# Zehong-Ma/MagCache

Hardware: AMD Instinct MI355X
Metric: denoising steps/sec (MagCache on), Wan2.1-T2V-1.3B 480p 81f (higher is better)
Workload: dtype bf16

## Files before the change

### include/magcache_hip.h

```cpp
#ifndef MAGCACHE_HIP_H
#define MAGCACHE_HIP_H

#include <stddef.h>
#include <stdint.h>

#ifdef __cplusplus
extern "C" {
#endif

typedef struct mc_engine mc_engine;
typedef void* mc_stream;

typedef enum {
  MC_OK = 0,
  MC_EINVAL = 1,
  MC_ENOMEM = 2,
  MC_EHIP = 3,
  MC_ESTATE = 4
} mc_status;

typedef enum { MC_F32 = 0, MC_BF16 = 1 } mc_dtype;

typedef enum {
  MC_MODE_FULL = 0,
  MC_MODE_SKIP = 1,
  MC_MODE_CALIB = 2
} mc_mode;

typedef struct {
  int dim, ffn_dim, num_heads, num_layers;
  int in_dim, out_dim, freq_dim, text_dim, text_len;
  int latent_f, latent_h, latent_w;
  float eps;
  int sp_rank, sp_size;
  int n_branches;
  int calibration;
  int clip_dim;
  int vace_layers;
  int vace_stride;
  int vace_in_dim;
  int fp8_linear;
  int no_context_cache;
  int no_token_timesteps;
  int sp_phases;
} mc_config;

const char* mc_last_error(void);
const char* mc_version(void);
mc_status mc_set_option(const char* key, int value);

mc_status mc_create(const mc_config* cfg, mc_engine** out);
mc_status mc_create_sized(const mc_config* cfg, size_t cfg_bytes, mc_engine** out);
void mc_destroy(mc_engine* e);
size_t mc_workspace_bytes(const mc_engine* e);
mc_status mc_set_workspace(mc_engine* e, void* ws_dev, size_t bytes);
mc_status mc_geometry_bytes(const mc_engine* e, int latent_f, int latent_h, int latent_w, size_t* bytes);
mc_status mc_set_geometry(mc_engine* e, int latent_f, int latent_h, int latent_w);
mc_status mc_buffer_info(const mc_engine* e, const char* name, size_t* offset, size_t* bytes);

mc_status mc_set_weight(mc_engine* e, const char* name, const void* src_dev, mc_dtype dtype, const int64_t* shape,
                        int ndim, mc_stream stream);
int mc_weights_missing(const mc_engine* e, char* buf, size_t buflen);

mc_status mc_lora_set(mc_engine* e, const char* adapter, const char* weight_name, const void* down_dev, const int64_t* down_shape,
                      const void* up_dev, const int64_t* up_shape, mc_dtype dtype, float factor, mc_stream stream);
mc_status mc_lora_set_delta(mc_engine* e, const char* adapter, const char* param_name, const void* delta_dev, size_t numel,
                            mc_dtype dtype, mc_stream stream);
mc_status mc_lora_scale(mc_engine* e, const char* adapter, float scale);
mc_status mc_lora_remove(mc_engine* e, const char* adapter);
mc_status mc_lora_apply(mc_engine* e, mc_stream stream);
mc_status mc_lora_info(const mc_engine* e, int* adapters, int* params, size_t* base_bytes);

mc_status mc_forward(mc_engine* e, const float* latent_dev, const float* t_dev, double t_host,
                     const void* context_dev, mc_dtype ctx_dtype, int ctx_len, int branch, mc_mode mode,
                     float* out_dev, mc_stream stream);

mc_status mc_pair_begin(mc_engine* e);
mc_status mc_pair_end(mc_engine* e);

mc_status mc_set_context(mc_engine* e, int slot, const void* context_dev, mc_dtype ctx_dtype, int ctx_len,
                         mc_stream stream);
mc_status mc_use_context(mc_engine* e, int slot);

mc_status mc_set_clip_fea(mc_engine* e, const void* clip_dev, mc_dtype dtype, int n_tokens, mc_stream stream);

mc_status mc_set_vace_context(mc_engine* e, const float* vace_dev, float context_scale, mc_stream stream);

mc_status mc_set_token_timesteps(mc_engine* e, const float* t_tokens_dev, mc_stream stream);

typedef enum {
  MC_PROF_ATTN_SELF = 0,
  MC_PROF_ATTN_CROSS = 1,
  MC_PROF_GEMM_QKV = 2,
  MC_PROF_GEMM_O = 3,
  MC_PROF_GEMM_CROSS_Q = 4,
  MC_PROF_GEMM_CROSS_O = 5,
  MC_PROF_GEMM_FFN1 = 6,
  MC_PROF_GEMM_FFN2 = 7,
  MC_PROF_LN_MODULATE = 8,
  MC_PROF_RMSNORM_ROPE = 9,
  MC_PROF_EMBED = 10,
  MC_PROF_HEAD = 11,
  MC_PROF_OTHER = 12,
  MC_PROF_SP_WAIT = 13,
  MC_PROF_NCLASS = 14
} mc_prof_class;
mc_status mc_profile_enable(mc_engine* e, int level);
mc_status mc_profile_read(mc_engine* e, double* attn_ms_total, int* attn_launches);
mc_status mc_profile_read_classes(mc_engine* e, double ms_total[MC_PROF_NCLASS], int launches[MC_PROF_NCLASS]);

mc_status mc_embed(mc_engine* e, const float* latent_dev, const float* t_dev, double t_host,
                   const void* context_dev, mc_dtype ctx_dtype, int ctx_len, mc_stream stream);
mc_status mc_block_pre_attn(mc_engine* e, int layer, mc_stream stream);
mc_status mc_block_pre_kv(mc_engine* e, int layer, mc_stream stream);
mc_status mc_block_pre_q(mc_engine* e, int layer, mc_stream stream);
mc_status mc_sp_set_chunks(mc_engine* e, int chunks);
mc_status mc_sp_round_info(const mc_engine* e, int round, int* n_rounds, int* chunk_rows, int* valid);
mc_status mc_block_attn_local(mc_engine* e, int layer, mc_stream stream);
mc_status mc_block_attn_round(mc_engine* e, int layer, int round, mc_stream stream);
mc_status mc_block_post_attn(mc_engine* e, int layer, int branch, mc_mode mode, mc_stream stream);
typedef int (*mc_sp_gather_fn)(void* user, int layer, int phase, mc_stream stream);
mc_status mc_blocks_sp(mc_engine* e, int layer_begin, int layer_end, int branch, mc_mode mode, int overlap,
                       mc_sp_gather_fn gather, void* user, mc_stream stream);
mc_status mc_sp_geometry(const mc_engine* e, int* num_layers, int* seq_len, int* rows_per_rank, int* head_stride, int* dim,
                         int* sp_size);
void* mc_workspace_base(const mc_engine* e);

#define MC_SP_ID_BYTES 128
typedef struct mc_sp_comm mc_sp_comm;
int mc_sp_rccl_available(void);
mc_status mc_sp_comm_id(void* id_out);
mc_status mc_sp_comm_create(const void* id, int nranks, int rank, mc_sp_comm** out);
void mc_sp_comm_destroy(mc_sp_comm* c);
const char* mc_sp_comm_info(const mc_sp_comm* c);
mc_status mc_blocks_sp_rccl(mc_engine* e, mc_sp_comm* c, int layer_begin, int layer_end, int branch, mc_mode mode,
                            int overlap, mc_stream stream);
mc_status mc_forward_sp_rccl(mc_engine* e, mc_sp_comm* c, const float* latent_dev, const float* t_dev, double t_host,
                             const void* context_dev, mc_dtype ctx_dtype, int ctx_len, int branch, mc_mode mode,
                             int overlap, float* tokens_full_dev, float* out_dev, mc_stream stream);
mc_status mc_vace_block_pre(mc_engine* e, int i, mc_stream stream);
mc_status mc_vace_block_post(mc_engine* e, int i, int branch, mc_mode mode, mc_stream stream);
mc_status mc_head(mc_engine* e, int branch, mc_mode mode, mc_stream stream);
mc_status mc_unpatchify(mc_engine* e, const float* tokens_dev, int tok0, int n_tok, float* out_dev,
                        mc_stream stream);

mc_status mc_calib_ready(const mc_engine* e, int branch, int* has_stats);
mc_status mc_calib_finalize(mc_engine* e, int branch, mc_stream stream);
mc_status mc_state_reset(mc_engine* e);
mc_status mc_import_residual(mc_engine* e, int branch, const float* src_dev, mc_stream stream);

typedef struct mc_rule mc_rule;
enum {
  MC_RULE_WAN21 = 0,
  MC_RULE_HUNYUAN = 1,
  MC_RULE_FLUX = 2,
  MC_RULE_WAN22_T2V = 3,
  MC_RULE_WAN22_I2V = 4,
  MC_RULE_WAN22_TI2V = 5,
  MC_RULE_FRAMEPACK = 6,
  MC_RULE_OMNIGEN2 = 7,
  MC_RULE_QWEN = 8,
  MC_RULE_EVAL_WAN = 9,
  MC_RULE_EVAL_OPENSORA = 10
};
mc_rule* mc_rule_create(int variant, int num_steps, double thresh, int K, double retention_ratio,
                        const double* mag_ratios, int n_ratios, int split_step);
void mc_rule_destroy(mc_rule* r);
int mc_rule_step(mc_rule* r, int* branch);
int mc_rule_cnt(const mc_rule* r);
void mc_rule_state(const mc_rule* r, double acc_err[2], int acc_steps[2], double acc_ratio[2]);
void mc_nearest_interp(const double* src, int src_len, double* dst, int target_length);

mc_status mc_op_gemm_bf16(const void* A_dev, long lda, const void* W_dev, long ldw, const float* bias_dev, int M,
                          int N, int K, int epi, void* Cb_dev, long ldc, float* X_dev, long ldx,
                          const float* gate_dev, const void* X0_dev, long ldx0, float* R_dev, long ldr,
                          void* X0out_dev, long ldx0out, int m_valid, mc_stream stream);
mc_status mc_op_gemm_bf16_resid_sel(const void* A_dev, long lda, const void* W_dev, long ldw, const float* bias_dev, int M,
                                    int N, int K, int capture, float* X_dev, long ldx, const float* gate_dev,
                                    const float* gate2_dev, const unsigned char* gate_sel_dev, const void* X0_dev, long ldx0,
                                    float* R_dev, long ldr, mc_stream stream);
mc_status mc_op_gemm_bf16_rowsplit(const void* A_dev, long lda, const void* W_dev, const void* W_b_dev, long ldw,
                                   const float* bias_dev, const float* bias_b_dev, int M, int N, int K, int m_split, int epi,
                                   void* Cb_dev, long ldc, float* X_dev, long ldx, const float* gate_dev, const float* gate_b_dev,
                                   mc_stream stream);
mc_status mc_op_gemm_bf16_gelu_split(const void* A_dev, long lda, const void* W_dev, long ldw, const float* bias_dev, int M,
                                     int N, int K, int n_split, void* Cb_dev, long ldc, void* Cb2_dev, long ldc2,
                                     mc_stream stream);
int mc_op_gemm_bf16_kernel(int M, int N, int K, int epi);
mc_status mc_op_set_splitk_workspace(void* ws_dev, size_t bytes);
int mc_op_gemm_bf16_splitk(int M, int N, int K, int epi);
size_t mc_op_gemm_splitk_need(int M, int N, int K, int epi);
mc_status mc_op_quantize_rows_fp8(const void* x_dev, mc_dtype dtype, long ldx, int M, int K, void* q_dev, long ldq,
                                  float* scale_dev, mc_stream stream);
mc_status mc_op_gemm_fp8(const void* A_q_dev, long lda, const float* a_scale_dev, const void* W_q_dev, long ldw,
                         const float* w_scale_dev, const float* bias_dev, int M, int N, int K, int epi, void* Cb_dev,
                         long ldc, float* X_dev, long ldx, const float* gate_dev, mc_stream stream);
mc_status mc_op_quantize_rows_mx(const void* x_dev, mc_dtype dtype, long ldx, int M, int K, void* q_dev, long ldq,
                                 void* scales_dev, long rows_pad, mc_stream stream);
mc_status mc_op_gemm_mxfp8(const void* A_q_dev, long lda, const void* a_scales_dev, long rows_pad_a, const void* W_q_dev,
                           long ldw, const void* w_scales_dev, long rows_pad_w, const float* bias_dev, int M, int N, int K,
                           int epi, void* Cb_dev, long ldc, float* X_dev, long ldx, const float* gate_dev,
                           mc_stream stream);
mc_status mc_op_attention(const void* Q_dev, long ldq, const void* K_dev, long ldk, long k_shard_stride,
                          const void* V_dev, long ldv, long v_shard_stride, void* O_dev, long ldo, int Lq_pad,
                          int n_heads, int shard_rows, int shard_valid, int n_shards, float scale,
                          mc_stream stream);
mc_status mc_op_attention_partial(const void* Q_dev, long ldq, const void* K_dev, long ldk, long k_shard_stride,
                                  const void* V_dev, long ldv, long v_shard_stride, void* O_dev, long ldo,
                                  int Lq_pad, int n_heads, int shard_rows, int shard_valid, int n_shards,
                                  float scale, int skip_shard, float* lse_out_dev, const float* lse_in_dev,
                                  mc_stream stream);
mc_status mc_op_attn_merge(const void* const* o_parts, const float* const* lse_parts, int n, void* out_bf16_dev, long ldo,
                           int rows, int rows_pad, int d, mc_stream stream);
mc_status mc_op_ln_modulate(const float* x_dev, long ldx, const void* x0_dev, long ldx0, const float* sc_dev,
                            const float* sh_dev, int mode, float eps, void* out_bf16_dev, long ldo,
                            float* out_f32_dev, long ldof, int M, int D, mc_stream stream);
mc_status mc_op_rmsnorm_rope(void* x_bf16_dev, long ldx, const float* w_dev, float eps, const float* cs_dev,
                             int cs_row0, int M, int D, mc_stream stream);
mc_status mc_op_skip_add(const void* x0_bf16_dev, long ldx0, const float* r_dev, long ldr, float* out_dev, long ldo,
                         int M, int D, mc_stream stream);
mc_status mc_op_residual_sub(const float* x_dev, long ldx, const void* x0_bf16_dev, long ldx0, float* r_dev,
                             long ldr, int M, int D, mc_stream stream);
mc_status mc_op_add_rows(float* x_dev, long ldx, const void* s_dev, mc_dtype s_dtype, float* r_dev, long ldr,
                         const void* x0_bf16_dev, long ldx0, int rows, int D, mc_stream stream);
mc_status mc_op_calib_stats(const float* r_dev, long ldr, const float* rp_dev, long ldrp, int M, int D,
                            double* partial_dev, int n_blocks, double* sums_dev, float* stats_dev,
                            mc_stream stream);
mc_status mc_op_cfg_euler(const float* cond_dev, const float* uncond_dev, float guide, float dt, float* x_dev,
                          float* eps_out_dev, size_t n, mc_stream stream);
mc_status mc_op_cfg_norm_euler(const float* cond_dev, const float* uncond_dev, long ld_pred, float guide, float dt,
                               float* x_dev, long ldx, int n_rows, int C, mc_stream stream);
mc_status mc_op_rmsnorm_rows_bf16(const float* x_dev, long ldx, const float* w_dev, float eps, void* out_bf16_dev, long ldo,
                                  int rows_valid, int rows, int D, mc_stream stream);
mc_status mc_op_lincomb(const float* const* xs_dev, const float* coef, int k, float* out_dev, size_t n,
                        mc_stream stream);
mc_status mc_op_cast_bf16(const float* src_dev, void* dst_bf16_dev, size_t n, mc_stream stream);
mc_status mc_op_rope_table(int F, int Hp, int Wp, int tok0, int n_tok, float* cs_host);
mc_status mc_op_rope_axes(int F, int Hp, int Wp, float* axes_host, size_t* n_floats);
mc_status mc_op_rope_expand(const float* axes_dev, int F, int Hp, int Wp, int tok0, int n_tok, int n_rows, float* cs_dev,
                            mc_stream stream);

#define MC_LORA_MAX_TERMS 8
typedef struct mc_lora_term {
  const void* down;
  const void* up;
  int rank;
  float scale;
} mc_lora_term;
size_t mc_op_lora_merge_scratch(int rows, int K, const mc_lora_term* terms, int n_terms);
mc_status mc_op_lora_merge(const void* base_dev, long ld_base, void* out_dev, long ld_out, int rows, int K,
                           const mc_lora_term* terms, int n_terms, void* scratch_dev, size_t scratch_bytes, mc_stream stream);
mc_status mc_op_lora_merge_f32(const float* base_dev, long ld_base, float* out_dev, long ld_out, int rows, int K,
                               const mc_lora_term* terms, int n_terms, void* scratch_dev, size_t scratch_bytes, mc_stream stream);
mc_status mc_op_param_delta(const float* base_dev, float* out_dev, size_t n, const float* const* deltas, const float* scales,
                            int n_terms, mc_stream stream);

#ifdef __cplusplus
}
#endif
#endif
```

### magcache_amd/_lib.py

```python
import ctypes as C
import os

_HERE = os.path.dirname(os.path.abspath(__file__))
LIB_PATH = os.path.join(_HERE, "libmagcache_hip.so")
LIB_PATH = os.environ.get("MAGCACHE_HIP_LIB", LIB_PATH)

MC_OK, MC_EINVAL, MC_ENOMEM, MC_EHIP, MC_ESTATE = 0, 1, 2, 3, 4
MC_F32, MC_BF16 = 0, 1
MC_MODE_FULL, MC_MODE_SKIP, MC_MODE_CALIB = 0, 1, 2
PROF_CLASSES = ("attn_self", "attn_cross", "gemm_qkv", "gemm_o", "gemm_cross_q", "gemm_cross_o", "gemm_ffn1", "gemm_ffn2",
                "ln_modulate", "rmsnorm_rope", "embed", "head", "other", "sp_wait")
RULE_VARIANTS = {"wan21": 0, "hunyuan": 1, "flux": 2, "wan22_t2v": 3, "wan22_i2v": 4, "wan22_ti2v": 5, "framepack": 6,
                 "omnigen2": 7, "qwen": 8, "eval_wan": 9, "eval_opensora": 10}


class McConfig(C.Structure):
    _fields_ = [(n, C.c_int) for n in ("dim", "ffn_dim", "num_heads", "num_layers", "in_dim", "out_dim", "freq_dim",
                                       "text_dim", "text_len", "latent_f", "latent_h", "latent_w")] + \
               [("eps", C.c_float)] + \
               [(n, C.c_int) for n in ("sp_rank", "sp_size", "n_branches", "calibration", "clip_dim", "vace_layers",
                                         "vace_stride", "vace_in_dim", "fp8_linear", "no_context_cache",
                                         "no_token_timesteps", "sp_phases")]


class MagCacheHipError(RuntimeError):
    def __init__(self, status, msg):
        super().__init__(f"magcache_hip status {status}: {msg}")
        self.status = status


_vp, _i, _l, _f, _d, _sz = C.c_void_p, C.c_int, C.c_long, C.c_float, C.c_double, C.c_size_t
SP_GATHER_FN = C.CFUNCTYPE(C.c_int, C.c_void_p, C.c_int, C.c_int, C.c_void_p)

SIGNATURES = {
    "mc_last_error": (C.c_char_p, []),
    "mc_version": (C.c_char_p, []),
    "mc_set_option": (_i, [C.c_char_p, _i]),
    "mc_create": (_i, [C.POINTER(McConfig), C.POINTER(_vp)]),
    "mc_create_sized": (_i, [C.POINTER(McConfig), _sz, C.POINTER(_vp)]),
    "mc_destroy": (None, [_vp]),
    "mc_workspace_bytes": (_sz, [_vp]),
    "mc_set_workspace": (_i, [_vp, _vp, _sz]),
    "mc_geometry_bytes": (_i, [_vp, _i, _i, _i, C.POINTER(_sz)]),
    "mc_set_geometry": (_i, [_vp, _i, _i, _i]),
    "mc_buffer_info": (_i, [_vp, C.c_char_p, C.POINTER(_sz), C.POINTER(_sz)]),
    "mc_set_weight": (_i, [_vp, C.c_char_p, _vp, _i, C.POINTER(C.c_int64), _i, _vp]),
    "mc_weights_missing": (_i, [_vp, C.c_char_p, _sz]),
    "mc_forward": (_i, [_vp, _vp, _vp, _d, _vp, _i, _i, _i, _i, _vp, _vp]),
    "mc_pair_begin": (_i, [_vp]),
    "mc_pair_end": (_i, [_vp]),
    "mc_set_clip_fea": (_i, [_vp, _vp, _i, _i, _vp]),
    "mc_set_vace_context": (_i, [_vp, _vp, _f, _vp]),
    "mc_set_token_timesteps": (_i, [_vp, _vp, _vp]),
    "mc_set_context": (_i, [_vp, _i, _vp, _i, _i, _vp]),
    "mc_use_context": (_i, [_vp, _i]),
    "mc_profile_enable": (_i, [_vp, _i]),
    "mc_profile_read": (_i, [_vp, C.POINTER(_d), C.POINTER(_i)]),
    "mc_profile_read_classes": (_i, [_vp, C.POINTER(_d), C.POINTER(_i)]),
    "mc_embed": (_i, [_vp, _vp, _vp, _d, _vp, _i, _i, _vp]),
    "mc_block_pre_attn": (_i, [_vp, _i, _vp]),
    "mc_block_pre_kv": (_i, [_vp, _i, _vp]),
    "mc_block_pre_q": (_i, [_vp, _i, _vp]),
    "mc_sp_set_chunks": (_i, [_vp, _i]),
    "mc_sp_round_info": (_i, [_vp, _i, C.POINTER(_i), C.POINTER(_i), C.POINTER(_i)]),
    "mc_sp_geometry": (_i, [_vp] + [C.POINTER(_i)] * 6),
    "mc_workspace_base": (_vp, [_vp]),
    "mc_block_attn_local": (_i, [_vp, _i, _vp]),
    "mc_block_attn_round": (_i, [_vp, _i, _i, _vp]),
    "mc_sp_rccl_available": (_i, []),
    "mc_sp_comm_id": (_i, [_vp]),
    "mc_sp_comm_create": (_i, [_vp, _i, _i, C.POINTER(_vp)]),
    "mc_sp_comm_destroy": (None, [_vp]),
    "mc_sp_comm_info": (C.c_char_p, [_vp]),
    "mc_blocks_sp_rccl": (_i, [_vp, _vp, _i, _i, _i, _i, _i, _vp]),
    "mc_forward_sp_rccl": (_i, [_vp, _vp, _vp, _vp, _d, _vp, _i, _i, _i, _i, _i, _vp, _vp, _vp]),
    "mc_block_post_attn": (_i, [_vp, _i, _i, _i, _vp]),
    "mc_blocks_sp": (_i, [_vp, _i, _i, _i, _i, _i, _vp, _vp, _vp]),
    "mc_vace_block_pre": (_i, [_vp, _i, _vp]),
    "mc_vace_block_post": (_i, [_vp, _i, _i, _i, _vp]),
    "mc_head": (_i, [_vp, _i, _i, _vp]),
    "mc_unpatchify": (_i, [_vp, _vp, _i, _i, _vp, _vp]),
    "mc_calib_ready": (_i, [_vp, _i, C.POINTER(_i)]),
    "mc_calib_finalize": (_i, [_vp, _i, _vp]),
    "mc_state_reset": (_i, [_vp]),
    "mc_import_residual": (_i, [_vp, _i, _vp, _vp]),
    "mc_rule_create": (_vp, [_i, _i, _d, _i, _d, C.POINTER(_d), _i, _i]),
    "mc_rule_destroy": (None, [_vp]),
    "mc_rule_step": (_i, [_vp, C.POINTER(_i)]),
    "mc_rule_cnt": (_i, [_vp]),
    "mc_rule_state": (None, [_vp, C.POINTER(_d), C.POINTER(_i), C.POINTER(_d)]),
    "mc_nearest_interp": (None, [C.POINTER(_d), _i, C.POINTER(_d), _i]),
    "mc_op_gemm_bf16": (_i, [_vp, _l, _vp, _l, _vp, _i, _i, _i, _i, _vp, _l, _vp, _l, _vp, _vp, _l, _vp, _l, _vp, _l,
                             _i, _vp]),
    "mc_op_gemm_bf16_resid_sel": (_i, [_vp, _l, _vp, _l, _vp, _i, _i, _i, _i, _vp, _l, _vp, _vp, _vp, _vp, _l, _vp, _l, _vp]),
    "mc_op_gemm_bf16_rowsplit": (_i, [_vp, _l, _vp, _vp, _l, _vp, _vp, _i, _i, _i, _i, _i, _vp, _l, _vp, _l, _vp, _vp, _vp]),
    "mc_op_gemm_bf16_gelu_split": (_i, [_vp, _l, _vp, _l, _vp, _i, _i, _i, _i, _vp, _l, _vp, _l, _vp]),
    "mc_op_gemm_bf16_kernel": (_i, [_i, _i, _i, _i]),
    "mc_op_gemm_bf16_splitk": (_i, [_i, _i, _i, _i]),
    "mc_op_gemm_splitk_need": (_sz, [_i, _i, _i, _i]),
    "mc_op_set_splitk_workspace": (_i, [_vp, _sz]),
    "mc_op_attention": (_i, [_vp, _l, _vp, _l, _l, _vp, _l, _l, _vp, _l, _i, _i, _i, _i, _i, _f, _vp]),
    "mc_op_quantize_rows_fp8": (_i, [_vp, _i, _l, _i, _i, _vp, _l, _vp, _vp]),
    "mc_op_gemm_fp8": (_i, [_vp, _l, _vp, _vp, _l, _vp, _vp, _i, _i, _i, _i, _vp, _l, _vp, _l, _vp, _vp]),
    "mc_op_quantize_rows_mx": (_i, [_vp, _i, _l, _i, _i, _vp, _l, _vp, _l, _vp]),
    "mc_op_gemm_mxfp8": (_i, [_vp, _l, _vp, _l, _vp, _l, _vp, _l, _vp, _i, _i, _i, _i, _vp, _l, _vp, _l, _vp, _vp]),
    "mc_op_attention_partial": (_i, [_vp, _l, _vp, _l, _l, _vp, _l, _l, _vp, _l, _i, _i, _i, _i, _i, _f, _i, _vp, _vp, _vp]),
    "mc_op_attn_merge": (_i, [_vp, _vp, _i, _vp, _l, _i, _i, _i, _vp]),
    "mc_op_ln_modulate": (_i, [_vp, _l, _vp, _l, _vp, _vp, _i, _f, _vp, _l, _vp, _l, _i, _i, _vp]),
    "mc_op_rmsnorm_rope": (_i, [_vp, _l, _vp, _f, _vp, _i, _i, _i, _vp]),
    "mc_op_skip_add": (_i, [_vp, _l, _vp, _l, _vp, _l, _i, _i, _vp]),
    "mc_op_residual_sub": (_i, [_vp, _l, _vp, _l, _vp, _l, _i, _i, _vp]),
    "mc_op_calib_stats": (_i, [_vp, _l, _vp, _l, _i, _i, _vp, _i, _vp, _vp, _vp]),
    "mc_op_cfg_euler": (_i, [_vp, _vp, _f, _f, _vp, _vp, _sz, _vp]),
    "mc_op_cast_bf16": (_i, [_vp, _vp, _sz, _vp]),
    "mc_op_cfg_norm_euler": (_i, [_vp, _vp, _l, _f, _f, _vp, _l, _i, _i, _vp]),
    "mc_op_rmsnorm_rows_bf16": (_i, [_vp, _l, _vp, _f, _vp, _l, _i, _i, _i, _vp]),
    "mc_op_lincomb": (_i, [_vp, _vp, _i, _vp, _sz, _vp]),
    "mc_op_add_rows": (_i, [_vp, _l, _vp, _i, _vp, _l, _vp, _l, _i, _i, _vp]),
    "mc_op_rope_table": (_i, [_i, _i, _i, _i, _i, _vp]),
    "mc_op_rope_axes": (_i, [_i, _i, _i, _vp, C.POINTER(_sz)]),
    "mc_op_rope_expand": (_i, [_vp, _i, _i, _i, _i, _i, _i, _vp, _vp]),
    "mc_op_lora_merge_scratch": (_sz, [_i, _i, _vp, _i]),
    "mc_op_lora_merge": (_i, [_vp, _l, _vp, _l, _i, _i, _vp, _i, _vp, _sz, _vp]),
    "mc_op_lora_merge_f32": (_i, [_vp, _l, _vp, _l, _i, _i, _vp, _i, _vp, _sz, _vp]),
    "mc_op_param_delta": (_i, [_vp, _vp, _sz, C.POINTER(_vp), C.POINTER(_f), _i, _vp]),
    "mc_lora_set": (_i, [_vp, C.c_char_p, C.c_char_p, _vp, C.POINTER(C.c_int64), _vp, C.POINTER(C.c_int64), _i, _f, _vp]),
    "mc_lora_set_delta": (_i, [_vp, C.c_char_p, C.c_char_p, _vp, _sz, _i, _vp]),
    "mc_lora_scale": (_i, [_vp, C.c_char_p, _f]),
    "mc_lora_remove": (_i, [_vp, C.c_char_p]),
    "mc_lora_apply": (_i, [_vp, _vp]),
    "mc_lora_info": (_i, [_vp, C.POINTER(_i), C.POINTER(_i), C.POINTER(_sz)]),
    "mc_mmdit_create": (_i, [_vp, C.POINTER(_vp)]),
    "mc_mmdit_create_sized": (_i, [_vp, _sz, C.POINTER(_vp)]),
    "mc_mmdit_destroy": (None, [_vp]),
    "mc_mmdit_workspace_bytes": (_sz, [_vp]),
    "mc_mmdit_set_workspace": (_i, [_vp, _vp, _sz]),
    "mc_mmdit_buffer_info": (_i, [_vp, C.c_char_p, C.POINTER(_sz), C.POINTER(_sz)]),
    "mc_mmdit_geometry_bytes": (_i, [_vp, _i, _i, _i, _i, _i, C.POINTER(_sz)]),
    "mc_mmdit_set_geometry": (_i, [_vp, _i, _i, _i, _i, _i]),
    "mc_mmdit_set_weight": (_i, [_vp, C.c_char_p, _vp, _i, C.POINTER(C.c_int64), _i, _vp]),
    "mc_mmdit_weights_missing": (_i, [_vp, C.c_char_p, _sz]),
    "mc_mmdit_lora_set": (_i, [_vp, C.c_char_p, C.c_char_p, _vp, C.POINTER(C.c_int64), _vp, C.POINTER(C.c_int64), _i, _f, _vp]),
    "mc_mmdit_lora_scale": (_i, [_vp, C.c_char_p, _f]),
    "mc_mmdit_lora_remove": (_i, [_vp, C.c_char_p]),
    "mc_mmdit_lora_apply": (_i, [_vp, _vp]),
    "mc_mmdit_lora_info": (_i, [_vp, C.POINTER(_i), C.POINTER(_i), C.POINTER(_sz)]),
    "mc_mmdit_set_rope": (_i, [_vp, _vp, _vp, _i, _vp]),
    "mc_mmdit_set_controlnet": (_i, [_vp, _vp, _i, _vp, _i, _i, _i]),
    "mc_mmdit_controlnet_index": (_i, [_i, _i, _i, _i]),
    "mc_mmdit_forward": (_i, [_vp, _vp, _d, _d, _vp, _i, _vp, _i, _vp, _vp]),
    "mc_mmdit_forward2": (_i, [_vp, _vp, _d, _d, _vp, _i, _vp, _i, _i, _vp, _vp]),
    "mc_mmdit_begin": (_i, [_vp, _vp, _d, _d, _vp, _i, _vp, _i, _vp]),
    "mc_mmdit_block_pre": (_i, [_vp, _i, _vp]),
    "mc_mmdit_block_attn_local": (_i, [_vp, _i, _vp]),
    "mc_mmdit_block_post": (_i, [_vp, _i, _vp]),
    "mc_mmdit_end": (_i, [_vp, _vp, _vp]),
    "mc_mmdit_unpatchify": (_i, [_vp, _vp, _vp, _vp]),
    "mc_mmdit_calib_stats": (_i, [_vp, C.POINTER(C.c_float), _vp]),
    "mc_mmdit_state_reset": (_i, [_vp]),
}


class McMmditConfig(C.Structure):
    _fields_ = [(n, C.c_int) for n in ("family", "dim", "num_heads", "n_double", "n_single", "in_channels", "out_channels",
                                       "txt_dim", "txt_len", "vec_dim", "img_tokens", "latent_f", "latent_h", "latent_w",
                                       "refiner_depth", "calibration", "sp_rank", "sp_size",
                                       "fp8_linear")]


MC_FAMILY_FLUX, MC_FAMILY_HUNYUAN, MC_FAMILY_QWEN = 0, 1, 2
MC_LORA_MAX_TERMS = 8


class McLoraTerm(C.Structure):
    _fields_ = [("down", C.c_void_p), ("up", C.c_void_p), ("rank", C.c_int), ("scale", C.c_float)]


_lib = None


def load():
    global _lib
    if _lib is not None:
        return _lib
    if not os.path.exists(LIB_PATH):
        raise ImportError(f"{LIB_PATH} not found: the HIP engine is not built (python -m magcache_amd.build). "
                          "magcache_amd has no CPU fallback by design.")
    import torch
    lib = C.CDLL(LIB_PATH)
    for name, (res, args) in SIGNATURES.items():
        fn = getattr(lib, name)
        fn.restype = res
        fn.argtypes = args
    _lib = lib
    for kv in filter(None, os.environ.get("MAGCACHE_HIP_OPTIONS", "").split(",")):
        key, _, val = kv.partition("=")
        check(lib.mc_set_option(key.strip().encode(), int(val)))
    return lib


def check(status):
    if status != MC_OK:
        raise MagCacheHipError(status, load().mc_last_error().decode())
```

### magcache_amd/csrc/engine.cpp

```cpp
#include <cmath>
#include <cstddef>
#include <memory>

#include "host.h"

using mc::align_up;
using mc::bf16_t;
using mc::fail;
using mc::Keys;
using mc::Linear;
using mc::RowRange;
using mc::whole;

namespace {

struct Layer {
  Linear qkv, o, cq, ckv, co, ffn1, ffn2;
  float *nq, *nk, *cnq, *cnk, *n3w, *n3b, *mod;
  Linear ckv_img;
  float* cnk_img = nullptr;
  int index = 0;
};

}

constexpr int kSpMaxParts = 9;

struct mc_engine {
  mc_config cfg;
  int d, ffn, H, NL, L, Lr, Lp, P, rank, tok0, Kp;
  int ctx_rows;
  std::vector<Layer> layers;
  Linear patch, text0, text1;
  float *w_time0, *b_time0, *w_time1, *b_time1, *w_tproj, *b_tproj;
  float *w_head, *b_head, *head_mod;
  Linear img1, img3;
  float *ln_img0_w = nullptr, *ln_img0_b = nullptr, *ln_img4_w = nullptr, *ln_img4_b = nullptr;
  int img_rows = 0;
  bool have_clip = false;
  bool sp = false;
  int sp_chunks = 1;
  int attn_layer = -2;
  int attn_launches = 0;
  bool attn_local_done = false;
  int attn_rounds_done = 0;
  hipStream_t side = nullptr;
  hipEvent_t ev_fork = nullptr, ev_join = nullptr;
  size_t splitk_bytes = 0;
  bool ctx_valid[2] = {false, false};
  int ctx_active = -1;
  const float* tok_t = nullptr;
  int HT = 64;
  int profile = 0;
  std::vector<hipEvent_t> prof_ev;
  std::vector<uint8_t> prof_cls;
  size_t prof_n = 0;
  std::vector<Layer> vlayers;
  Linear vpatch, before;
  std::vector<Linear> after;
  float* vscale = nullptr;
  int NV = 0, Kvp = 0;
  bool have_vace = false;
  float* cs_table = nullptr;
  float* rope_axes = nullptr;
  int cs_rows = 0;
  size_t axes_cap = 0;
  bool phase_open = false;
  mc::WeightStore weights;
  mc::Workspace work;
  int res_slot[2] = {0, 1};
  int res_scratch = 2;
  bool have_res[2] = {false, false};
  bool have_stats[2] = {false, false};
  bool embedded = false;
  enum { PAIR_NONE, PAIR_ARMED, PAIR_KEPT, PAIR_DEAD };
  int pair = PAIR_NONE;
  const float *pair_latent = nullptr, *pair_t_dev = nullptr;
  double pair_t_host = 0.0;
  bool pair_capable() const { return !sp && NV == 0 && cfg.clip_dim == 0 && cfg.fp8_linear == 0; }
  void pair_drop() { if (pair != PAIR_NONE) pair = PAIR_DEAD; }

  template <class T>
  T* buf(const char* name) const { return work.get<T>(name); }
  float* residual(int idx) const {
    static const char* names[3] = {"residual0", "residual1", "residual2"};
    return buf<float>(names[idx]);
  }
  const Layer& layer(int flat) const { return flat < NL ? layers[flat] : vlayers[flat - NL]; }
  const float* emod(const Layer& l) const { return buf<float>("emod") + (size_t)l.index * 6 * d; }
};

namespace {

struct Prof {
  mc_engine* e;
  hipStream_t s;
  size_t idx = 0;
  bool on = false;
  Prof(mc_engine* e_, int cls, hipStream_t s_) : e(e_), s(s_) {
    if (cls < 0 || !e->profile || (e->profile < 2 && cls != MC_PROF_ATTN_SELF) || e->prof_n + 2 > e->prof_ev.size()) return;
    idx = e->prof_n;
    if (hipEventRecord(e->prof_ev[idx], s) != hipSuccess) return;
    e->prof_cls[idx / 2] = (uint8_t)cls;
    e->prof_n += 2;
    on = true;
  }
  ~Prof() {
    if (on && hipEventRecord(e->prof_ev[idx + 1], s) != hipSuccess) e->prof_cls[idx / 2] = 0xff;
  }
  Prof(const Prof&) = delete;
  Prof& operator=(const Prof&) = delete;
};

constexpr int kRopeT = mc::kRopePairsT, kRopeHW = mc::kRopePairsHW;
constexpr double kRopeDimT = 44.0, kRopeDimHW = 42.0;

inline void rope_pair(int pos, int j, double dim, float* cs) {
  const double fr = 1.0 / std::pow(10000.0, (2.0 * j) / dim);
  const double a = (double)pos * fr;
  cs[0] = (float)std::cos(a);
  cs[1] = (float)std::sin(a);
}

void rope_table_host(int F, int Hp, int Wp, int tok0, int n_tok, float* cs) {
  const int c = kRopeT + 2 * kRopeHW;
  for (int r = 0; r < n_tok; ++r) {
    const int tok = tok0 + r;
    float* row = cs + (size_t)r * 2 * c;
    if (tok >= F * Hp * Wp) {
      for (int i = 0; i < c; ++i) { row[2 * i] = 1.f; row[2 * i + 1] = 0.f; }
      continue;
    }
    const int f = tok / (Hp * Wp), rem = tok % (Hp * Wp), h = rem / Wp, w = rem % Wp;
    for (int i = 0; i < c; ++i) {
      if (i < kRopeT) rope_pair(f, i, kRopeDimT, row + 2 * i);
      else if (i < kRopeT + kRopeHW) rope_pair(h, i - kRopeT, kRopeDimHW, row + 2 * i);
      else rope_pair(w, i - kRopeT - kRopeHW, kRopeDimHW, row + 2 * i);
    }
  }
}

size_t rope_axes_floats(int F, int Hp, int Wp) { return 2 * ((size_t)F * kRopeT + ((size_t)Hp + Wp) * kRopeHW); }

void rope_axes_host(int F, int Hp, int Wp, float* axes) {
  for (int f = 0; f < F; ++f)
    for (int j = 0; j < kRopeT; ++j, axes += 2) rope_pair(f, j, kRopeDimT, axes);
  for (int h = 0; h < Hp; ++h)
    for (int j = 0; j < kRopeHW; ++j, axes += 2) rope_pair(h, j, kRopeDimHW, axes);
  for (int w = 0; w < Wp; ++w)
    for (int j = 0; j < kRopeHW; ++j, axes += 2) rope_pair(w, j, kRopeDimHW, axes);
}

struct Rows { int L, Lr, Lp, tok0; };

mc_status check_geometry(int latent_f, int latent_h, int latent_w, int P) {
  if ((latent_h & 1) || (latent_w & 1) || latent_f <= 0 || latent_h <= 0 || latent_w <= 0)
    return fail(MC_EINVAL, "latent grid %dx%dx%d not divisible by patch (1,2,2)", latent_f, latent_h, latent_w);
  const long long L = (long long)latent_f * (latent_h / 2) * (latent_w / 2);
  if (L > (1ll << 24)) return fail(MC_EINVAL, "latent grid %dx%dx%d: %lld tokens", latent_f, latent_h, latent_w, L);
  if (L % P) return fail(MC_EINVAL, "seq_len %d not divisible by sp_size %d", (int)L, P);
  return MC_OK;
}

Rows derive_rows(int latent_f, int latent_h, int latent_w, int P, int rank) {
  Rows r;
  r.L = latent_f * (latent_h / 2) * (latent_w / 2);
  r.Lr = r.L / P;
  r.Lp = (int)align_up(r.Lr, 256);
  r.tok0 = rank * r.Lr;
  return r;
}

size_t splitk_need(const mc_engine* e, int Lp) {
  return e->sp ? mc::gemm_splitk_ws_need(Lp, e->d, e->ffn, mc::EPI_RESID_GATE) : 0;
}

void plan_workspace(const mc_engine* e, const Rows& rows, mc::Workspace& ws) {
  const mc_config& c = e->cfg;
  const size_t d = e->d, ffn = e->ffn;
  const size_t Lp = rows.Lp;
  ws.add("x", Lp * d * 4);
  ws.add("x0", Lp * d * 2);
  ws.add("xn", Lp * d * 2);
  ws.add("qkv", Lp * 3 * d * 2);
  ws.add("ao", Lp * d * 2);
  ws.add("h", std::max(Lp * ffn * 2, Lp * d * 4));
  ws.add("tokens", Lp * e->Kp * 2);
  ws.add("ctx_in", (size_t)e->ctx_rows * c.text_dim * 2);
  ws.add("ctx_h", (size_t)e->ctx_rows * d * 2);
  ws.add("ctx", (size_t)e->ctx_rows * d * 2);
  ws.add("ckv", (size_t)e->ctx_rows * 2 * d * 2);
  ws.add("ctx_cache", (size_t)2 * e->ctx_rows * d * 2);
  if (!c.no_context_cache)
    ws.add("ckv_cache", (size_t)2 * (e->NL + e->NV) * e->ctx_rows * 2 * d * 2);
  const size_t tsets = c.no_token_timesteps ? 1 : 2;
  ws.add("temb", tsets * (c.freq_dim + 2 * d + 6 * d) * 4);
  ws.add("emod", tsets * (e->NL + e->NV) * 6 * d * 4);
  ws.add("tok_sel", c.no_token_timesteps ? 256 : (size_t)Lp + 256);
  ws.add("tok_t2", 64);
  if (c.fp8_linear) {
    ws.add("aq", Lp * std::max(d, ffn));
    ws.add("a_scale", Lp * 4);
    if (c.fp8_linear >= 2) ws.add("a_mx", (std::max(d, ffn) / 32) * Lp);
  }
  if (e->NV > 0) {
    ws.add("xc", Lp * d * 4);
    ws.add("c0", Lp * d * 2);
    ws.add("vtokens", Lp * (size_t)e->Kvp * 2);
  }
  ws.add("ehead", 2 * 2 * d * 4);
  ws.add("head_tokens", (size_t)Lp * e->HT * 4);
  ws.add("kv_local", e->sp ? Lp * 2 * d * 2 : 256);
  ws.add("kv_gather", e->sp ? (size_t)e->P * Lp * 2 * d * 2 : 256);
  ws.add("residual0", Lp * d * 4);
  ws.add("residual1", c.n_branches > 1 ? Lp * d * 4 : 256);
  ws.add("residual2", c.calibration ? Lp * d * 4 : 256);
  if (c.clip_dim > 0) {
    const size_t ir = e->img_rows, cd = c.clip_dim;
    ws.add("clip_in", ir * cd * 4);
    ws.add("clip_n", ir * cd * 2);
    ws.add("clip_h", ir * cd * 2);
    ws.add("clip_o", ir * d * 4);
    ws.add("clip_h2", ir * d * 2);
    ws.add("ctx_img", ir * d * 2);
    ws.add("ckv_img", ir * 2 * d * 2);
    ws.add("ao2", Lp * d * 2);
  }
  if (e->sp) ws.add("attn_lse", (size_t)e->H * Lp * 4);
  const size_t splitk = splitk_need(e, rows.Lp);
  ws.add("splitk", splitk ? splitk : 256);
  ws.add("ao_part", e->P > 1 ? (size_t)kSpMaxParts * Lp * d * 2 : 256);
  ws.add("lse_part", e->P > 1 ? (size_t)kSpMaxParts * e->H * Lp * 4 : 256);
  ws.add("calib_partial", (2048 * 4 + 2) * 8);
  ws.add("calib_sums", 4 * 8);
  ws.add("calib_stats", 2 * 3 * 4);
  ws.add("pair_x", e->pair_capable() ? Lp * d * 4 : 256);
  ws.add("pair_cq", e->pair_capable() ? Lp * d * 2 : 256);
}

mc_status rope_reserve(mc_engine* e, int Lp, size_t axes_floats) {
  if (Lp > e->cs_rows) {
    float* grown = nullptr;
    MC_TRY(e->weights.alloc(&grown, (size_t)Lp * 128));
    if (e->cs_table) e->weights.release(e->cs_table);
    e->cs_table = grown;
    e->cs_rows = Lp;
  }
  if (axes_floats > e->axes_cap) {
    float* grown = nullptr;
    MC_TRY(e->weights.alloc(&grown, axes_floats));
    if (e->rope_axes) e->weights.release(e->rope_axes);
    e->rope_axes = grown;
    e->axes_cap = axes_floats;
  }
  return MC_OK;
}

mc_status rope_build(mc_engine* e) {
  const int F = e->cfg.latent_f, Hp = e->cfg.latent_h / 2, Wp = e->cfg.latent_w / 2;
  std::vector<float> axes(rope_axes_floats(F, Hp, Wp));
  rope_axes_host(F, Hp, Wp, axes.data());
  HIP_TRY(hipMemcpy(e->rope_axes, axes.data(), axes.size() * sizeof(float), hipMemcpyHostToDevice));
  HIP_TRY(mc::launch_rope_expand(e->rope_axes, F, Hp, Wp, e->tok0, e->Lr, e->Lp, e->cs_table, nullptr));
  HIP_TRY(hipStreamSynchronize(nullptr));
  return MC_OK;
}

mc_status forget_workspace_state(mc_engine* e) {
  e->have_res[0] = e->have_res[1] = false;
  e->have_stats[0] = e->have_stats[1] = false;
  e->res_slot[0] = 0; e->res_slot[1] = 1; e->res_scratch = 2;
  e->embedded = e->phase_open = false;
  e->ctx_valid[0] = e->ctx_valid[1] = false;
  e->ctx_active = -1;
  e->have_clip = e->have_vace = false;
  e->tok_t = nullptr;
  e->attn_layer = -2;
  e->pair_drop();
  if (e->work.ws) HIP_TRY(hipMemset(e->buf<double>("calib_partial") + 2048 * 4, 0, 16));
  return MC_OK;
}

mc_status check_ready(const mc_engine* e) {
  if (!e) return fail(MC_EINVAL, "null engine");
  if (e->weights.dirty()) return fail(MC_ESTATE, "LoRA adapters, scales or a touched weight changed: call mc_lora_apply first");
  return mc::check_ready(e->work, e->weights, "mc_set_workspace");
}

struct ActSrc {
  const bf16_t* rows = nullptr; long ld = 0;
  bool quantised = false;
  uint8_t *q = nullptr, *mx = nullptr;
};

mc_status linear(mc_engine* e, const Linear& l, RowRange out, int M, ActSrc a, mc::GemmParams p, int epi, hipStream_t s) {
  const int K = l.k_in;
  if (!l.q) {
    HIP_TRY(mc::launch_linear_bf16(l, out, a.rows, a.ld, M, p, epi, s));
    return MC_OK;
  }
  const int Lp = e->Lp;
  if (M != Lp) return fail(MC_EINVAL, "an fp8 Linear runs over the %d rows of a block, not %d", Lp, M);
  p.M = Lp; p.N = out.count; p.K = K; p.bias = l.b + out.first;
  uint8_t* aq = a.q ? a.q : e->buf<uint8_t>("aq");
  p.A = (const bf16_t*)aq; p.lda = K; p.W = (const bf16_t*)(l.q + (size_t)out.first * K); p.ldw = K;
  if (l.mx) {
    uint8_t* am = a.mx ? a.mx : e->buf<uint8_t>("a_mx");
    if (!a.quantised) HIP_TRY(mc::launch_quantize_rows_mx(a.rows, nullptr, a.ld, Lp, K, aq, K, am, (long)Lp, s));
    p.a_mx = am; p.mx_rows_a = (long)Lp; p.w_mx = l.mx + out.first; p.mx_rows_w = l.n_out;
    HIP_TRY(mc::launch_gemm_mxfp8(p, epi, s));
    return MC_OK;
  }
  float* as = e->buf<float>("a_scale");
  if (!a.quantised) HIP_TRY(mc::launch_quantize_rows_fp8(a.rows, nullptr, a.ld, Lp, K, aq, K, as, s));
  p.a_scale = as; p.w_scale = l.q_scale + out.first;
  HIP_TRY(mc::launch_gemm_fp8(p, epi, s));
  return MC_OK;
}
mc_status linear_bf16_out(mc_engine* e, const Linear& l, int M, ActSrc a, bf16_t* C, int epi, hipStream_t s) {
  mc::GemmParams p = {};
  p.Cb = C; p.ldc = l.n_out;
  return linear(e, l, whole(l), M, a, p, epi, s);
}

Keys kv_pairs(const bf16_t* kv, int d, int rows, int valid) { return {kv, kv + d, 2L * d, 0, rows, valid, 1, 0}; }
Keys qkv_keys(const mc_engine* e) {
  const bf16_t* k = e->buf<bf16_t>("qkv") + e->d;
  return {k, k + e->d, 3L * e->d, 0, e->Lp, e->Lr, 1, 0};
}
Keys local_keys(const mc_engine* e) { return kv_pairs(e->buf<bf16_t>("kv_local"), e->d, e->Lp, e->Lr); }
int sp_chunk_rows(const mc_engine* e) { return e->Lp / e->sp_chunks; }
int sp_round_valid(const mc_engine* e, int c) {
  const int lc = sp_chunk_rows(e);
  return std::max(0, std::min(lc, e->Lr - c * lc));
}
int sp_rounds(const mc_engine* e) {
  const int lc = sp_chunk_rows(e);
  return (e->Lr + lc - 1) / lc;
}
Keys sp_keys(const mc_engine* e, int round, bool skip_own) {
  if (round < 0) return local_keys(e);
  const int lc = sp_chunk_rows(e), d = e->d;
  Keys k = kv_pairs(e->buf<bf16_t>("kv_gather") + (size_t)round * e->P * lc * 2 * d, d, lc, sp_round_valid(e, round));
  k.stride = (long)lc * 2 * d; k.n_shards = e->P; k.skip_shard_p1 = skip_own ? e->rank + 1 : 0;
  return k;
}
mc_status attend(const mc_engine* e, const bf16_t* Q, long ldq, bf16_t* O, const Keys& keys, const float* lse_in, float* lse_out,
                 hipStream_t s) {
  HIP_TRY(mc::launch_attention_keys(Q, ldq, O, e->d, e->Lp, e->H, keys, lse_in, lse_out, s));
  return MC_OK;
}
void attn_chain_set(mc_engine* e, int layer, int launches, bool local_done, int rounds_done) {
  e->attn_layer = layer; e->attn_launches = launches; e->attn_local_done = local_done; e->attn_rounds_done = rounds_done;
}
void attn_chain_open(mc_engine* e, int layer) {
  if (e->attn_layer != layer) attn_chain_set(e, layer, 0, false, 0);
}

}

namespace mc {
int g_fp8_fused_quant = 1;
int g_sp_attn_partials = 1;
}
static int g_n_cu = 0;

extern "C" {

mc_status mc_create_sized(const mc_config* cfg, size_t cfg_bytes, mc_engine** out) {
  if (!cfg || !out) return fail(MC_EINVAL, "null argument");
  if (cfg_bytes < offsetof(mc_config, fp8_linear) || cfg_bytes > sizeof(mc_config) || (cfg_bytes % sizeof(int)) != 0)
    return fail(MC_EINVAL, "mc_config of %zu bytes: this library knows %zu (0.1 layout) .. %zu", cfg_bytes,
                offsetof(mc_config, fp8_linear), sizeof(mc_config));
  mc_config full;
  memset(&full, 0, sizeof(full));
  memcpy(&full, cfg, cfg_bytes);
  return mc_create(&full, out);
}

mc_status mc_create(const mc_config* cfg, mc_engine** out) {
  if (!cfg || !out) return fail(MC_EINVAL, "null argument");
  const mc_config& c = *cfg;
  if (c.dim <= 0 || c.num_heads <= 0 || c.dim != c.num_heads * 128)
    return fail(MC_EINVAL, "dim (%d) must be num_heads (%d) * 128", c.dim, c.num_heads);
  if ((c.dim % 256) || (c.ffn_dim % 64) || (c.text_dim % 64) || (c.freq_dim % 4) || c.num_layers <= 0)
    return fail(MC_EINVAL, "unsupported geometry dim=%d ffn=%d text_dim=%d", c.dim, c.ffn_dim, c.text_dim);
  if (c.sp_size < 1 || c.sp_rank < 0 || c.sp_rank >= c.sp_size) return fail(MC_EINVAL, "bad sp rank/size");
  MC_TRY(check_geometry(c.latent_f, c.latent_h, c.latent_w, c.sp_size));
  if (c.n_branches != 1 && c.n_branches != 2) return fail(MC_EINVAL, "n_branches must be 1 or 2");
  if (c.out_dim * 4 > 256) return fail(MC_EINVAL, "out_dim*4 > 256 unsupported by the head kernel");
  if (c.clip_dim < 0 || (c.clip_dim % 256) != 0) return fail(MC_EINVAL, "clip_dim %d must be 0 or a multiple of 256", c.clip_dim);
  if (c.vace_layers < 0 || (c.vace_layers > 0 && (c.vace_stride <= 0 || c.vace_in_dim <= 0 ||
                                                   (c.vace_layers - 1) * c.vace_stride >= c.num_layers)))
    return fail(MC_EINVAL, "bad VACE geometry: %d blocks, stride %d, in_dim %d", c.vace_layers, c.vace_stride, c.vace_in_dim);
  if ((c.no_context_cache | c.no_token_timesteps) & ~1) return fail(MC_EINVAL, "no_context_cache / no_token_timesteps must be 0 or 1");
  if (c.fp8_linear < 0 || c.fp8_linear > 3)
    return fail(MC_EINVAL, "fp8_linear must be 0, 1 (per-row scales), 2 (MX block scales: QKV, FFN-1, FFN-2) or 3 (MX, the d x d Linears too)");
  if (c.fp8_linear && ((c.dim % 256) || (c.ffn_dim % 256) || c.dim < 512 || c.ffn_dim < 512))
    return fail(MC_EINVAL, "fp8_linear needs dim and ffn_dim to be multiples of 256 and >= 512");
  if (c.vace_layers > 0 && c.sp_size > 1 && (c.vace_layers - 1) * c.vace_stride == c.num_layers - 1)
    return fail(MC_EINVAL, "VACE with a hint on the last layer is single-GPU in this engine");

  std::unique_ptr<mc_engine, void (*)(mc_engine*)> own(new mc_engine(), mc_destroy);
  mc_engine* e = own.get();
  e->cfg = c;
  e->d = c.dim; e->ffn = c.ffn_dim; e->H = c.num_heads; e->NL = c.num_layers;
  e->P = c.sp_size; e->rank = c.sp_rank;
  e->sp = c.sp_size > 1 || c.sp_phases != 0;
  const Rows rows = derive_rows(c.latent_f, c.latent_h, c.latent_w, e->P, e->rank);
  e->L = rows.L; e->Lr = rows.Lr; e->Lp = rows.Lp; e->tok0 = rows.tok0;
  e->Kp = (int)align_up((size_t)c.in_dim * 4, 64);
  e->HT = (int)align_up((size_t)c.out_dim * 4, 64);
  e->ctx_rows = (int)align_up(c.text_len, 64);
  const size_t d = e->d, ffn = e->ffn;
  mc::WeightStore& W = e->weights;
  W.allow_f32_targets = true;

  const mc::Quant q_big = c.fp8_linear >= 2 ? mc::QUANT_MX : c.fp8_linear == 1 ? mc::QUANT_ROW : mc::QUANT_NONE;
  const mc::Quant q_dd = c.fp8_linear == 3 ? mc::QUANT_MX : mc::QUANT_NONE;
  e->layers.resize(e->NL);
  e->NV = c.vace_layers;
  e->vlayers.resize(e->NV);
  for (int i = 0; i < e->NL + e->NV; ++i) {
    const bool is_vace = i >= e->NL;
    Layer& l = is_vace ? e->vlayers[i - e->NL] : e->layers[i];
    l.index = i;
    const std::string p = (is_vace ? "vace_blocks." + std::to_string(i - e->NL) : "blocks." + std::to_string(i)) + ".";
    MC_TRY(W.add_linear(l.qkv, p + "self_attn.", {{"q", d}, {"k", d}, {"v", d}}, d, q_big));
    MC_TRY(W.add_linear(l.o, p + "self_attn.", {{"o", d}}, d, q_dd));
    MC_TRY(W.add_linear(l.cq, p + "cross_attn.", {{"q", d}}, d, q_dd));
    MC_TRY(W.add_linear(l.ckv, p + "cross_attn.", {{"k", d}, {"v", d}}, d));
    MC_TRY(W.add_linear(l.co, p + "cross_attn.", {{"o", d}}, d, q_dd));
    MC_TRY(W.add_linear(l.ffn1, p + "ffn.", {{"0", ffn}}, d, q_big));
    MC_TRY(W.add_linear(l.ffn2, p + "ffn.", {{"2", d}}, ffn, q_big));
    MC_TRY(W.add_f32(l.nq, p + "self_attn.norm_q.weight", d));
    MC_TRY(W.add_f32(l.nk, p + "self_attn.norm_k.weight", d));
    MC_TRY(W.add_f32(l.n3w, p + "norm3.weight", d));
    MC_TRY(W.add_f32(l.n3b, p + "norm3.bias", d));
    MC_TRY(W.add_f32(l.cnq, p + "cross_attn.norm_q.weight", d));
    MC_TRY(W.add_f32(l.cnk, p + "cross_attn.norm_k.weight", d));
    MC_TRY(W.add_f32(l.mod, p + "modulation", 6 * d));
    if (c.clip_dim > 0) {
      MC_TRY(W.add_linear(l.ckv_img, p + "cross_attn.", {{"k_img", d}, {"v_img", d}}, d));
      MC_TRY(W.add_f32(l.cnk_img, p + "cross_attn.norm_k_img.weight", d));
    }
  }
  if (e->NV > 0) {
    e->Kvp = (int)align_up((size_t)c.vace_in_dim * 4, 64);
    const size_t kv = (size_t)c.vace_in_dim * 4;
    if (kv != (size_t)e->Kvp) { return fail(MC_EINVAL, "vace_in_dim*4 must be a multiple of 64"); }
    MC_TRY(W.add_linear(e->vpatch, "", {{"vace_patch_embedding", d}}, kv));
    W.slots.at("vace_patch_embedding.weight").fixed = true;
    MC_TRY(W.add_linear(e->before, "vace_blocks.0.", {{"before_proj", d}}, d));
    MC_TRY(W.alloc(&e->vscale, d));
    e->after.resize(e->NV);
    for (int i = 0; i < e->NV; ++i)
      MC_TRY(W.add_linear(e->after[i], "vace_blocks." + std::to_string(i) + ".", {{"after_proj", d}}, d));
  }
  if (c.clip_dim > 0) {
    const size_t cd = c.clip_dim;
    e->img_rows = (int)align_up(257, 64);
    MC_TRY(W.add_f32(e->ln_img0_w, "img_emb.proj.0.weight", cd));
    MC_TRY(W.add_f32(e->ln_img0_b, "img_emb.proj.0.bias", cd));
    MC_TRY(W.add_linear(e->img1, "img_emb.proj.", {{"1", cd}}, cd));
    MC_TRY(W.add_linear(e->img3, "img_emb.proj.", {{"3", d}}, cd));
    MC_TRY(W.add_f32(e->ln_img4_w, "img_emb.proj.4.weight", d));
    MC_TRY(W.add_f32(e->ln_img4_b, "img_emb.proj.4.bias", d));
  }
  const size_t kin = (size_t)c.in_dim * 4;
  MC_TRY(W.alloc_linear(e->patch, d, e->Kp));
  HIP_TRY(hipMemset(e->patch.w, 0, d * e->Kp * sizeof(bf16_t)));
  mc::Slot& w_patch = W.add_parts(e->patch, "", {{"patch_embedding", d}});
  w_patch.fixed = true;
  if (kin != (size_t)e->Kp) {
    w_patch.numel = d * kin;
    w_patch.pad = {d, kin, (size_t)e->Kp};
  }
  MC_TRY(W.add_linear(e->text0, "text_embedding.", {{"0", d}}, c.text_dim));
  MC_TRY(W.add_linear(e->text1, "text_embedding.", {{"2", d}}, d));
  MC_TRY(W.add_f32(e->w_time0, "time_embedding.0.weight", d * c.freq_dim, c.freq_dim));
  MC_TRY(W.add_f32(e->b_time0, "time_embedding.0.bias", d));
  MC_TRY(W.add_f32(e->w_time1, "time_embedding.2.weight", d * d, d));
  MC_TRY(W.add_f32(e->b_time1, "time_embedding.2.bias", d));
  MC_TRY(W.add_f32(e->w_tproj, "time_projection.1.weight", 6 * d * d, d));
  MC_TRY(W.add_f32(e->b_tproj, "time_projection.1.bias", 6 * d));
  MC_TRY(W.add_f32(e->w_head, "head.head.weight", (size_t)c.out_dim * 4 * d, d));
  MC_TRY(W.add_f32(e->b_head, "head.head.bias", (size_t)c.out_dim * 4));
  MC_TRY(W.add_f32(e->head_mod, "head.modulation", 2 * d));

  MC_TRY(rope_reserve(e, e->Lp, rope_axes_floats(c.latent_f, c.latent_h / 2, c.latent_w / 2)));
  MC_TRY(rope_build(e));

  e->splitk_bytes = splitk_need(e, e->Lp);
  plan_workspace(e, rows, e->work);
  *out = own.release();
  return MC_OK;
}

void mc_destroy(mc_engine* e) {
  if (!e) return;
  e->weights.free_all();
  for (hipEvent_t ev : e->prof_ev) (void)hipEventDestroy(ev);
  if (e->ev_fork) (void)hipEventDestroy(e->ev_fork);
  if (e->ev_join) (void)hipEventDestroy(e->ev_join);
  if (e->side) (void)hipStreamDestroy(e->side);
  delete e;
}

size_t mc_workspace_bytes(const mc_engine* e) { return e ? e->work.need : 0; }

mc_status mc_set_workspace(mc_engine* e, void* ws_dev, size_t bytes) {
  if (!e) return fail(MC_EINVAL, "null argument");
  MC_TRY(e->work.bind(ws_dev, bytes));
  return forget_workspace_state(e);
}

mc_status mc_geometry_bytes(const mc_engine* e, int latent_f, int latent_h, int latent_w, size_t* bytes) {
  if (!e || !bytes) return fail(MC_EINVAL, "null argument");
  MC_TRY(check_geometry(latent_f, latent_h, latent_w, e->P));
  mc::Workspace plan;
  plan_workspace(e, derive_rows(latent_f, latent_h, latent_w, e->P, e->rank), plan);
  *bytes = plan.need;
  return MC_OK;
}

mc_status mc_set_geometry(mc_engine* e, int latent_f, int latent_h, int latent_w) {
  if (!e) return fail(MC_EINVAL, "null engine");
  if (e->sp)
    return fail(MC_EINVAL, "mc_set_geometry: a sharded engine (sp_size %d%s) keeps the grid it was created with", e->P,
                e->cfg.sp_phases ? ", sp_phases" : "");
  if (e->phase_open) return fail(MC_ESTATE, "mc_set_geometry between mc_embed and mc_head");
  MC_TRY(check_geometry(latent_f, latent_h, latent_w, e->P));
  const Rows r = derive_rows(latent_f, latent_h, latent_w, e->P, e->rank);
  mc::Workspace plan;
  plan_workspace(e, r, plan);
  if (e->work.ws && plan.need > e->work.bound)
    return fail(MC_EINVAL, "latent grid %dx%dx%d needs a workspace of %zu bytes, %zu bytes are bound (mc_set_workspace)", latent_f,
                latent_h, latent_w, plan.need, e->work.bound);
  HIP_TRY(hipDeviceSynchronize());
  MC_TRY(rope_reserve(e, r.Lp, rope_axes_floats(latent_f, latent_h / 2, latent_w / 2)));
  MC_TRY(e->work.replan(plan));
  e->cfg.latent_f = latent_f; e->cfg.latent_h = latent_h; e->cfg.latent_w = latent_w;
  e->L = r.L; e->Lr = r.Lr; e->Lp = r.Lp; e->tok0 = r.tok0;
  MC_TRY(rope_build(e));
  return forget_workspace_state(e);
}

mc_status mc_buffer_info(const mc_engine* e, const char* name, size_t* offset, size_t* bytes) {
  if (!e || !name) return fail(MC_EINVAL, "null argument");
  std::string n(name);
  if (n == "residual_branch0" || n == "residual_branch1") {
    static const char* names[3] = {"residual0", "residual1", "residual2"};
    n = names[e->res_slot[n.back() - '0']];
  }
  return e->work.info(n, offset, bytes);
}

mc_status mc_set_weight(mc_engine* e, const char* name, const void* src_dev, mc_dtype dtype, const int64_t* shape,
                        int ndim, mc_stream stream) {
  if (e) {
    e->ctx_valid[0] = e->ctx_valid[1] = false;
    e->ctx_active = -1;
    e->pair_drop();
  }
  if (!e || !name || !src_dev || !shape) return fail(MC_EINVAL, "null argument");
  return e->weights.set(name, src_dev, dtype, shape, ndim, (hipStream_t)stream);
}

int mc_weights_missing(const mc_engine* e, char* buf, size_t buflen) { return e ? e->weights.missing(buf, buflen) : -1; }

static mc_status lora_entry(const mc_engine* e, const char* what) {
  if (!e) return fail(MC_EINVAL, "null engine");
  if (e->pair != mc_engine::PAIR_NONE) return fail(MC_ESTATE, "%s between mc_pair_begin and mc_pair_end", what);
  if (e->phase_open) return fail(MC_ESTATE, "%s between mc_embed and mc_head", what);
  return MC_OK;
}

mc_status mc_lora_set(mc_engine* e, const char* adapter, const char* weight_name, const void* down_dev, const int64_t* down_shape,
                      const void* up_dev, const int64_t* up_shape, mc_dtype dtype, float factor, mc_stream stream) {
  MC_TRY(lora_entry(e, "mc_lora_set"));
  if (!adapter || !weight_name || !down_dev || !down_shape || !up_dev || !up_shape) return fail(MC_EINVAL, "null argument");
  if (down_shape[0] <= 0 || down_shape[0] > (1 << 20) || down_shape[1] <= 0 || up_shape[0] <= 0 || up_shape[1] != down_shape[0])
    return fail(MC_EINVAL, "LoRA '%s': down [%lld, %lld] and up [%lld, %lld] share no rank", weight_name, (long long)down_shape[0],
                (long long)down_shape[1], (long long)up_shape[0], (long long)up_shape[1]);
  return e->weights.lora_set(adapter, weight_name, down_dev, (size_t)down_shape[0] * down_shape[1], up_dev,
                             (size_t)up_shape[0] * up_shape[1], dtype, (int)down_shape[0], factor, (hipStream_t)stream);
}

mc_status mc_lora_set_delta(mc_engine* e, const char* adapter, const char* param_name, const void* delta_dev, size_t numel,
                            mc_dtype dtype, mc_stream stream) {
  MC_TRY(lora_entry(e, "mc_lora_set_delta"));
  if (!adapter || !param_name || !delta_dev) return fail(MC_EINVAL, "null argument");
  return e->weights.lora_set_delta(adapter, param_name, delta_dev, numel, dtype, (hipStream_t)stream);
}

mc_status mc_lora_scale(mc_engine* e, const char* adapter, float scale) {
  MC_TRY(lora_entry(e, "mc_lora_scale"));
  if (!adapter) return fail(MC_EINVAL, "null argument");
  return e->weights.lora_scale(adapter, scale);
}

mc_status mc_lora_remove(mc_engine* e, const char* adapter) {
  MC_TRY(lora_entry(e, "mc_lora_remove"));
  return e->weights.lora_remove(adapter);
}

mc_status mc_lora_apply(mc_engine* e, mc_stream stream) {
  MC_TRY(lora_entry(e, "mc_lora_apply"));
  int merged = 0;
  const mc_status st = e->weights.lora_apply((hipStream_t)stream, &merged);
  if (merged > 0) {
    e->ctx_valid[0] = e->ctx_valid[1] = false;
    e->ctx_active = -1;
    e->have_clip = e->have_vace = false;
    e->pair_drop();
  }
  return st;
}

mc_status mc_lora_info(const mc_engine* e, int* adapters, int* params, size_t* base_bytes) {
  if (!e) return fail(MC_EINVAL, "null engine");
  e->weights.lora_info(adapters, params, base_bytes);
  return MC_OK;
}

mc_status mc_set_clip_fea(mc_engine* e, const void* clip_dev, mc_dtype dtype, int n_tokens, mc_stream stream_) {
  hipStream_t s = (hipStream_t)stream_;
  MC_TRY(check_ready(e));
  e->pair_drop();
  const mc_config& c = e->cfg;
  if (c.clip_dim <= 0) return fail(MC_EINVAL, "engine was created without clip_dim (t2v model)");
  if (!clip_dev || n_tokens != 257) return fail(MC_EINVAL, "clip_fea must be [257, %d]", c.clip_dim);
  const int cd = c.clip_dim, ir = e->img_rows, d = e->d;
  float* in = e->buf<float>("clip_in");
  HIP_TRY(hipMemsetAsync(in, 0, (size_t)ir * cd * 4, s));
  if (dtype == MC_F32) {
    HIP_TRY(hipMemcpyAsync(in, clip_dev, (size_t)n_tokens * cd * 4, hipMemcpyDeviceToDevice, s));
  } else {
    return fail(MC_EINVAL, "clip_fea must be given as fp32");
  }
  bf16_t* n0 = e->buf<bf16_t>("clip_n");
  HIP_TRY(mc::launch_ln_modulate(in, cd, nullptr, 0, e->ln_img0_w, e->ln_img0_b, 1, 1e-5f, n0, cd, nullptr, 0, ir, cd, s));
  MC_TRY(linear_bf16_out(e, e->img1, ir, ActSrc{n0, cd}, e->buf<bf16_t>("clip_h"), mc::EPI_GELU_ERF_BF16, s));
  MC_TRY(linear_bf16_out(e, e->img3, ir, ActSrc{e->buf<bf16_t>("clip_h"), cd}, e->buf<bf16_t>("clip_h2"), mc::EPI_BF16, s));
  HIP_TRY(hipMemsetAsync(e->buf<float>("clip_o"), 0, (size_t)ir * d * 4, s));
  HIP_TRY(mc::launch_ln_modulate(e->buf<float>("clip_o"), d, e->buf<bf16_t>("clip_h2"), d, e->ln_img4_w,
                                 e->ln_img4_b, 1, 1e-5f, e->buf<bf16_t>("ctx_img"), d, nullptr, 0, ir, d, s));
  e->have_clip = true;
  return MC_OK;
}

mc_status mc_set_vace_context(mc_engine* e, const float* vace_dev, float context_scale, mc_stream stream_) {
  hipStream_t s = (hipStream_t)stream_;
  MC_TRY(check_ready(e));
  e->pair_drop();
  if (e->NV <= 0) return fail(MC_EINVAL, "engine was created without VACE blocks");
  const mc_config& c = e->cfg;
  const int d = e->d;
  if (vace_dev) {
    bf16_t* vt = e->buf<bf16_t>("vtokens");
    HIP_TRY(mc::launch_patchify(vace_dev, c.vace_in_dim, c.latent_f, c.latent_h, c.latent_w, e->tok0, e->Lr, e->Lp, vt,
                                e->Kvp, s));
    mc::GemmParams p = {};
    p.X = e->buf<float>("xc"); p.ldx = d;
    p.X0out = e->buf<bf16_t>("c0"); p.ldx0out = d;
    p.m_valid = e->Lr;
    MC_TRY(linear(e, e->vpatch, whole(e->vpatch), e->Lp, ActSrc{vt, e->Kvp}, p, mc::EPI_EMBED, s));
    e->have_vace = true;
  } else if (!e->have_vace) {
    return fail(MC_EINVAL, "null vace_context and none set before");
  }
  std::vector<float> sc(d, context_scale);
  HIP_TRY(hipMemcpyAsync(e->vscale, sc.data(), (size_t)d * 4, hipMemcpyHostToDevice, s));
  HIP_TRY(hipStreamSynchronize(s));
  return MC_OK;
}

static mc_status embed_context(mc_engine* e, const void* context_dev, mc_dtype ctx_dtype, int ctx_len, bf16_t* dst,
                               hipStream_t s) {
  const mc_config& c = e->cfg;
  if (ctx_len <= 0 || ctx_len > c.text_len)
    return fail(MC_EINVAL, "context length %d exceeds text_len %d", ctx_len, c.text_len);
  bf16_t* ctx_in = e->buf<bf16_t>("ctx_in");
  if (ctx_dtype == MC_F32) {
    HIP_TRY(mc::launch_cast_pad_bf16((const float*)context_dev, c.text_dim, ctx_len, e->ctx_rows, c.text_dim, ctx_in,
                                     c.text_dim, s));
  } else {
    HIP_TRY(hipMemsetAsync(ctx_in, 0, (size_t)e->ctx_rows * c.text_dim * 2, s));
    HIP_TRY(hipMemcpyAsync(ctx_in, context_dev, (size_t)ctx_len * c.text_dim * 2, hipMemcpyDeviceToDevice, s));
  }
  bf16_t* ctx_h = e->buf<bf16_t>("ctx_h");
  MC_TRY(linear_bf16_out(e, e->text0, e->ctx_rows, ActSrc{ctx_in, c.text_dim}, ctx_h, mc::EPI_GELU_BF16, s));
  return linear_bf16_out(e, e->text1, e->ctx_rows, ActSrc{ctx_h, e->d}, dst, mc::EPI_BF16, s);
}

static mc_status context_kv(mc_engine* e, const Layer& l, const bf16_t* ctx, bf16_t* ckv, hipStream_t s) {
  const int d = e->d;
  MC_TRY(linear_bf16_out(e, l.ckv, e->ctx_rows, ActSrc{ctx, d}, ckv, mc::EPI_BF16, s));
  HIP_TRY(mc::launch_rmsnorm_rope(ckv, 2 * d, l.cnk, e->cfg.eps, nullptr, 0, e->ctx_rows, d, s));
  return MC_OK;
}

static mc_status embed_latent_time(mc_engine* e, const float* latent_dev, const float* t_dev, double t_host, float* x,
                                   hipStream_t s) {
  const mc_config& c = e->cfg;
  const int d = e->d;
  bf16_t* tokens = e->buf<bf16_t>("tokens");
  if (e->Kp != c.in_dim * 4) HIP_TRY(hipMemsetAsync(tokens, 0, (size_t)e->Lp * e->Kp * 2, s));
  HIP_TRY(mc::launch_patchify(latent_dev, c.in_dim, c.latent_f, c.latent_h, c.latent_w, e->tok0, e->Lr, e->Lp,
                              tokens, e->Kp, s));
  {
    mc::GemmParams p = {};
    p.X = x; p.ldx = d;
    p.X0out = e->buf<bf16_t>("x0"); p.ldx0out = d;
    p.m_valid = e->Lr;
    MC_TRY(linear(e, e->patch, whole(e->patch), e->Lp, ActSrc{tokens, e->Kp}, p, mc::EPI_EMBED, s));
  }
  const int n_sets = e->tok_t ? 2 : 1;
  float* t2 = e->buf<float>("tok_t2");
  if (e->tok_t)
    HIP_TRY(mc::launch_token_t_prepare(e->tok_t, e->L, e->tok0, e->Lr, e->Lp, t2, e->buf<uint8_t>("tok_sel"), s));
  const size_t temb_set = (size_t)c.freq_dim + 2 * d + 6 * d, emod_set = (size_t)(e->NL + e->NV) * 6 * d;
  for (int set = 0; set < n_sets; ++set) {
    float* temb = e->buf<float>("temb") + set * temb_set;
    float* sinus = temb;
    float* h1 = temb + c.freq_dim;
    float* ev = h1 + d;
    float* e0 = ev + d;
    HIP_TRY(mc::launch_sinusoid(e->tok_t ? t2 + set : t_dev, t_host, c.freq_dim, sinus, s));
    HIP_TRY(mc::launch_gemv_f32(e->w_time0, sinus, e->b_time0, h1, d, c.freq_dim, 0, 1, s));
    HIP_TRY(mc::launch_gemv_f32(e->w_time1, h1, e->b_time1, ev, d, d, 0, 0, s));
    HIP_TRY(mc::launch_gemv_f32(e->w_tproj, ev, e->b_tproj, e0, 6 * d, d, 1, 0, s));
    float* emod = e->buf<float>("emod") + set * emod_set;
    for (int l = 0; l < e->NL + e->NV; ++l)
      HIP_TRY(mc::launch_add_bcast(e0, 6 * d, e->layer(l).mod, emod + (size_t)l * 6 * d, 6 * d, s));
    HIP_TRY(mc::launch_add_bcast(ev, d, e->head_mod, e->buf<float>("ehead") + set * 2 * d, 2 * d, s));
  }
  return MC_OK;
}

static mc_status embed_text(mc_engine* e, const void* context_dev, mc_dtype ctx_dtype, int ctx_len, hipStream_t s) {
  if (context_dev) {
    e->ctx_active = -1;
    return embed_context(e, context_dev, ctx_dtype, ctx_len, e->buf<bf16_t>("ctx"), s);
  }
  if (e->ctx_active < 0 || !e->ctx_valid[e->ctx_active])
    return fail(MC_ESTATE, "context_dev is NULL but no cached context is selected (mc_set_context)");
  return MC_OK;
}

static mc_status embed(mc_engine* e, const float* latent_dev, const float* t_dev, double t_host, const void* context_dev,
                       mc_dtype ctx_dtype, int ctx_len, float* x, hipStream_t s) {
  MC_TRY(check_ready(e));
  if (!latent_dev) return fail(MC_EINVAL, "null input");
  if (e->cfg.clip_dim > 0 && !e->have_clip)
    return fail(MC_ESTATE, "i2v model: mc_set_clip_fea must run before the forward (reference assert :226-227)");
  Prof pr(e, MC_PROF_EMBED, s);
  MC_TRY(embed_latent_time(e, latent_dev, t_dev, t_host, x, s));
  MC_TRY(embed_text(e, context_dev, ctx_dtype, ctx_len, s));
  e->embedded = true;
  return MC_OK;
}

mc_status mc_embed(mc_engine* e, const float* latent_dev, const float* t_dev, double t_host,
                   const void* context_dev, mc_dtype ctx_dtype, int ctx_len, mc_stream stream_) {
  if (e) e->pair_drop();
  const mc_status st = embed(e, latent_dev, t_dev, t_host, context_dev, ctx_dtype, ctx_len, e ? e->buf<float>("x") : nullptr,
                             (hipStream_t)stream_);
  if (e && st == MC_OK) e->phase_open = true;
  return st;
}

static mc_status ln_for_gemm(mc_engine* e, const Linear& l, const float* x, const float* sc, const float* sh, int mode,
                             const float* sc2, const float* sh2, const uint8_t* sel, hipStream_t s, ActSrc* a) {
  const int d = e->d, Lp = e->Lp;
  bf16_t* xn = e->buf<bf16_t>("xn");
  *a = ActSrc{xn, d, l.q && mc::g_fp8_fused_quant};
  if (a->quantised) {
    HIP_TRY(mc::launch_ln_modulate_fp8(x, d, sc, sh, mode, e->cfg.eps, e->buf<uint8_t>("aq"), d,
                                       l.mx ? nullptr : e->buf<float>("a_scale"), l.mx ? e->buf<uint8_t>("a_mx") : nullptr,
                                       (long)Lp, Lp, d, s, sc2, sh2, sel));
  } else {
    HIP_TRY(mc::launch_ln_modulate(x, d, nullptr, 0, sc, sh, mode, e->cfg.eps, xn, d, nullptr, 0, Lp, d, s, sc2, sh2, sel));
  }
  return MC_OK;
}

static const float* second_set(const mc_engine* e, const float* em) {
  return e->tok_t ? em + (size_t)(e->NL + e->NV) * 6 * e->d : nullptr;
}
static const uint8_t* tok_sel(const mc_engine* e) { return e->tok_t ? e->buf<uint8_t>("tok_sel") : nullptr; }

static mc_status block_pre_kv(mc_engine* e, const Layer& l, const float* em, float* x, hipStream_t s) {
  const int d = e->d, Lp = e->Lp;
  const float* em2 = second_set(e, em);
  ActSrc a;
  {
    Prof pr(e, MC_PROF_LN_MODULATE, s);
    MC_TRY(ln_for_gemm(e, l.qkv, x, em + d, em, 0, em2 ? em2 + d : nullptr, em2, tok_sel(e), s, &a));
  }
  mc::GemmParams p = {};
  if (!e->sp) {
    bf16_t* qkv = e->buf<bf16_t>("qkv");
    p.Cb = qkv; p.ldc = 3 * d;
    {
      Prof pr(e, MC_PROF_GEMM_QKV, s);
      MC_TRY(linear(e, l.qkv, whole(l.qkv), Lp, a, p, mc::EPI_BF16, s));
    }
    Prof pr(e, MC_PROF_RMSNORM_ROPE, s);
    HIP_TRY(mc::launch_rmsnorm_rope(qkv, 3 * d, l.nq, e->cfg.eps, e->cs_table, 0, Lp, d, s));
    HIP_TRY(mc::launch_rmsnorm_rope(qkv + d, 3 * d, l.nk, e->cfg.eps, e->cs_table, 0, Lp, d, s));
  } else {
    bf16_t* kvl = e->buf<bf16_t>("kv_local");
    p.Cb = kvl; p.ldc = 2 * d;
    {
      Prof pr(e, MC_PROF_GEMM_QKV, s);
      MC_TRY(linear(e, l.qkv, RowRange{d, 2 * d}, Lp, a, p, mc::EPI_BF16, s));
    }
    Prof pr(e, MC_PROF_RMSNORM_ROPE, s);
    HIP_TRY(mc::launch_rmsnorm_rope(kvl, 2 * d, l.nk, e->cfg.eps, e->cs_table, 0, Lp, d, s));
  }
  e->attn_layer = -2;
  return MC_OK;
}

static mc_status block_pre_q(mc_engine* e, const Layer& l, hipStream_t s) {
  const int d = e->d, Lp = e->Lp;
  if (!e->sp) return MC_OK;
  bf16_t* qkv = e->buf<bf16_t>("qkv");
  {
    Prof pr(e, MC_PROF_GEMM_QKV, s);
    mc::GemmParams p = {};
    p.Cb = qkv; p.ldc = d;
    MC_TRY(linear(e, l.qkv, RowRange{0, d}, Lp, ActSrc{e->buf<bf16_t>("xn"), d, true}, p, mc::EPI_BF16, s));
  }
  Prof pr(e, MC_PROF_RMSNORM_ROPE, s);
  HIP_TRY(mc::launch_rmsnorm_rope(qkv, d, l.nq, e->cfg.eps, e->cs_table, 0, Lp, d, s));
  return MC_OK;
}

static mc_status block_pre(mc_engine* e, const Layer& l, const float* em, float* x, hipStream_t s) {
  MC_TRY(block_pre_kv(e, l, em, x, s));
  return block_pre_q(e, l, s);
}

static mc_status check_layer_call(mc_engine* e, int layer) {
  if (!e || !e->embedded) return fail(MC_ESTATE, "mc_embed must run first");
  if (layer < 0 || layer >= e->NL) return fail(MC_EINVAL, "layer %d out of range", layer);
  return MC_OK;
}

mc_status mc_block_pre_attn(mc_engine* e, int layer, mc_stream stream_) {
  MC_TRY(check_layer_call(e, layer));
  e->pair_drop();
  return block_pre(e, e->layers[layer], e->emod(e->layers[layer]), e->buf<float>("x"), (hipStream_t)stream_);
}

mc_status mc_block_pre_kv(mc_engine* e, int layer, mc_stream stream_) {
  MC_TRY(check_layer_call(e, layer));
  if (!e->sp) return fail(MC_ESTATE, "mc_block_pre_kv needs a sequence-parallel engine (sp_size > 1 or sp_phases) (one GPU: mc_block_pre_attn / mc_forward)");
  e->pair_drop();
  return block_pre_kv(e, e->layers[layer], e->emod(e->layers[layer]), e->buf<float>("x"), (hipStream_t)stream_);
}

mc_status mc_block_pre_q(mc_engine* e, int layer, mc_stream stream_) {
  MC_TRY(check_layer_call(e, layer));
  if (!e->sp) return fail(MC_ESTATE, "mc_block_pre_q needs a sequence-parallel engine (sp_size > 1 or sp_phases)");
  e->pair_drop();
  return block_pre_q(e, e->layers[layer], (hipStream_t)stream_);
}

static mc_status sp_attn_launch(mc_engine* e, int layer, int round, hipStream_t s) {
  attn_chain_open(e, layer);
  const int n_rounds = sp_rounds(e);
  bool more;
  if (round < 0) {
    if (e->attn_launches) return fail(MC_ESTATE, "the local-shard attention must be the first launch of a layer's chain");
    more = true;
  } else {
    if (round != e->attn_rounds_done || round >= n_rounds)
      return fail(MC_ESTATE, "attention round %d out of order (rounds done %d of %d)", round, e->attn_rounds_done, n_rounds);
    more = round + 1 < n_rounds;
    if (e->attn_local_done && e->P == 1) {
      e->attn_rounds_done++;
      return MC_OK;
    }
  }
  float* lse = e->buf<float>("attn_lse");
  {
    Prof pr(e, MC_PROF_ATTN_SELF, s);
    MC_TRY(attend(e, e->buf<bf16_t>("qkv"), e->d, e->buf<bf16_t>("ao"), sp_keys(e, round, e->attn_local_done),
                  e->attn_launches ? lse : nullptr, more ? lse : nullptr, s));
  }
  e->attn_launches++;
  if (round < 0) e->attn_local_done = true; else e->attn_rounds_done++;
  return MC_OK;
}

static mc_status sp_attn_partial(mc_engine* e, int round, hipStream_t s) {
  const size_t slot = round < 0 ? 0 : 1 + round;
  return attend(e, e->buf<bf16_t>("qkv"), e->d, e->buf<bf16_t>("ao_part") + slot * e->Lp * e->d, sp_keys(e, round, true), nullptr,
                e->buf<float>("lse_part") + slot * e->H * e->Lp, s);
}

static mc_status sp_side_stream(mc_engine* e) {
  if (e->side) return MC_OK;
  HIP_TRY(hipStreamCreateWithFlags(&e->side, hipStreamNonBlocking));
  HIP_TRY(hipEventCreateWithFlags(&e->ev_fork, hipEventDisableTiming));
  HIP_TRY(hipEventCreateWithFlags(&e->ev_join, hipEventDisableTiming));
  return MC_OK;
}

mc_status mc_block_attn_local(mc_engine* e, int layer, mc_stream stream_) {
  MC_TRY(check_layer_call(e, layer));
  if (!e->sp) return fail(MC_ESTATE, "mc_block_attn_local needs a sequence-parallel engine (sp_size > 1 or sp_phases)");
  return sp_attn_launch(e, layer, -1, (hipStream_t)stream_);
}

mc_status mc_block_attn_round(mc_engine* e, int layer, int round, mc_stream stream_) {
  MC_TRY(check_layer_call(e, layer));
  if (!e->sp) return fail(MC_ESTATE, "mc_block_attn_round needs a sequence-parallel engine (sp_size > 1 or sp_phases)");
  if (round < 0) return fail(MC_EINVAL, "round %d", round);
  return sp_attn_launch(e, layer, round, (hipStream_t)stream_);
}

mc_status mc_sp_set_chunks(mc_engine* e, int chunks) {
  if (!e) return fail(MC_EINVAL, "null engine");
  if (!e->sp) return fail(MC_ESTATE, "mc_sp_set_chunks needs a sequence-parallel engine (sp_size > 1 or sp_phases)");
  if (chunks < 1 || chunks > 64 || e->Lp % chunks || (e->Lp / chunks) % 64)
    return fail(MC_EINVAL, "sp chunks %d: rows per shard %d / chunks must be a multiple of 64", chunks, e->Lp);
  e->sp_chunks = chunks;
  e->attn_layer = -2;
  e->pair_drop();
  return MC_OK;
}

mc_status mc_sp_geometry(const mc_engine* e, int* num_layers, int* seq_len, int* rows_per_rank, int* head_stride, int* dim,
                         int* sp_size) {
  if (!e) return fail(MC_EINVAL, "null engine");
  if (num_layers) *num_layers = e->NL;
  if (seq_len) *seq_len = e->L;
  if (rows_per_rank) *rows_per_rank = e->Lr;
  if (head_stride) *head_stride = e->HT;
  if (dim) *dim = e->d;
  if (sp_size) *sp_size = e->P;
  return MC_OK;
}

void* mc_workspace_base(const mc_engine* e) { return e ? (void*)e->work.ws : nullptr; }

mc_status mc_sp_round_info(const mc_engine* e, int round, int* n_rounds, int* chunk_rows, int* valid) {
  if (!e) return fail(MC_EINVAL, "null engine");
  if (round < 0 || round >= e->sp_chunks) return fail(MC_EINVAL, "round %d of %d", round, e->sp_chunks);
  if (n_rounds) *n_rounds = e->sp ? sp_rounds(e) : 0;
  if (chunk_rows) *chunk_rows = sp_chunk_rows(e);
  if (valid) *valid = sp_round_valid(e, round);
  return MC_OK;
}

static mc_status block_post_self(mc_engine* e, const Layer& l, const float* em, float* x, int layer, bf16_t* cq, hipStream_t s) {
  const int d = e->d, Lp = e->Lp;
  bf16_t* ao = e->buf<bf16_t>("ao");
  const float* em2 = second_set(e, em);
  const uint8_t* sel = tok_sel(e);

  if (!e->sp) {
    Prof pr(e, MC_PROF_ATTN_SELF, s);
    MC_TRY(attend(e, e->buf<bf16_t>("qkv"), 3 * d, ao, qkv_keys(e), nullptr, nullptr, s));
  } else {
    attn_chain_open(e, layer);
    while (e->attn_rounds_done < sp_rounds(e)) MC_TRY(sp_attn_launch(e, layer, e->attn_rounds_done, s));
    e->attn_layer = -2;
  }
  {
    Prof pr(e, MC_PROF_GEMM_O, s);
    mc::GemmParams p = {};
    p.X = x; p.ldx = d; p.gate = em + 2 * d;
    if (em2) { p.gate2 = em2 + 2 * d; p.gate_sel = sel; }
    MC_TRY(linear(e, l.o, whole(l.o), Lp, ActSrc{ao, d}, p, mc::EPI_RESID_GATE, s));
  }
  ActSrc xn;
  {
    Prof pr(e, MC_PROF_LN_MODULATE, s);
    MC_TRY(ln_for_gemm(e, l.cq, x, l.n3w, l.n3b, 1, nullptr, nullptr, nullptr, s, &xn));
  }
  {
    Prof pr(e, MC_PROF_GEMM_CROSS_Q, s);
    MC_TRY(linear_bf16_out(e, l.cq, Lp, xn, cq, mc::EPI_BF16, s));
  }
  Prof pr(e, MC_PROF_RMSNORM_ROPE, s);
  HIP_TRY(mc::launch_rmsnorm_rope(cq, d, l.cnq, e->cfg.eps, nullptr, 0, Lp, d, s));
  return MC_OK;
}

static float* capture_dst(const mc_engine* e, int branch, mc_mode mode) {
  return e->residual(mode == MC_MODE_CALIB ? e->res_scratch : e->res_slot[branch]);
}
static mc_status capture_written(mc_engine* e, int branch, mc_mode mode, bool timed, hipStream_t s) {
  const int d = e->d;
  if (mode == MC_MODE_CALIB) {
    if (!e->cfg.calibration) return fail(MC_ESTATE, "engine was created without calibration=1");
    if (e->have_res[branch]) {
      Prof pr(e, timed ? MC_PROF_OTHER : -1, s);
      HIP_TRY(mc::launch_calib_stats(e->residual(e->res_scratch), d, e->residual(e->res_slot[branch]), d, e->Lr, d,
                                     e->buf<double>("calib_partial"), 2048, e->buf<double>("calib_sums"),
                                     e->buf<float>("calib_stats") + 3 * branch, s));
    }
    e->have_stats[branch] = e->have_res[branch];
    std::swap(e->res_slot[branch], e->res_scratch);
  }
  e->have_res[branch] = true;
  return MC_OK;
}

static mc_status block_post_ctx(mc_engine* e, const Layer& l, const float* em, float* x, const bf16_t* cq, bool capture,
                                int branch, mc_mode mode, hipStream_t s) {
  const int d = e->d, Lp = e->Lp, ffn = e->ffn;
  bf16_t* ao = e->buf<bf16_t>("ao");
  const float* em2 = second_set(e, em);
  const uint8_t* sel = tok_sel(e);
  bf16_t* ckv = e->buf<bf16_t>("ckv");
  {
    if (e->ctx_active >= 0) {
      ckv = e->buf<bf16_t>("ckv_cache") + ((size_t)e->ctx_active * (e->NL + e->NV) + l.index) * e->ctx_rows * 2 * d;
    } else {
      Prof pr(e, MC_PROF_OTHER, s);
      MC_TRY(context_kv(e, l, e->buf<bf16_t>("ctx"), ckv, s));
    }
    {
      Prof pr(e, MC_PROF_ATTN_CROSS, s);
      MC_TRY(attend(e, cq, d, ao, kv_pairs(ckv, d, e->ctx_rows, e->cfg.text_len), nullptr, nullptr, s));
    }
    if (e->cfg.clip_dim > 0) {
      Prof pr(e, MC_PROF_OTHER, s);
      bf16_t* ckvi = e->buf<bf16_t>("ckv_img");
      bf16_t* ao2 = e->buf<bf16_t>("ao2");
      MC_TRY(linear_bf16_out(e, l.ckv_img, e->img_rows, ActSrc{e->buf<bf16_t>("ctx_img"), d}, ckvi, mc::EPI_BF16, s));
      HIP_TRY(mc::launch_rmsnorm_rope(ckvi, 2 * d, l.cnk_img, e->cfg.eps, nullptr, 0, e->img_rows, d, s));
      MC_TRY(attend(e, cq, d, ao2, kv_pairs(ckvi, d, e->img_rows, 257), nullptr, nullptr, s));
      HIP_TRY(mc::launch_add_bf16(ao, ao2, (size_t)Lp * d, s));
    }
    Prof pr(e, MC_PROF_GEMM_CROSS_O, s);
    mc::GemmParams o = {};
    o.X = x; o.ldx = d; o.gate = nullptr;
    MC_TRY(linear(e, l.co, whole(l.co), Lp, ActSrc{ao, d}, o, mc::EPI_RESID_GATE, s));
  }
  ActSrc xn;
  {
    Prof pr(e, MC_PROF_LN_MODULATE, s);
    MC_TRY(ln_for_gemm(e, l.ffn1, x, em + 4 * d, em + 3 * d, 0, em2 ? em2 + 4 * d : nullptr, em2 ? em2 + 3 * d : nullptr, sel,
                       s, &xn));
  }
  bf16_t* h = e->buf<bf16_t>("h");
  mc::GemmParams p = {};
  p.Cb = h; p.ldc = ffn;
  const bool h_fp8 = l.ffn1.mx && l.ffn2.mx && mc::g_fp8_fused_quant;
  ActSrc hidden{h, ffn};
  if (h_fp8) {
    hidden.quantised = true; hidden.q = (uint8_t*)h; hidden.mx = hidden.q + (size_t)Lp * ffn;
    p.Cq = hidden.q; p.ldcq = ffn; p.c_mx = hidden.mx; p.mx_rows_c = Lp;
  }
  {
    Prof pr(e, MC_PROF_GEMM_FFN1, s);
    MC_TRY(linear(e, l.ffn1, whole(l.ffn1), Lp, xn, p, h_fp8 ? mc::EPI_GELU_MXFP8 : mc::EPI_GELU_BF16, s));
  }
  mc::GemmParams q = {};
  q.X = x; q.ldx = d; q.gate = em + 5 * d;
  if (e->splitk_bytes) { q.splitk_ws = e->buf<float>("splitk"); q.splitk_ws_bytes = e->splitk_bytes; }
  if (em2) { q.gate2 = em2 + 5 * d; q.gate_sel = sel; }
  if (capture) {
    q.X0 = e->buf<bf16_t>("x0"); q.ldx0 = d;
    q.R = capture_dst(e, branch, mode); q.ldr = d;
  }
  {
    Prof pr(e, MC_PROF_GEMM_FFN2, s);
    MC_TRY(linear(e, l.ffn2, whole(l.ffn2), Lp, hidden, q, capture ? mc::EPI_RESID_CAPTURE : mc::EPI_RESID_GATE, s));
  }
  return capture ? capture_written(e, branch, mode, true, s) : MC_OK;
}

static mc_status block_post(mc_engine* e, const Layer& l, const float* em, float* x, int layer, bf16_t* cq, bool capture,
                            int branch, mc_mode mode, hipStream_t s) {
  MC_TRY(block_post_self(e, l, em, x, layer, cq, s));
  return block_post_ctx(e, l, em, x, cq, capture, branch, mode, s);
}

static bool hint_on_last_layer(const mc_engine* e) {
  return e->NV > 0 && (e->NV - 1) * e->cfg.vace_stride == e->NL - 1;
}

mc_status mc_block_post_attn(mc_engine* e, int layer, int branch, mc_mode mode, mc_stream stream_) {
  if (!e || !e->embedded) return fail(MC_ESTATE, "mc_embed must run first");
  if (layer < 0 || layer >= e->NL) return fail(MC_EINVAL, "layer %d out of range", layer);
  if (branch < 0 || branch >= e->cfg.n_branches) return fail(MC_EINVAL, "branch %d out of range", branch);
  e->pair_drop();
  return block_post(e, e->layers[layer], e->emod(e->layers[layer]), e->buf<float>("x"), layer, e->buf<bf16_t>("qkv"),
                    layer == e->NL - 1 && !hint_on_last_layer(e), branch, mode, (hipStream_t)stream_);
}

static mc_status vace_pre_kv(mc_engine* e, int i, hipStream_t s) {
  const int d = e->d, Lp = e->Lp;
  float* xc = e->buf<float>("xc");
  if (i == 0) {
    HIP_TRY(hipMemsetAsync(xc, 0, (size_t)Lp * d * 4, s));
    HIP_TRY(mc::launch_skip_add(e->buf<bf16_t>("x0"), d, xc, d, xc, d, Lp, d, s));
    mc::GemmParams p = {};
    p.X = xc; p.ldx = d; p.gate = nullptr;
    MC_TRY(linear(e, e->before, whole(e->before), Lp, ActSrc{e->buf<bf16_t>("c0"), d}, p, mc::EPI_RESID_GATE, s));
  }
  return block_pre_kv(e, e->vlayers[i], e->emod(e->vlayers[i]), xc, s);
}

static mc_status vace_pre(mc_engine* e, int i, hipStream_t s) {
  MC_TRY(vace_pre_kv(e, i, s));
  return block_pre_q(e, e->vlayers[i], s);
}

static mc_status vace_post(mc_engine* e, int i, int branch, mc_mode mode, hipStream_t s) {
  const int d = e->d, Lp = e->Lp;
  float* xc = e->buf<float>("xc");
  MC_TRY(block_post(e, e->vlayers[i], e->emod(e->vlayers[i]), xc, -1, e->buf<bf16_t>("qkv"), false, branch, mode, s));
  bf16_t* xn = e->buf<bf16_t>("xn");
  HIP_TRY(mc::launch_cast_bf16(xc, xn, (size_t)Lp * d, s));
  mc::GemmParams h = {};
  h.X = e->buf<float>("x"); h.ldx = d; h.gate = e->vscale;
  return linear(e, e->after[i], whole(e->after[i]), Lp, ActSrc{xn, d}, h, mc::EPI_RESID_GATE, s);
}

static mc_status vace_block(mc_engine* e, int i, int branch, mc_mode mode, hipStream_t s) {
  MC_TRY(vace_pre(e, i, s));
  return vace_post(e, i, branch, mode, s);
}

mc_status mc_vace_block_pre(mc_engine* e, int i, mc_stream stream) {
  if (!e || !e->embedded) return fail(MC_ESTATE, "mc_embed must run first");
  if (i < 0 || i >= e->NV) return fail(MC_EINVAL, "VACE block %d out of range", i);
  if (!e->have_vace) return fail(MC_ESTATE, "mc_set_vace_context must run first");
  return vace_pre(e, i, (hipStream_t)stream);
}

mc_status mc_vace_block_post(mc_engine* e, int i, int branch, mc_mode mode, mc_stream stream) {
  if (!e || !e->embedded) return fail(MC_ESTATE, "mc_embed must run first");
  if (i < 0 || i >= e->NV) return fail(MC_EINVAL, "VACE block %d out of range", i);
  if (branch < 0 || branch >= e->cfg.n_branches) return fail(MC_EINVAL, "branch %d out of range", branch);
  return vace_post(e, i, branch, mode, (hipStream_t)stream);
}

mc_status mc_blocks_sp(mc_engine* e, int layer_begin, int layer_end, int branch, mc_mode mode, int overlap,
                       mc_sp_gather_fn gather, void* user, mc_stream stream) {
  if (!e || !e->embedded) return fail(MC_ESTATE, "mc_embed must run first");
  if (!gather) return fail(MC_EINVAL, "null gather callback");
  if (!e->sp) return fail(MC_ESTATE, "mc_blocks_sp needs a sequence-parallel engine (sp_size > 1 or sp_phases) (one GPU: mc_forward)");
  if (layer_begin < 0 || layer_end > e->NL || layer_begin > layer_end)
    return fail(MC_EINVAL, "layers [%d, %d) out of range (num_layers %d)", layer_begin, layer_end, e->NL);
  if (mode == MC_MODE_SKIP) return fail(MC_EINVAL, "a skipped forward runs no blocks (mc_embed -> mc_head)");
  hipStream_t s = (hipStream_t)stream;
  const int R = sp_rounds(e);
  auto coll = [&](int layer, int phase) -> mc_status {
    const int rc = gather(user, layer, phase, stream);
    return rc == 0 ? MC_OK : fail(MC_ESTATE, "gather callback failed (layer %d, phase %d, code %d)", layer, phase, rc);
  };
  auto wait_round = [&](int layer, int c, hipStream_t on) -> mc_status {
    Prof pr(e, MC_PROF_SP_WAIT, on);
    const int rc = gather(user, layer, 2 * c + 1, (mc_stream)on);
    return rc == 0 ? MC_OK : fail(MC_ESTATE, "gather callback failed (layer %d, phase %d, code %d)", layer, 2 * c + 1, rc);
  };
  if (!g_n_cu) {
    int dev = 0, n = 0;
    if (hipGetDevice(&dev) == hipSuccess && hipDeviceGetAttribute(&n, hipDeviceAttributeMultiprocessorCount, dev) == hipSuccess && n > 0)
      g_n_cu = n;
    else
      g_n_cu = 256;
  }
  const long wg = (long)(e->Lp / 256) * e->H, waves = (wg + g_n_cu - 1) / g_n_cu;
  const bool underfilled = wg * 10 < waves * g_n_cu * 9;
  const bool partials = (mc::g_sp_attn_partials == 2 || (mc::g_sp_attn_partials == 1 && underfilled)) && e->P > 1 && 1 + R <= kSpMaxParts;
  if (partials) MC_TRY(sp_side_stream(e));
  auto chain = [&](int l, const Layer& ly, int chain_id) -> mc_status {
    for (int c = 0; c < R; ++c) MC_TRY(coll(l, 2 * c));
    if (!overlap)
      for (int c = 0; c < R; ++c) MC_TRY(wait_round(l, c, s));
    MC_TRY(block_pre_q(e, ly, s));
    if (!partials) {
      MC_TRY(sp_attn_launch(e, chain_id, -1, s));
      for (int c = 0; c < R; ++c) {
        if (overlap) MC_TRY(wait_round(l, c, s));
        MC_TRY(sp_attn_launch(e, chain_id, c, s));
      }
      return MC_OK;
    }
    Prof chain_pr(e, MC_PROF_ATTN_SELF, s);
    HIP_TRY(hipEventRecord(e->ev_fork, s));
    HIP_TRY(hipStreamWaitEvent(e->side, e->ev_fork, 0));
    MC_TRY(sp_attn_partial(e, -1, s));
    for (int c = 0; c < R; ++c) {
      hipStream_t on = (c & 1) ? s : e->side;
      if (overlap) MC_TRY(wait_round(l, c, on));
      MC_TRY(sp_attn_partial(e, c, on));
    }
    HIP_TRY(hipEventRecord(e->ev_join, e->side));
    HIP_TRY(hipStreamWaitEvent(s, e->ev_join, 0));
    const bf16_t* op[kSpMaxParts];
    const float* lp[kSpMaxParts];
    for (int i = 0; i <= R; ++i) {
      op[i] = e->buf<bf16_t>("ao_part") + (size_t)i * e->Lp * e->d;
      lp[i] = e->buf<float>("lse_part") + (size_t)i * e->H * e->Lp;
    }
    HIP_TRY(mc::launch_attn_merge(op, lp, 1 + R, e->buf<bf16_t>("ao"), e->d, e->Lp, e->Lp, e->d, s));
    attn_chain_set(e, chain_id, 1 + R, true, R);
    return MC_OK;
  };
  for (int l = layer_begin; l < layer_end; ++l) {
    MC_TRY(block_pre_kv(e, e->layers[l], e->emod(e->layers[l]), e->buf<float>("x"), s));
    MC_TRY(chain(l, e->layers[l], l));
    MC_TRY(mc_block_post_attn(e, l, branch, mode, stream));
    if (e->NV > 0 && l % e->cfg.vace_stride == 0 && l / e->cfg.vace_stride < e->NV) {
      const int i = l / e->cfg.vace_stride;
      if (!e->have_vace) return fail(MC_ESTATE, "mc_set_vace_context must run first");
      MC_TRY(vace_pre_kv(e, i, s));
      MC_TRY(chain(l, e->vlayers[i], -1));
      MC_TRY(mc_vace_block_post(e, i, branch, mode, stream));
    }
  }
  return MC_OK;
}

static mc_status capture_unfused(mc_engine* e, int branch, mc_mode mode, hipStream_t s) {
  const int d = e->d;
  HIP_TRY(mc::launch_residual_sub(e->buf<float>("x"), d, e->buf<bf16_t>("x0"), d, capture_dst(e, branch, mode), d, e->Lp, d, s));
  return capture_written(e, branch, mode, false, s);
}

static mc_status head(mc_engine* e, const float* x, int branch, mc_mode mode, hipStream_t s) {
  if (!e || !e->embedded) return fail(MC_ESTATE, "mc_embed must run first");
  if (branch < 0 || branch >= e->cfg.n_branches) return fail(MC_EINVAL, "branch %d out of range", branch);
  const int d = e->d;
  const float* eh = e->buf<float>("ehead");
  const float* eh2 = e->tok_t ? eh + 2 * d : nullptr;
  const uint8_t* sel = tok_sel(e);
  float* hn = e->buf<float>("h");
  Prof pr(e, MC_PROF_HEAD, s);
  if (mode == MC_MODE_SKIP) {
    if (!e->have_res[branch]) return fail(MC_ESTATE, "skip requested but residual_cache[%d] is empty", branch);
    HIP_TRY(mc::launch_ln_modulate(e->residual(e->res_slot[branch]), d, e->buf<bf16_t>("x0"), d, eh + d, eh, 0,
                                   e->cfg.eps, nullptr, 0, hn, d, e->Lr, d, s, eh2 ? eh2 + d : nullptr, eh2, sel));
  } else {
    HIP_TRY(mc::launch_ln_modulate(x, d, nullptr, 0, eh + d, eh, 0, e->cfg.eps, nullptr, 0, hn, d,
                                   e->Lr, d, s, eh2 ? eh2 + d : nullptr, eh2, sel));
  }
  HIP_TRY(mc::launch_head_linear(hn, d, e->w_head, e->b_head, e->buf<float>("head_tokens"), e->HT, e->Lr,
                                 e->cfg.out_dim * 4, d, s));
  return MC_OK;
}

mc_status mc_head(mc_engine* e, int branch, mc_mode mode, mc_stream stream) {
  if (!e) return fail(MC_ESTATE, "mc_embed must run first");
  e->pair_drop();
  e->phase_open = false;
  return head(e, e->buf<float>("x"), branch, mode, (hipStream_t)stream);
}

mc_status mc_unpatchify(mc_engine* e, const float* tokens_dev, int tok0, int n_tok, float* out_dev,
                        mc_stream stream_) {
  if (!e || !tokens_dev || !out_dev) return fail(MC_EINVAL, "null argument");
  if (tok0 < 0 || n_tok <= 0 || tok0 + n_tok > e->L) return fail(MC_EINVAL, "token range out of bounds");
  const mc_config& c = e->cfg;
  Prof pr(e, MC_PROF_HEAD, (hipStream_t)stream_);
  HIP_TRY(mc::launch_unpatchify(tokens_dev, e->HT, c.out_dim, c.latent_f, c.latent_h, c.latent_w, tok0, n_tok, out_dev,
                                (hipStream_t)stream_));
  return MC_OK;
}

mc_status mc_pair_begin(mc_engine* e) {
  if (!e) return fail(MC_EINVAL, "null engine");
  e->pair = e->pair_capable() ? mc_engine::PAIR_ARMED : mc_engine::PAIR_NONE;
  return MC_OK;
}

mc_status mc_pair_end(mc_engine* e) {
  if (!e) return fail(MC_EINVAL, "null engine");
  e->pair = mc_engine::PAIR_NONE;
  return MC_OK;
}

static mc_status forward(mc_engine* e, const float* latent_dev, const float* t_dev, double t_host, const void* context_dev,
                         mc_dtype ctx_dtype, int ctx_len, int branch, mc_mode mode, float* out_dev, hipStream_t s) {
  const int d = e->d;
  const bool runs = mode != MC_MODE_SKIP;
  const bool reuse = e->pair == mc_engine::PAIR_KEPT && runs && latent_dev == e->pair_latent && t_dev == e->pair_t_dev &&
                     t_host == e->pair_t_host;
  const bool keep = e->pair == mc_engine::PAIR_ARMED && runs;
  e->pair = keep ? mc_engine::PAIR_KEPT : e->pair == mc_engine::PAIR_NONE ? mc_engine::PAIR_NONE : mc_engine::PAIR_DEAD;
  if (keep) { e->pair_latent = latent_dev; e->pair_t_dev = t_dev; e->pair_t_host = t_host; }
  float* x = e->buf<float>(keep ? "pair_x" : "x");
  bf16_t* cq = e->buf<bf16_t>(keep || reuse ? "pair_cq" : "qkv");
  if (reuse) {
    MC_TRY(check_ready(e));
    Prof pr(e, context_dev ? MC_PROF_EMBED : -1, s);
    MC_TRY(embed_text(e, context_dev, ctx_dtype, ctx_len, s));
  } else {
    MC_TRY(embed(e, latent_dev, t_dev, t_host, context_dev, ctx_dtype, ctx_len, x, s));
  }
  for (int l = 0; runs && l < e->NL; ++l) {
    const Layer& ly = e->layers[l];
    const float* em = e->emod(ly);
    bf16_t* lcq = l == 0 ? cq : e->buf<bf16_t>("qkv");
    if (!(reuse && l == 0)) {
      MC_TRY(block_pre(e, ly, em, x, s));
      MC_TRY(block_post_self(e, ly, em, x, l, lcq, s));
    }
    if (keep && l == 0) {
      Prof pr(e, MC_PROF_OTHER, s);
      if (hipMemcpyAsync(e->buf<float>("x"), x, (size_t)e->Lp * d * 4, hipMemcpyDeviceToDevice, s) != hipSuccess)
        return fail(MC_EHIP, "hipMemcpyAsync of the kept stream failed");
    }
    MC_TRY(block_post_ctx(e, ly, em, x, lcq, l == e->NL - 1 && !hint_on_last_layer(e), branch, mode, s));
    if (e->NV > 0 && l % e->cfg.vace_stride == 0 && l / e->cfg.vace_stride < e->NV)
      MC_TRY(vace_block(e, l / e->cfg.vace_stride, branch, mode, s));
  }
  if (runs && hint_on_last_layer(e)) MC_TRY(capture_unfused(e, branch, mode, s));
  MC_TRY(head(e, x, branch, mode, s));
  return mc_unpatchify(e, e->buf<float>("head_tokens"), 0, e->L, out_dev, (mc_stream)s);
}

mc_status mc_forward(mc_engine* e, const float* latent_dev, const float* t_dev, double t_host,
                     const void* context_dev, mc_dtype ctx_dtype, int ctx_len, int branch, mc_mode mode,
                     float* out_dev, mc_stream stream) {
  if (!e) return fail(MC_EINVAL, "null engine");
  if (e->sp) return fail(MC_ESTATE, "mc_forward is single-GPU; drive a sharded engine through the phase calls");
  if (!out_dev) return fail(MC_EINVAL, "null output");
  if (e->NV > 0 && mode != MC_MODE_SKIP && !e->have_vace)
    return fail(MC_ESTATE, "VACE model: mc_set_vace_context must run before a non-skipped forward");
  if (branch < 0 || branch >= e->cfg.n_branches) return fail(MC_EINVAL, "branch %d out of range", branch);
  const mc_status st = forward(e, latent_dev, t_dev, t_host, context_dev, ctx_dtype, ctx_len, branch, mode, out_dev,
                               (hipStream_t)stream);
  if (st != MC_OK) e->pair_drop();
  return st;
}

mc_status mc_calib_ready(const mc_engine* e, int branch, int* has_stats) {
  if (!e || !has_stats || branch < 0 || branch > 1) return fail(MC_EINVAL, "bad argument");
  *has_stats = e->have_stats[branch] ? 1 : 0;
  return MC_OK;
}

mc_status mc_calib_finalize(mc_engine* e, int branch, mc_stream stream) {
  if (!e || !e->work.ws) return fail(MC_ESTATE, "no workspace");
  if (branch < 0 || branch > 1) return fail(MC_EINVAL, "branch %d out of range", branch);
  HIP_TRY(mc::launch_calib_finalize(e->buf<double>("calib_sums"), e->buf<float>("calib_stats") + 3 * branch,
                                    (hipStream_t)stream));
  return MC_OK;
}

mc_status mc_import_residual(mc_engine* e, int branch, const float* src_dev, mc_stream stream) {
  if (!e || !e->work.ws || !src_dev) return fail(MC_EINVAL, "null argument / no workspace");
  if (branch < 0 || branch >= e->cfg.n_branches) return fail(MC_EINVAL, "branch %d out of range", branch);
  float* dst = e->residual(e->res_slot[branch]);
  if (dst != src_dev)
    HIP_TRY(hipMemcpyAsync(dst, src_dev, (size_t)e->Lr * e->d * sizeof(float), hipMemcpyDeviceToDevice,
                           (hipStream_t)stream));
  e->have_res[branch] = true;
  return MC_OK;
}

mc_status mc_set_context(mc_engine* e, int slot, const void* context_dev, mc_dtype ctx_dtype, int ctx_len,
                         mc_stream stream_) {
  hipStream_t s = (hipStream_t)stream_;
  MC_TRY(check_ready(e));
  if (slot < 0 || slot > 1) return fail(MC_EINVAL, "context slot %d out of range (0, 1)", slot);
  if (e->cfg.no_context_cache) return fail(MC_ESTATE, "the engine was created with no_context_cache: pass the context to every forward");
  if (!context_dev) return fail(MC_EINVAL, "null context");
  const int d = e->d;
  bf16_t* ctx = e->buf<bf16_t>("ctx_cache") + (size_t)slot * e->ctx_rows * d;
  e->ctx_valid[slot] = false;
  MC_TRY(embed_context(e, context_dev, ctx_dtype, ctx_len, ctx, s));
  bf16_t* base = e->buf<bf16_t>("ckv_cache") + (size_t)slot * (e->NL + e->NV) * e->ctx_rows * 2 * d;
  for (int l = 0; l < e->NL + e->NV; ++l) MC_TRY(context_kv(e, e->layer(l), ctx, base + (size_t)l * e->ctx_rows * 2 * d, s));
  e->ctx_valid[slot] = true;
  e->ctx_active = slot;
  return MC_OK;
}

mc_status mc_use_context(mc_engine* e, int slot) {
  if (!e) return fail(MC_EINVAL, "null engine");
  if (slot < -1 || slot > 1) return fail(MC_EINVAL, "context slot %d out of range (-1, 0, 1)", slot);
  if (slot >= 0 && e->cfg.no_context_cache) return fail(MC_ESTATE, "the engine was created with no_context_cache");
  if (slot >= 0 && !e->ctx_valid[slot]) return fail(MC_ESTATE, "context slot %d was never set (mc_set_context)", slot);
  e->ctx_active = slot;
  return MC_OK;
}

mc_status mc_set_token_timesteps(mc_engine* e, const float* t_tokens_dev, mc_stream) {
  if (!e) return fail(MC_EINVAL, "null engine");
  if (t_tokens_dev && e->NV > 0) return fail(MC_EINVAL, "per-token timesteps are not defined for the VACE model");
  if (t_tokens_dev && e->cfg.no_token_timesteps) return fail(MC_ESTATE, "the engine was created with no_token_timesteps");
  e->tok_t = t_tokens_dev;
  e->pair_drop();
  return MC_OK;
}

mc_status mc_profile_enable(mc_engine* e, int on) {
  if (!e) return fail(MC_EINVAL, "null engine");
  if (on < 0 || on > 2) return fail(MC_EINVAL, "profile level %d (0 off, 1 self-attention, 2 every class)", on);
  if (on && e->prof_ev.empty()) {
    e->prof_ev.resize(2 * 8192);
    e->prof_cls.assign(8192, 0);
    for (auto& ev : e->prof_ev) HIP_TRY(hipEventCreate(&ev));
  }
  e->profile = on;
  e->prof_n = 0;
  return MC_OK;
}

mc_status mc_profile_read_classes(mc_engine* e, double ms_total[MC_PROF_NCLASS], int launches[MC_PROF_NCLASS]) {
  if (!e || !ms_total || !launches) return fail(MC_EINVAL, "null argument");
  for (int c = 0; c < MC_PROF_NCLASS; ++c) { ms_total[c] = 0.0; launches[c] = 0; }
  const size_t n = e->prof_n;
  e->prof_n = 0;
  for (size_t i = 0; i + 1 < n; i += 2) {
    const int c = e->prof_cls[i / 2];
    if (c >= MC_PROF_NCLASS) continue;
    HIP_TRY(hipEventSynchronize(e->prof_ev[i + 1]));
    float ms = 0.f;
    HIP_TRY(hipEventElapsedTime(&ms, e->prof_ev[i], e->prof_ev[i + 1]));
    ms_total[c] += ms;
    launches[c] += 1;
  }
  return MC_OK;
}

mc_status mc_profile_read(mc_engine* e, double* attn_ms_total, int* attn_launches) {
  if (!e || !attn_ms_total || !attn_launches) return fail(MC_EINVAL, "null argument");
  double ms[MC_PROF_NCLASS];
  int n[MC_PROF_NCLASS];
  MC_TRY(mc_profile_read_classes(e, ms, n));
  *attn_ms_total = ms[MC_PROF_ATTN_SELF];
  *attn_launches = n[MC_PROF_ATTN_SELF];
  return MC_OK;
}

mc_status mc_state_reset(mc_engine* e) {
  if (!e) return fail(MC_EINVAL, "null engine");
  e->have_res[0] = e->have_res[1] = false;
  e->have_stats[0] = e->have_stats[1] = false;
  return MC_OK;
}

mc_status mc_op_rope_table(int F, int Hp, int Wp, int tok0, int n_tok, float* cs_host) {
  if (!cs_host || n_tok <= 0) return fail(MC_EINVAL, "bad argument");
  rope_table_host(F, Hp, Wp, tok0, n_tok, cs_host);
  return MC_OK;
}

mc_status mc_op_rope_axes(int F, int Hp, int Wp, float* axes_host, size_t* n_floats) {
  if (F <= 0 || Hp <= 0 || Wp <= 0 || (!axes_host && !n_floats)) return fail(MC_EINVAL, "bad argument");
  if (n_floats) *n_floats = rope_axes_floats(F, Hp, Wp);
  if (axes_host) rope_axes_host(F, Hp, Wp, axes_host);
  return MC_OK;
}

}
```

### magcache_amd/engine.py

```python
import ctypes as C

import torch

from . import _lib
from ._lib import MC_BF16, MC_F32, MC_MODE_CALIB, MC_MODE_FULL, MC_MODE_SKIP, McConfig, check
from .adapters import LoraHost

WAN_T2V_1_3B = dict(dim=1536, ffn_dim=8960, freq_dim=256, num_heads=12, num_layers=30, text_len=512, in_dim=16,
                    out_dim=16, text_dim=4096, eps=1e-6)
WAN_T2V_14B = dict(dim=5120, ffn_dim=13824, freq_dim=256, num_heads=40, num_layers=40, text_len=512, in_dim=16,
                   out_dim=16, text_dim=4096, eps=1e-6)
WAN_I2V_14B = dict(WAN_T2V_14B, model_type="i2v", in_dim=36, clip_dim=1280)
N_CLIP_TOKENS = 257
WAN_VACE_1_3B = dict(WAN_T2V_1_3B, model_type="vace", vace_layers=list(range(0, 30, 2)), vace_in_dim=96)
WAN_VACE_14B = dict(WAN_T2V_14B, model_type="vace", vace_layers=list(range(0, 40, 5)), vace_in_dim=96)


def vace_geometry(cfg):
    if "vace_in_dim" not in cfg and "vace_layers" not in cfg:
        return 0, 0
    layers = cfg.get("vace_layers") or list(range(0, cfg["num_layers"], 2))
    stride = layers[1] - layers[0] if len(layers) > 1 else cfg["num_layers"]
    assert layers[0] == 0 and all(b - a == stride for a, b in zip(layers, layers[1:])), \
        f"vace_layers {layers}: the engine takes an arithmetic progression starting at 0 (upstream's configs are)"
    return len(layers), stride


def _stream():
    return C.c_void_p(torch.cuda.current_stream().cuda_stream)


def _ptr(t):
    return C.c_void_p(t.data_ptr()) if t is not None else C.c_void_p(0)


def weight_names(cfg):
    d, ffn = cfg["dim"], cfg["ffn_dim"]
    out = [("patch_embedding.weight", (d, cfg["in_dim"], 1, 2, 2)), ("patch_embedding.bias", (d,)),
           ("text_embedding.0.weight", (d, cfg["text_dim"])), ("text_embedding.0.bias", (d,)),
           ("text_embedding.2.weight", (d, d)), ("text_embedding.2.bias", (d,)),
           ("time_embedding.0.weight", (d, cfg["freq_dim"])), ("time_embedding.0.bias", (d,)),
           ("time_embedding.2.weight", (d, d)), ("time_embedding.2.bias", (d,)),
           ("time_projection.1.weight", (6 * d, d)), ("time_projection.1.bias", (6 * d,)),
           ("head.head.weight", (4 * cfg["out_dim"], d)), ("head.head.bias", (4 * cfg["out_dim"],)),
           ("head.modulation", (1, 2, d))]
    cd = cfg.get("clip_dim", 0)
    if cd:
        out += [("img_emb.proj.0.weight", (cd,)), ("img_emb.proj.0.bias", (cd,)),
                ("img_emb.proj.1.weight", (cd, cd)), ("img_emb.proj.1.bias", (cd,)),
                ("img_emb.proj.3.weight", (d, cd)), ("img_emb.proj.3.bias", (d,)),
                ("img_emb.proj.4.weight", (d,)), ("img_emb.proj.4.bias", (d,))]
    nv, _ = vace_geometry(cfg)
    if nv:
        out += [("vace_patch_embedding.weight", (d, cfg["vace_in_dim"], 1, 2, 2)), ("vace_patch_embedding.bias", (d,)),
                ("vace_blocks.0.before_proj.weight", (d, d)), ("vace_blocks.0.before_proj.bias", (d,))]
        out += [(f"vace_blocks.{i}.after_proj.{w}", (d, d) if w == "weight" else (d,)) for i in range(nv) for w in ("weight", "bias")]
    for p in [f"blocks.{i}." for i in range(cfg["num_layers"])] + [f"vace_blocks.{i}." for i in range(nv)]:
        for a in ("self_attn", "cross_attn"):
            for w in ("q", "k", "v", "o"):
                out += [(p + f"{a}.{w}.weight", (d, d)), (p + f"{a}.{w}.bias", (d,))]
            out += [(p + f"{a}.norm_q.weight", (d,)), (p + f"{a}.norm_k.weight", (d,))]
        if cd:
            out += [(p + "cross_attn.k_img.weight", (d, d)), (p + "cross_attn.k_img.bias", (d,)),
                    (p + "cross_attn.v_img.weight", (d, d)), (p + "cross_attn.v_img.bias", (d,)),
                    (p + "cross_attn.norm_k_img.weight", (d,))]
        out += [(p + "norm3.weight", (d,)), (p + "norm3.bias", (d,)),
                (p + "ffn.0.weight", (ffn, d)), (p + "ffn.0.bias", (ffn,)),
                (p + "ffn.2.weight", (d, ffn)), (p + "ffn.2.bias", (d,)),
                (p + "modulation", (1, 6, d))]
    return out


def synthetic_weights(cfg, seed=0, std=0.02, device="cuda"):
    g = torch.Generator(device=device).manual_seed(seed)
    for name, shape in weight_names(cfg):
        kind = name.replace("img_emb.proj.0.", "img_emb.norm0.").replace("img_emb.proj.4.", "img_emb.norm4.")
        if name.endswith("modulation"):
            t = torch.randn(shape, generator=g, device=device) / cfg["dim"] ** 0.5
        elif "norm" in kind and name.endswith("weight"):
            t = 1.0 + 0.1 * torch.randn(shape, generator=g, device=device)
        elif "norm" in kind and name.endswith("bias"):
            t = 0.1 * torch.randn(shape, generator=g, device=device)
        else:
            t = std * torch.randn(shape, generator=g, device=device)
        yield name, t


class Engine(LoraHost):
    _lora_abi = "mc_lora_"
    _lora_prefix = ""

    def _lora_entries(self, sd, prefix):
        from .lora import parse_wan_lora_state_dict
        return parse_wan_lora_state_dict(sd)

    def __init__(self, cfg, latent_grid, device="cuda:0", sp_rank=0, sp_size=1, n_branches=2, calibration=False,
                 sp_phases=False):
        if not torch.cuda.is_available():
            raise RuntimeError("magcache_amd.Engine needs a ROCm device; there is no CPU fallback")
        self.lib = _lib.load()
        self.cfg = dict(cfg)
        self.device = torch.device(device)
        torch.cuda.set_device(self.device)
        F_, H_, W_ = latent_grid
        self.grid = (F_, H_, W_)
        self.seq_len = F_ * (H_ // 2) * (W_ // 2)
        c = McConfig(dim=cfg["dim"], ffn_dim=cfg["ffn_dim"], num_heads=cfg["num_heads"], num_layers=cfg["num_layers"],
                     in_dim=cfg["in_dim"], out_dim=cfg["out_dim"], freq_dim=cfg["freq_dim"], text_dim=cfg["text_dim"],
                     text_len=cfg["text_len"], latent_f=F_, latent_h=H_, latent_w=W_, eps=cfg.get("eps", 1e-6),
                     sp_rank=sp_rank, sp_size=sp_size, n_branches=n_branches, calibration=int(calibration),
                     clip_dim=cfg.get("clip_dim", 0), vace_layers=vace_geometry(cfg)[0], vace_stride=vace_geometry(cfg)[1],
                     vace_in_dim=cfg.get("vace_in_dim", 0) if vace_geometry(cfg)[0] else 0,
                     fp8_linear=int(cfg.get("fp8_linear", 0) or 0),
                     no_context_cache=int(bool(cfg.get("no_context_cache", 0))),
                     no_token_timesteps=int(bool(cfg.get("no_token_timesteps", 0))), sp_phases=int(bool(sp_phases)))
        self.context_cache = not cfg.get("no_context_cache", 0)
        self.sp_rank, self.sp_size, self.n_branches = sp_rank, sp_size, n_branches
        self.sharded = sp_size > 1 or bool(sp_phases)
        self.vace_layers, self.vace_stride = vace_geometry(cfg)
        h = C.c_void_p()
        check(self.lib.mc_create_sized(C.byref(c), C.sizeof(c), C.byref(h)))
        self.h = h
        self._bind(self.lib.mc_workspace_bytes(self.h))
        self.tokens_per_rank = self.seq_len // sp_size
        self.head_stride = (4 * cfg["out_dim"] + 63) // 64 * 64
        self._tok_t = None
        self._lora_init()

    def _bind(self, nbytes):
        workspace = torch.empty(nbytes + 256, dtype=torch.uint8, device=self.device)
        off = (-workspace.data_ptr()) % 256
        ws = workspace[off:off + nbytes]
        ws.zero_()
        torch.cuda.synchronize(self.device)
        check(self.lib.mc_set_workspace(self.h, _ptr(ws), nbytes))
        self.workspace, self.ws = workspace, ws
        self._tok_t = None

    def geometry_bytes(self, latent_grid):
        n = C.c_size_t()
        f, h, w = (int(v) for v in latent_grid)
        check(self.lib.mc_geometry_bytes(self.h, f, h, w, C.byref(n)))
        return n.value

    def reserve(self, grids):
        need = self.ws.numel()
        for g in grids:
            need = max(need, self.geometry_bytes(g))
        if need > self.ws.numel():
            self._bind(need)
        return need

    def set_geometry(self, latent_grid):
        grid = tuple(int(v) for v in latent_grid)
        if self.sharded:
            raise ValueError("set_geometry: a sharded engine (sp_size > 1 or sp_phases) keeps the grid it was created with")
        need = self.geometry_bytes(grid)
        if need > self.ws.numel():
            self._bind(need)
        check(self.lib.mc_set_geometry(self.h, *grid))
        self.grid = grid
        self.seq_len = grid[0] * (grid[1] // 2) * (grid[2] // 2)
        self.tokens_per_rank = self.seq_len // self.sp_size
        self._tok_t = None

    def __del__(self):
        try:
            if getattr(self, "h", None):
                torch.cuda.synchronize(self.device)
                for comm in getattr(self, "_rccl", []):
                    self.lib.mc_sp_comm_destroy(comm)
                self._rccl = []
                self.lib.mc_destroy(self.h)
                self.h = None
        except Exception:
            pass

    def set_weight(self, name, tensor):
        t = tensor.detach()
        if t.dtype not in (torch.float32, torch.bfloat16):
            t = t.float()
        t = t.to(self.device).contiguous()
        shape = (C.c_int64 * t.dim())(*t.shape)
        dt = MC_F32 if t.dtype == torch.float32 else MC_BF16
        st = self.lib.mc_set_weight(self.h, name.encode(), _ptr(t), dt, shape, t.dim(), _stream())
        if st != 0 and dt == MC_BF16 and b"must be given as fp32" in self.lib.mc_last_error():
            t = t.float()
            st = self.lib.mc_set_weight(self.h, name.encode(), _ptr(t), MC_F32, shape, t.dim(), _stream())
        check(st)
        torch.cuda.current_stream().synchronize()

    def load_weights(self, named_tensors):
        items = named_tensors.items() if hasattr(named_tensors, "items") else named_tensors
        for name, t in items:
            self.set_weight(name, t)
        buf = C.create_string_buffer(4096)
        n = self.lib.mc_weights_missing(self.h, buf, 4096)
        if n:
            raise KeyError(f"{n} weights missing, e.g.: {buf.value.decode().split()[:5]}")

    def buffer(self, name, dtype=torch.uint8):
        off, nb = C.c_size_t(), C.c_size_t()
        check(self.lib.mc_buffer_info(self.h, name.encode(), C.byref(off), C.byref(nb)))
        return self.ws[off.value:off.value + nb.value].view(dtype)

    def residual(self, branch):
        d = self.cfg["dim"]
        return self.buffer(f"residual_branch{branch}", torch.float32).view(-1, d)[:self.tokens_per_rank]

    def set_clip_fea(self, clip_fea):
        c = clip_fea.detach().to(self.device, torch.float32).reshape(-1, clip_fea.shape[-1]).contiguous()
        check(self.lib.mc_set_clip_fea(self.h, _ptr(c), MC_F32, c.shape[0], _stream()))
        torch.cuda.current_stream().synchronize()

    def set_token_timesteps(self, t_tokens):
        if t_tokens is None:
            if self._tok_t is not None:
                check(self.lib.mc_set_token_timesteps(self.h, C.c_void_p(0), _stream()))
                self._tok_t = None
            return
        t = t_tokens.detach().reshape(-1).to(self.device, torch.float32).contiguous()
        assert t.numel() >= self.seq_len, f"per-token timesteps: {t.numel()} < seq_len {self.seq_len}"
        check(self.lib.mc_set_token_timesteps(self.h, _ptr(t), _stream()))
        self._tok_t = t

    def token_timestep_record(self):
        r = self.buffer("tok_t2", torch.float32)[:3].cpu()
        return float(r[0]), float(r[1]), int(r[2])

    def profile(self, on=True):
        check(self.lib.mc_profile_enable(self.h, int(on)))

    def profile_read(self):
        ms, n = C.c_double(), C.c_int()
        check(self.lib.mc_profile_read(self.h, C.byref(ms), C.byref(n)))
        return ms.value, n.value

    def profile_read_classes(self):
        from ._lib import PROF_CLASSES
        ms, n = (C.c_double * len(PROF_CLASSES))(), (C.c_int * len(PROF_CLASSES))()
        check(self.lib.mc_profile_read_classes(self.h, ms, n))
        return {name: (ms[i], n[i]) for i, name in enumerate(PROF_CLASSES)}

    def set_vace_context(self, vace_context, scale=1.0):
        v = None if vace_context is None else vace_context.detach().to(self.device, torch.float32).contiguous()
        check(self.lib.mc_set_vace_context(self.h, _ptr(v), float(scale), _stream()))

    def _ctx(self, context):
        if context.dtype == torch.bfloat16:
            return context.contiguous(), MC_BF16
        return context.float().contiguous(), MC_F32

    def set_context(self, slot, context):
        ctx, cdt = self._ctx(context.to(self.device))
        check(self.lib.mc_set_context(self.h, int(slot), _ptr(ctx), cdt, ctx.shape[0], _stream()))
        self._keep_ctx = ctx

    def use_context(self, slot):
        check(self.lib.mc_use_context(self.h, int(slot)))

    def _ctx_args(self, context):
        if context is None:
            return None, MC_F32, 0
        ctx, cdt = self._ctx(context)
        return ctx, cdt, ctx.shape[0]

    def forward(self, latent, t, context, branch=0, mode=MC_MODE_FULL, out=None):
        assert not self.sharded, "use magcache_amd.parallel.SequenceParallelForward for a sharded engine"
        latent = latent.float().contiguous()
        ctx, cdt, clen = self._ctx_args(context)
        if out is None:
            out = torch.empty((self.cfg["out_dim"],) + self.grid, dtype=torch.float32, device=self.device)
        t_dev, t_host = self._t(t)
        check(self.lib.mc_forward(self.h, _ptr(latent), _ptr(t_dev), t_host, _ptr(ctx), cdt, clen, branch,
                                  mode, _ptr(out), _stream()))
        self._keep = (latent, ctx, t_dev)
        return out

    def _t(self, t):
        if torch.is_tensor(t):
            if t.is_cuda:
                return t.reshape(-1)[:1].to(torch.float32), 0.0
            return None, float(t.reshape(-1)[0])
        return None, float(t)

    def pair_begin(self):
        check(self.lib.mc_pair_begin(self.h))

    def pair_end(self):
        check(self.lib.mc_pair_end(self.h))

    def embed(self, latent, t, context):
        latent = latent.float().contiguous()
        ctx, cdt, clen = self._ctx_args(context)
        t_dev, t_host = self._t(t)
        check(self.lib.mc_embed(self.h, _ptr(latent), _ptr(t_dev), t_host, _ptr(ctx), cdt, clen, _stream()))
        self._keep = (latent, ctx, t_dev)

    def block_pre_attn(self, layer):
        check(self.lib.mc_block_pre_attn(self.h, layer, _stream()))

    def block_pre_kv(self, layer):
        check(self.lib.mc_block_pre_kv(self.h, layer, _stream()))

    def block_pre_q(self, layer):
        check(self.lib.mc_block_pre_q(self.h, layer, _stream()))

    def block_attn_local(self, layer):
        check(self.lib.mc_block_attn_local(self.h, layer, _stream()))

    def block_attn_round(self, layer, rnd):
        check(self.lib.mc_block_attn_round(self.h, layer, rnd, _stream()))

    def sp_set_chunks(self, chunks):
        check(self.lib.mc_sp_set_chunks(self.h, int(chunks)))

    def sp_round_info(self, rnd=0):
        n, rows, valid = C.c_int(), C.c_int(), C.c_int()
        check(self.lib.mc_sp_round_info(self.h, rnd, C.byref(n), C.byref(rows), C.byref(valid)))
        return n.value, rows.value, valid.value

    def rccl_attach(self, group=None):
        import torch.distributed as dist
        rank, n = dist.get_rank(group), dist.get_world_size(group)
        assert n == self.sp_size and rank == self.sp_rank, (n, rank, self.sp_size, self.sp_rank)
        have = torch.tensor([float(self.lib.mc_sp_rccl_available())], device=self.device)
        mine = have.item() > 0.5
        dist.all_reduce(have, op=dist.ReduceOp.MIN, group=group)
        if have.item() < 0.5:
            raise RuntimeError("librccl could not be bound on " + ("this rank: " + self.lib.mc_last_error().decode() if not mine
                                                                  else "another rank of the group"))
        box = [None]
        if rank == 0:
            buf = C.create_string_buffer(128)
            if self.lib.mc_sp_comm_id(buf) == 0:
                box[0] = buf.raw
        src = dist.get_global_rank(group, 0) if group is not None else 0
        dist.broadcast_object_list(box, src=src, group=group)
        if box[0] is None:
            raise RuntimeError("ncclGetUniqueId failed on the group's first rank")
        comm = C.c_void_p()
        check(self.lib.mc_sp_comm_create(C.c_char_p(box[0]), n, rank, C.byref(comm)))
        self._rccl = getattr(self, "_rccl", [])
        self._rccl.append(comm)
        return comm

    def rccl_detach(self, comm):
        torch.cuda.synchronize(self.device)
        self.lib.mc_sp_comm_destroy(comm)
        self._rccl = [c for c in getattr(self, "_rccl", []) if c is not comm]

    def rccl_info(self, comm):
        return self.lib.mc_sp_comm_info(comm).decode()

    def forward_sp_rccl(self, comm, latent, t, context, branch, mode, overlap, tokens_full, out):
        latent = latent.float().contiguous()
        ctx, cdt, clen = self._ctx_args(context)
        t_dev, t_host = self._t(t)
        check(self.lib.mc_forward_sp_rccl(self.h, comm, _ptr(latent), _ptr(t_dev), t_host, _ptr(ctx), cdt, clen, branch, mode,
                                          int(bool(overlap)), _ptr(tokens_full), _ptr(out), _stream()))
        self._keep = (latent, ctx, t_dev)

    def block_post_attn(self, layer, branch, mode):
        check(self.lib.mc_block_post_attn(self.h, layer, branch, mode, _stream()))

    def blocks_sp(self, layer_begin, layer_end, branch, mode, overlap, gather):
        from ._lib import SP_GATHER_FN
        err = []

        def cb(_user, layer, phase, stream_):
            try:
                gather(layer, phase, stream_)
                return 0
            except BaseException as ex:
                err.append(ex)
                return 1
        fn = SP_GATHER_FN(cb)
        st = self.lib.mc_blocks_sp(self.h, layer_begin, layer_end, branch, mode, int(bool(overlap)), fn, None, _stream())
        if err:
            raise err[0]
        check(st)

    def vace_block_pre(self, i):
        check(self.lib.mc_vace_block_pre(self.h, i, _stream()))

    def vace_block_post(self, i, branch, mode):
        check(self.lib.mc_vace_block_post(self.h, i, branch, mode, _stream()))

    def head(self, branch, mode):
        check(self.lib.mc_head(self.h, branch, mode, _stream()))

    def unpatchify(self, tokens, tok0, n_tok, out):
        check(self.lib.mc_unpatchify(self.h, _ptr(tokens), tok0, n_tok, _ptr(out), _stream()))

    def calib_has_stats(self, branch):
        has = C.c_int()
        check(self.lib.mc_calib_ready(self.h, branch, C.byref(has)))
        return bool(has.value)

    def calib_finalize(self, branch):
        check(self.lib.mc_calib_finalize(self.h, branch, _stream()))

    def calib_stats(self, branch):
        has = C.c_int()
        check(self.lib.mc_calib_ready(self.h, branch, C.byref(has)))
        if not has.value:
            return None
        s = self.buffer("calib_stats", torch.float32)[3 * branch:3 * branch + 3].cpu()
        return float(s[0]), float(s[1]), float(s[2])

    def import_residual(self, branch, tensor):
        t = tensor.float().contiguous()
        assert tuple(t.shape) == (self.tokens_per_rank, self.cfg["dim"]), tuple(t.shape)
        check(self.lib.mc_import_residual(self.h, branch, _ptr(t), _stream()))
        self._keep_res = t

    def reset(self):
        check(self.lib.mc_state_reset(self.h))


__all__ = ["Engine", "WAN_T2V_1_3B", "WAN_T2V_14B", "weight_names", "synthetic_weights", "MC_MODE_FULL",
           "MC_MODE_SKIP", "MC_MODE_CALIB"]
```

### magcache_amd/model.py

```python
import json
import os

import numpy as np
import torch

from .engine import MC_MODE_CALIB, MC_MODE_FULL, MC_MODE_SKIP, Engine
from .mag_ratios import TABLES


def nearest_interp(src_array, target_length):
    src_array = np.asarray(src_array)
    if target_length == 1:
        return np.array([src_array[-1]])
    pos = np.arange(target_length) * ((len(src_array) - 1) / (target_length - 1))
    return src_array[np.round(pos).astype(int)]


def resample_cfg_table(mag_ratios, sample_steps):
    mag_ratios = np.asarray(mag_ratios, dtype=np.float64)
    if len(mag_ratios) == sample_steps * 2:
        return mag_ratios
    pair = [nearest_interp(mag_ratios[i::2], sample_steps) for i in (0, 1)]
    return np.stack(pair, axis=1).reshape(-1)


def select_table(ckpt_dir, task="t2v"):
    s = str(ckpt_dir)
    if "vace" in task:
        return TABLES["wan2.1_vace_14B" if "14B" in s else "wan2.1_vace_1.3B"]
    if "i2v" in task:
        return TABLES["wan2.1_i2v_720P" if "720P" in s else "wan2.1_i2v_480P"]
    if "T2V-14B" in s:
        return TABLES["wan2.1_t2v_14B"]
    if "T2V-1.3B" in s:
        return TABLES["wan2.1_t2v_1.3B"]
    raise ValueError(f"no mag_ratios table for ckpt_dir={ckpt_dir!r}; run --magcache_calibration first")


def _version_of(t):
    try:
        return t._version
    except RuntimeError:
        return None


def _fingerprint(t):
    v = t.detach().contiguous()
    words = v.view(torch.int16 if v.element_size() == 2 else (torch.int32 if v.element_size() == 4 else torch.uint8))
    w = words.reshape(-1).to(torch.int64)
    idx = torch.arange(w.numel(), dtype=torch.int64, device=w.device) * 2654435761 + 1
    return torch.stack([w.sum(), (w * idx).sum()])


def _compare_conditioning():
    return os.environ.get("MAGCACHE_COMPARE_CONDITIONING") == "1"


def _tensor_key(t):
    return (t, _version_of(t), _fingerprint(t) if _compare_conditioning() else None)


def _same_tensor(key, t):
    k, ver, fp = key
    now = _version_of(t)
    if ver is None or now is None:
        return False
    same = k is t and ver == now or (k.data_ptr() == t.data_ptr() and k.shape == t.shape and k.dtype == t.dtype and
                                     k.device == t.device and ver == _version_of(k) == now)
    if same and _compare_conditioning():
        same = fp is not None and bool(torch.equal(fp, _fingerprint(t)))
    return same


class WanModelHIP:

    model_type = "t2v"
    patch_size = (1, 2, 2)
    dynamic_geometry = False

    def __init__(self, cfg, latent_grid, device="cuda:0", calibration=True, engine=None, sp_rank=0, sp_size=1,
                 sp_group=None, sp_phases=False, dynamic_geometry=False):
        self.cfg = dict(cfg)
        self.dynamic_geometry = dynamic_geometry
        for k in ("dim", "ffn_dim", "freq_dim", "text_len", "text_dim", "in_dim", "out_dim", "num_heads",
                  "num_layers"):
            setattr(self, k, cfg[k])
        self.latent_grid = tuple(latent_grid)
        if cfg.get("model_type", "t2v") != "t2v":
            self.model_type = cfg["model_type"]
        self._clip_key = None
        self._vace_key = None
        self._ctx_keys = [None, None]
        self._ctx_lru = 0
        self.engine = engine or Engine(cfg, latent_grid, device=device, n_branches=2, calibration=calibration,
                                       sp_rank=sp_rank, sp_size=sp_size, sp_phases=sp_phases)
        self.device = self.engine.device
        self.sp_group = sp_group

    def load_state_dict(self, state_dict):
        self.engine.load_weights(state_dict)
        self._ctx_keys = [None, None]
        return self

    def _cached_context(self, ctx):
        for slot, key in enumerate(self._ctx_keys):
            if key is not None and _same_tensor(key, ctx):
                try:
                    self.engine.use_context(slot)
                except Exception:
                    self._ctx_keys[slot] = None
                    break
                self._ctx_lru = 1 - slot
                return
        slot = self._ctx_lru
        self.engine.set_context(slot, ctx)
        self._ctx_keys[slot] = _tensor_key(ctx)
        self._ctx_lru = 1 - slot

    def _geometry(self, x):
        if not self.dynamic_geometry or len(x) != 1 or x[0].dim() != 4:
            return
        grid = tuple(int(v) for v in x[0].shape[1:])
        if grid == self.latent_grid:
            return
        if getattr(self.engine, "sharded", self.engine.sp_size > 1):
            raise ValueError(f"dynamic_geometry: a sharded engine keeps its latent grid {self.latent_grid} (got {grid})")
        follows = int(getattr(self, "cnt", 0)) != 0 and getattr(type(self), "_sample_grid", None) == grid
        self.check_token_timesteps()
        self.engine.set_geometry(grid)
        self.latent_grid = grid
        self._ctx_keys, self._ctx_lru = [None, None], 0
        self._clip_key = self._vace_key = self._tok_t_key = None
        if follows:
            return
        type(self)._sample_grid = grid
        fresh = dict(cnt=0, accumulated_err=[0.0, 0.0], accumulated_steps=[0, 0], accumulated_ratio=[1.0, 1.0],
                     residual_cache=[None, None], norm_ratio=[], norm_std=[], cos_dis=[])
        for k, v in fresh.items():
            if k in self.__dict__:
                setattr(self, k, v)
            elif hasattr(type(self), k):
                setattr(type(self), k, v)

    def _check_inputs(self, x, context, seq_len, clip_fea, y):
        if self.model_type == "i2v":
            assert clip_fea is not None and y is not None
        assert len(x) == 1 and len(context) == 1, "the engine evaluates one sample per call, as the Wan sampler does"
        self._geometry(x)
        u = x[0]
        c_in = u.shape[0] + (y[0].shape[0] if y is not None else 0)
        assert tuple(u.shape[1:]) == self.latent_grid and c_in == self.in_dim, \
            f"latent {tuple(u.shape)} (+y) does not match the engine grid {(self.in_dim,) + self.latent_grid}"
        if y is not None:
            assert len(y) == 1 and tuple(y[0].shape[1:]) == self.latent_grid
        assert self.engine.seq_len <= seq_len
        assert context[0].shape[0] <= self.text_len and context[0].shape[1] == self.text_dim

    def _run(self, x, t, context, branch, mode, clip_fea=None, y=None, vace=None):
        lat = x[0].to(self.device)
        if y is not None:
            lat = torch.cat([lat, y[0].to(self.device)], dim=0)
        if vace is not None:
            vc, scale = vace[0][0], float(vace[1])
            k = self._vace_key
            if k is None or not _same_tensor(k[0], vc):
                self.engine.set_vace_context(vc, scale)
                self._vace_key = (_tensor_key(vc), scale)
            elif k[1] != scale:
                self.engine.set_vace_context(None, scale)
                self._vace_key = (k[0], scale)
        if clip_fea is not None:
            if self._clip_key is None or not _same_tensor(self._clip_key, clip_fea):
                self.engine.set_clip_fea(clip_fea)
                self._clip_key = _tensor_key(clip_fea)
        if torch.is_tensor(t) and t.numel() > 1:
            assert t.shape[0] == 1 or t.dim() == 1, "one sample per call"
            tv = t.reshape(-1)
            assert tv.numel() >= self.engine.seq_len, f"t has {tv.numel()} entries, the sequence {self.engine.seq_len}"
            tv = tv[:self.engine.seq_len]
            k = getattr(self, "_tok_t_key", None)
            trusted = getattr(t, "_mc_two_valued", False) or os.environ.get("MAGCACHE_VALIDATE_TOKEN_T") == "0"
            if not trusted and (k is None or not _same_tensor(k, t)):
                n = int(torch.unique(tv).numel())
                if n > 2:
                    raise ValueError(f"per-token timesteps with {n} distinct values: the engine supports at most two "
                                     "per forward (Wan2.2 TI2V: conditioning frame + the step's t)")
                self._tok_t_key = _tensor_key(t)
            self.check_token_timesteps(block=False)
            self.engine.set_token_timesteps(tv)
            self._tok_trusted = trusted
            t = tv[-1:]
        elif hasattr(self.engine, "set_token_timesteps"):
            self.engine.set_token_timesteps(None)
        t = t if not torch.is_tensor(t) else t.to(self.device)
        if hasattr(self.engine, "set_context") and getattr(self.engine, "context_cache", True):
            self._cached_context(context[0])
            ctx = None
        else:
            ctx = context[0].to(self.device)
        if getattr(self.engine, "sharded", self.engine.sp_size > 1):
            if getattr(self, "_sp", None) is None:
                from .parallel import SequenceParallelForward
                self._sp = SequenceParallelForward(self.engine, group=self.sp_group)
            out = self._sp.forward(lat, t, ctx, branch, mode)
        else:
            out = self.engine.forward(lat, t, ctx, branch=branch, mode=mode)
        if getattr(self, "_tok_trusted", False):
            self._tok_trusted = False
            if getattr(self, "_tok_ring", None) is None:
                self._tok_ring = [[torch.zeros(3, dtype=torch.float32).pin_memory(), torch.cuda.Event(), False]
                                  for _ in range(16)]
                self._tok_next = 0
            slot = self._tok_ring[self._tok_next]
            if slot[2]:
                slot[1].synchronize()
                self._tok_examine(slot)
            slot[0].copy_(self.engine.buffer("tok_t2", torch.float32)[:3], non_blocking=True)
            slot[1].record()
            slot[2] = True
            self._tok_next = (self._tok_next + 1) % len(self._tok_ring)
        return [out.float()]

    def _lora_call(self, name, *args, **kw):
        try:
            return getattr(self.engine, name)(*args, **kw)
        finally:
            self._ctx_keys, self._ctx_lru = [None, None], 0
            self._clip_key = self._vace_key = None

    def load_lora(self, sd, adapter="default", scale=1.0, strict=True):
        return self._lora_call("load_lora", sd, adapter=adapter, scale=scale, strict=strict)

    def set_adapters(self, names, scales=None):
        return self._lora_call("set_adapters", names, scales)

    def set_lora_call_scale(self, scale):
        return self._lora_call("set_lora_call_scale", scale)

    def unload_lora(self, adapter=None):
        return self._lora_call("unload_lora", adapter)

    def apply_lora(self):
        return self._lora_call("apply_lora")

    def lora_info(self):
        return self.engine.lora_info()

    def pair_begin(self):
        begin = getattr(self.engine, "pair_begin", None)
        if begin is not None:
            begin()

    def pair_end(self):
        end = getattr(self.engine, "pair_end", None)
        if end is not None:
            end()

    @staticmethod
    def _tok_examine(slot):
        slot[2] = False
        tmax, tmin, neither = (float(v) for v in slot[0])
        if neither > 0:
            raise ValueError(f"per-token timesteps: {int(neither)} tokens carried neither t = {tmax:g} nor t = {tmin:g} in a "
                             "forward whose tensor was tagged two-valued (the engine supports at most two distinct values)")

    def check_token_timesteps(self, block=True):
        err = None
        for slot in getattr(self, "_tok_ring", None) or []:
            if not slot[2]:
                continue
            if block:
                slot[1].synchronize()
            elif not slot[1].query():
                continue
            try:
                self._tok_examine(slot)
            except ValueError as ex:
                err = err or ex
        if err is not None:
            raise err

    def __call__(self, *args, **kwargs):
        return type(self).forward(self, *args, **kwargs)


def _i2v_inputs(clip_fea, y):
    return {} if clip_fea is None and y is None else dict(clip_fea=clip_fea, y=y)


def plain_forward(self, x, t, context, seq_len, clip_fea=None, y=None):
    self._check_inputs(x, context, seq_len, clip_fea, y)
    return self._run(x, t, context, 0, MC_MODE_FULL, **_i2v_inputs(clip_fea, y))


WanModelHIP.forward = plain_forward


def _advance(self):
    self.cnt += 1
    if self.cnt >= self.num_steps:
        self.cnt = 0
        self.accumulated_ratio = [1.0, 1.0]
        self.accumulated_err = [0.0, 0.0]
        self.accumulated_steps = [0, 0]


def _decide(self):
    p = self.cnt % 2
    skip_forward = False
    if self.cnt >= int(self.num_steps * self.retention_ratio):
        self.accumulated_ratio[p] = self.accumulated_ratio[p] * self.mag_ratios[self.cnt]
        self.accumulated_steps[p] += 1
        self.accumulated_err[p] += np.abs(1 - self.accumulated_ratio[p])
        if self.accumulated_err[p] < self.magcache_thresh and self.accumulated_steps[p] <= self.K:
            skip_forward = True
        else:
            self.accumulated_err[p] = 0
            self.accumulated_steps[p] = 0
            self.accumulated_ratio[p] = 1.0
    if skip_forward and self.residual_cache[p] is None:
        raise RuntimeError("MagCache asked to skip before any residual was cached (retention_ratio too small?)")
    return p, skip_forward


def _cached_forward(self, x, t, context, **run_kw):
    p, skip_forward = _decide(self)
    out = self._run(x, t, context, p, MC_MODE_SKIP if skip_forward else MC_MODE_FULL, **run_kw)
    self.residual_cache[p] = self.engine.residual(p)
    _advance(self)
    return out


def _calibration_forward(self, x, t, context, **run_kw):
    p = self.cnt % 2
    out = self._run(x, t, context, p, MC_MODE_CALIB, **run_kw)
    if self.cnt >= 2:
        norm_ratio, norm_std, cos_dis = self.engine.calib_stats(p)
        self.norm_ratio.append(round(norm_ratio, 5))
        self.norm_std.append(round(norm_std, 5))
        self.cos_dis.append(round(cos_dis, 5))
        print(f"time: {self.cnt}, norm_ratio: {norm_ratio}, norm_std: {norm_std}, cos_dis: {cos_dis}")
    self.residual_cache[p] = self.engine.residual(p)
    self.cnt += 1
    if self.cnt >= self.num_steps:
        self.cnt = 0
        self.accumulated_ratio = [1.0, 1.0]
        self.accumulated_err = [0.0, 0.0]
        self.accumulated_steps = [0, 0]
        print("norm ratio")
        print(self.norm_ratio)
        print("norm std")
        print(self.norm_std)
        print("cos_dis")
        print(self.cos_dis)
        for fn, v in (("wan2_1_mag_ratio", self.norm_ratio), ("wan2_1_mag_std", self.norm_std),
                      ("wan2_1_cos_dis", self.cos_dis)):
            with open(fn + ".json", "w") as f:
                json.dump(v, f)
    return out


def magcache_forward(self, x, t, context, seq_len, clip_fea=None, y=None):
    self._check_inputs(x, context, seq_len, clip_fea, y)
    return _cached_forward(self, x, t, context, **_i2v_inputs(clip_fea, y))


def magcache_calibration(self, x, t, context, seq_len, clip_fea=None, y=None):
    self._check_inputs(x, context, seq_len, clip_fea, y)
    return _calibration_forward(self, x, t, context, **_i2v_inputs(clip_fea, y))


def _vace_checks(self, x, vace_context, context, seq_len):
    type(self)._check_inputs(self, x, context, seq_len, None, None)
    assert len(vace_context) == 1 and tuple(vace_context[0].shape[1:]) == self.latent_grid \
        and vace_context[0].shape[0] == self.cfg["vace_in_dim"], f"vace_context {tuple(vace_context[0].shape)}"


def magcache_vace_forward(self, x, t, vace_context, context, seq_len, vace_context_scale=1.0, clip_fea=None, y=None):
    _vace_checks(self, x, vace_context, context, seq_len)
    return _cached_forward(self, x, t, context, vace=(vace_context, vace_context_scale))


def magcache_vace_calibration(self, x, t, vace_context, context, seq_len, vace_context_scale=1.0, clip_fea=None, y=None):
    _vace_checks(self, x, vace_context, context, seq_len)
    return _calibration_forward(self, x, t, context, vace=(vace_context, vace_context_scale))


def vace_plain_forward(self, x, t, vace_context, context, seq_len, vace_context_scale=1.0, clip_fea=None, y=None):
    _vace_checks(self, x, vace_context, context, seq_len)
    return self._run(x, t, context, 0, MC_MODE_FULL, vace=(vace_context, vace_context_scale))


def call_branch(model, step, branch, x, t, context, seq_len, **kw):
    cls = type(model)
    has_state = getattr(cls, "forward", None) in (magcache_forward, magcache_calibration, magcache_vace_forward,
                                                  magcache_vace_calibration)
    if has_state:
        model.cnt = 2 * step + branch
    out = model(x, t=t, context=context, seq_len=seq_len, **kw)
    if has_state and branch == 0:
        _advance(model)
    return out


def init_magcache(model, sample_steps, magcache_thresh=0.12, magcache_K=2, retention_ratio=0.2, mag_ratios=None,
                  ckpt_dir="Wan2.1-T2V-1.3B"):
    cls = model.__class__
    cls.forward = magcache_forward
    cls.cnt = 0
    cls.num_steps = sample_steps * 2
    cls.magcache_thresh = magcache_thresh
    cls.K = magcache_K
    cls.accumulated_err = [0.0, 0.0]
    cls.accumulated_steps = [0, 0]
    cls.accumulated_ratio = [1.0, 1.0]
    cls.retention_ratio = retention_ratio
    cls.residual_cache = [None, None]
    table = select_table(ckpt_dir) if mag_ratios is None else np.asarray(mag_ratios, dtype=np.float64)
    cls.mag_ratios = resample_cfg_table(table, sample_steps)
    model.engine.reset()
    return model


def init_magcache_calibration(model, sample_steps):
    cls = model.__class__
    cls.forward = magcache_calibration
    cls.cnt = 0
    cls.num_steps = sample_steps * 2
    cls.norm_ratio, cls.norm_std, cls.cos_dis = [], [], []
    cls.residual_cache = [None, None]
    cls.accumulated_err, cls.accumulated_steps, cls.accumulated_ratio = [0.0, 0.0], [0, 0], [1.0, 1.0]
    model.engine.reset()
    return model


def disable_magcache(model):
    model.__class__.forward = plain_forward
    model.engine.reset()
    return model
```

Measured before the change: 5.466.

## Batch conditional and unconditional CFG forwards into one 2×Lp pass

Adds a deferred pair state. The first CFG forward of a pair runs layer 0 and then parks its state, and the second forward runs both branches together as one batch of 2×Lp rows through the GEMMs, while attention runs per half. Doubling M per GEMM is meant to improve GEMM utilisation and cut per-launch overhead across the two branches. The cost is extra workspace for pair2 buffers and a doubled rope table, plus a more complex state machine that flushes on any state change. Python pair_begin now prefers the batched variant.

```diff
diff --git a/include/magcache_hip.h b/include/magcache_hip.h
--- a/include/magcache_hip.h
+++ b/include/magcache_hip.h
@@ -43,6 +43,7 @@
   int no_context_cache;
   int no_token_timesteps;
   int sp_phases;
+  int no_pair_batch;
 } mc_config;
 
 const char* mc_last_error(void);
@@ -76,7 +77,19 @@
                      float* out_dev, mc_stream stream);
 
 mc_status mc_pair_begin(mc_engine* e);
+mc_status mc_pair_begin_batched(mc_engine* e);
 mc_status mc_pair_end(mc_engine* e);
+enum { MC_PAIR_NONE = 0, MC_PAIR_ARMED = 1, MC_PAIR_KEPT = 2, MC_PAIR_DEFERRED = 3, MC_PAIR_DEAD = 4 };
+enum { MC_PAIR_EV_FORWARD = 0, MC_PAIR_EV_END = 1, MC_PAIR_EV_DROP = 2 };
+enum { MC_PAIR_F_RUNS = 1,
+       MC_PAIR_F_FULL = 2,
+       MC_PAIR_F_SAME_INPUT = 4,
+       MC_PAIR_F_CTX_SLOT = 8,
+       MC_PAIR_F_SAME_STREAM = 16,
+       MC_PAIR_F_CAN_DEFER = 32 };
+enum { MC_PAIR_ACT_FULL = 0, MC_PAIR_ACT_KEEP = 1, MC_PAIR_ACT_DEFER = 2, MC_PAIR_ACT_REUSE = 3, MC_PAIR_ACT_BATCH = 4,
+       MC_PAIR_ACT_FLUSH_FIRST = 8 };
+int mc_op_pair_step(int state, int event, unsigned facts, int* next_state);
 
 mc_status mc_set_context(mc_engine* e, int slot, const void* context_dev, mc_dtype ctx_dtype, int ctx_len,
                          mc_stream stream);
diff --git a/magcache_amd/_lib.py b/magcache_amd/_lib.py
--- a/magcache_amd/_lib.py
+++ b/magcache_amd/_lib.py
@@ -20,7 +20,7 @@
                [("eps", C.c_float)] + \
                [(n, C.c_int) for n in ("sp_rank", "sp_size", "n_branches", "calibration", "clip_dim", "vace_layers",
                                          "vace_stride", "vace_in_dim", "fp8_linear", "no_context_cache",
-                                         "no_token_timesteps", "sp_phases")]
+                                         "no_token_timesteps", "sp_phases", "no_pair_batch")]
 
 
 class MagCacheHipError(RuntimeError):
@@ -48,6 +48,8 @@
     "mc_weights_missing": (_i, [_vp, C.c_char_p, _sz]),
     "mc_forward": (_i, [_vp, _vp, _vp, _d, _vp, _i, _i, _i, _i, _vp, _vp]),
     "mc_pair_begin": (_i, [_vp]),
+    "mc_pair_begin_batched": (_i, [_vp]),
+    "mc_op_pair_step": (_i, [_i, _i, C.c_uint, C.POINTER(_i)]),
     "mc_pair_end": (_i, [_vp]),
     "mc_set_clip_fea": (_i, [_vp, _vp, _i, _i, _vp]),
     "mc_set_vace_context": (_i, [_vp, _vp, _f, _vp]),
diff --git a/magcache_amd/csrc/engine.cpp b/magcache_amd/csrc/engine.cpp
--- a/magcache_amd/csrc/engine.cpp
+++ b/magcache_amd/csrc/engine.cpp
@@ -25,6 +25,28 @@
 }
 
 constexpr int kSpMaxParts = 9;
+
+struct mc_engine;
+static mc_status pair_flush(mc_engine* e, int then);
+
+struct PairStep { int action; bool flush; int next; };
+static PairStep pair_step(int state, int event, unsigned f) {
+  const bool deferred = state == MC_PAIR_DEFERRED;
+  if (event == MC_PAIR_EV_END) return {MC_PAIR_ACT_FULL, deferred, MC_PAIR_NONE};
+  if (event == MC_PAIR_EV_DROP) return {MC_PAIR_ACT_FULL, deferred, state == MC_PAIR_NONE ? MC_PAIR_NONE : MC_PAIR_DEAD};
+  const bool runs = f & MC_PAIR_F_RUNS, full = f & MC_PAIR_F_FULL, same = f & MC_PAIR_F_SAME_INPUT, slot = f & MC_PAIR_F_CTX_SLOT;
+  if (deferred) {
+    if (runs && full && same && slot && (f & MC_PAIR_F_SAME_STREAM))
+      return {MC_PAIR_ACT_BATCH, false, MC_PAIR_DEAD};
+    state = MC_PAIR_KEPT;
+  }
+  if (state == MC_PAIR_KEPT && runs && same) return {MC_PAIR_ACT_REUSE, deferred, MC_PAIR_DEAD};
+  if (state == MC_PAIR_ARMED && runs) {
+    if (full && slot && (f & MC_PAIR_F_CAN_DEFER)) return {MC_PAIR_ACT_DEFER, false, MC_PAIR_DEFERRED};
+    return {MC_PAIR_ACT_KEEP, false, MC_PAIR_KEPT};
+  }
+  return {MC_PAIR_ACT_FULL, deferred, state == MC_PAIR_NONE ? MC_PAIR_NONE : MC_PAIR_DEAD};
+}
 
 struct mc_engine {
   mc_config cfg;
@@ -73,12 +95,22 @@
   bool have_res[2] = {false, false};
   bool have_stats[2] = {false, false};
   bool embedded = false;
-  enum { PAIR_NONE, PAIR_ARMED, PAIR_KEPT, PAIR_DEAD };
+  enum { PAIR_NONE = MC_PAIR_NONE, PAIR_ARMED = MC_PAIR_ARMED, PAIR_KEPT = MC_PAIR_KEPT, PAIR_DEFERRED = MC_PAIR_DEFERRED,
+         PAIR_DEAD = MC_PAIR_DEAD };
   int pair = PAIR_NONE;
   const float *pair_latent = nullptr, *pair_t_dev = nullptr;
   double pair_t_host = 0.0;
+  float* pair_kept_x = nullptr;
+  bool pair_may_defer = false;
+  struct { int ctx = -1, branch = 0; float* out = nullptr; hipStream_t s = nullptr; } pair_def;
   bool pair_capable() const { return !sp && NV == 0 && cfg.clip_dim == 0 && cfg.fp8_linear == 0; }
-  void pair_drop() { if (pair != PAIR_NONE) pair = PAIR_DEAD; }
+  bool pair_batch() const { return pair_capable() && !cfg.no_pair_batch && !cfg.no_context_cache; }
+  mc_status pair_drop() {
+    const PairStep st = pair_step(pair, MC_PAIR_EV_DROP, 0);
+    if (st.flush) return pair_flush(this, st.next);
+    pair = st.next;
+    return MC_OK;
+  }
 
   template <class T>
   T* buf(const char* name) const { return work.get<T>(name); }
@@ -236,15 +268,22 @@
   ws.add("calib_stats", 2 * 3 * 4);
   ws.add("pair_x", e->pair_capable() ? Lp * d * 4 : 256);
   ws.add("pair_cq", e->pair_capable() ? Lp * d * 2 : 256);
+  const size_t two = e->pair_batch() ? 2 * Lp : 0;
+  ws.add("pair2_x", two ? two * d * 4 : 256);
+  ws.add("pair2_xn", two ? two * d * 2 : 256);
+  ws.add("pair2_qkv", two ? two * 3 * d * 2 : 256);
+  ws.add("pair2_ao", two ? two * d * 2 : 256);
+  ws.add("pair2_h", two ? two * ffn * 2 : 256);
 }
 
 mc_status rope_reserve(mc_engine* e, int Lp, size_t axes_floats) {
-  if (Lp > e->cs_rows) {
+  const int rows = e->pair_batch() ? 2 * Lp : Lp;
+  if (rows > e->cs_rows) {
     float* grown = nullptr;
-    MC_TRY(e->weights.alloc(&grown, (size_t)Lp * 128));
+    MC_TRY(e->weights.alloc(&grown, (size_t)rows * 128));
     if (e->cs_table) e->weights.release(e->cs_table);
     e->cs_table = grown;
-    e->cs_rows = Lp;
+    e->cs_rows = rows;
   }
   if (axes_floats > e->axes_cap) {
     float* grown = nullptr;
@@ -262,6 +301,8 @@
   rope_axes_host(F, Hp, Wp, axes.data());
   HIP_TRY(hipMemcpy(e->rope_axes, axes.data(), axes.size() * sizeof(float), hipMemcpyHostToDevice));
   HIP_TRY(mc::launch_rope_expand(e->rope_axes, F, Hp, Wp, e->tok0, e->Lr, e->Lp, e->cs_table, nullptr));
+  if (e->pair_batch())
+    HIP_TRY(mc::launch_rope_expand(e->rope_axes, F, Hp, Wp, e->tok0, e->Lr, e->Lp, e->cs_table + (size_t)e->Lp * 128, nullptr));
   HIP_TRY(hipStreamSynchronize(nullptr));
   return MC_OK;
 }
@@ -276,7 +317,7 @@
   e->have_clip = e->have_vace = false;
   e->tok_t = nullptr;
   e->attn_layer = -2;
-  e->pair_drop();
+  if (e->pair != mc_engine::PAIR_NONE) e->pair = mc_engine::PAIR_DEAD;
   if (e->work.ws) HIP_TRY(hipMemset(e->buf<double>("calib_partial") + 2048 * 4, 0, 16));
   return MC_OK;
 }
@@ -323,9 +364,22 @@
   return linear(e, l, whole(l), M, a, p, epi, s);
 }
 
+struct Pass {
+  float* x;
+  bf16_t *xn, *qkv, *ao, *h;
+  int M, halves;
+  int ctx[2];
+  int branch[2];
+  mc_mode mode;
+};
+Pass pass_one(const mc_engine* e, float* x, int branch = 0, mc_mode mode = MC_MODE_FULL) {
+  return {x, e->buf<bf16_t>("xn"), e->buf<bf16_t>("qkv"), e->buf<bf16_t>("ao"), e->buf<bf16_t>("h"), e->Lp, 1,
+          {e->ctx_active, -1}, {branch, branch}, mode};
+}
+
 Keys kv_pairs(const bf16_t* kv, int d, int rows, int valid) { return {kv, kv + d, 2L * d, 0, rows, valid, 1, 0}; }
-Keys qkv_keys(const mc_engine* e) {
-  const bf16_t* k = e->buf<bf16_t>("qkv") + e->d;
+Keys qkv_keys(const mc_engine* e, const bf16_t* qkv) {
+  const bf16_t* k = qkv + e->d;
   return {k, k + e->d, 3L * e->d, 0, e->Lp, e->Lr, 1, 0};
 }
 Keys local_keys(const mc_engine* e) { return kv_pairs(e->buf<bf16_t>("kv_local"), e->d, e->Lp, e->Lr); }
@@ -394,6 +448,7 @@
                                                    (c.vace_layers - 1) * c.vace_stride >= c.num_layers)))
     return fail(MC_EINVAL, "bad VACE geometry: %d blocks, stride %d, in_dim %d", c.vace_layers, c.vace_stride, c.vace_in_dim);
   if ((c.no_context_cache | c.no_token_timesteps) & ~1) return fail(MC_EINVAL, "no_context_cache / no_token_timesteps must be 0 or 1");
+  if (c.no_pair_batch & ~1) return fail(MC_EINVAL, "no_pair_batch must be 0 or 1");
   if (c.fp8_linear < 0 || c.fp8_linear > 3)
     return fail(MC_EINVAL, "fp8_linear must be 0, 1 (per-row scales), 2 (MX block scales: QKV, FFN-1, FFN-2) or 3 (MX, the d x d Linears too)");
   if (c.fp8_linear && ((c.dim % 256) || (c.ffn_dim % 256) || c.dim < 512 || c.ffn_dim < 512))
@@ -511,6 +566,7 @@
 
 mc_status mc_set_workspace(mc_engine* e, void* ws_dev, size_t bytes) {
   if (!e) return fail(MC_EINVAL, "null argument");
+  MC_TRY(e->pair_drop());
   MC_TRY(e->work.bind(ws_dev, bytes));
   return forget_workspace_state(e);
 }
@@ -537,6 +593,7 @@
   if (e->work.ws && plan.need > e->work.bound)
     return fail(MC_EINVAL, "latent grid %dx%dx%d needs a workspace of %zu bytes, %zu bytes are bound (mc_set_workspace)", latent_f,
                 latent_h, latent_w, plan.need, e->work.bound);
+  MC_TRY(e->pair_drop());
   HIP_TRY(hipDeviceSynchronize());
   MC_TRY(rope_reserve(e, r.Lp, rope_axes_floats(latent_f, latent_h / 2, latent_w / 2)));
   MC_TRY(e->work.replan(plan));
@@ -559,9 +616,9 @@
 mc_status mc_set_weight(mc_engine* e, const char* name, const void* src_dev, mc_dtype dtype, const int64_t* shape,
                         int ndim, mc_stream stream) {
   if (e) {
+    MC_TRY(e->pair_drop());
     e->ctx_valid[0] = e->ctx_valid[1] = false;
     e->ctx_active = -1;
-    e->pair_drop();
   }
   if (!e || !name || !src_dev || !shape) return fail(MC_EINVAL, "null argument");
   return e->weights.set(name, src_dev, dtype, shape, ndim, (hipStream_t)stream);
@@ -613,7 +670,7 @@
     e->ctx_valid[0] = e->ctx_valid[1] = false;
     e->ctx_active = -1;
     e->have_clip = e->have_vace = false;
-    e->pair_drop();
+    MC_TRY(e->pair_drop());
   }
   return st;
 }
@@ -627,7 +684,7 @@
 mc_status mc_set_clip_fea(mc_engine* e, const void* clip_dev, mc_dtype dtype, int n_tokens, mc_stream stream_) {
   hipStream_t s = (hipStream_t)stream_;
   MC_TRY(check_ready(e));
-  e->pair_drop();
+  MC_TRY(e->pair_drop());
   const mc_config& c = e->cfg;
   if (c.clip_dim <= 0) return fail(MC_EINVAL, "engine was created without clip_dim (t2v model)");
   if (!clip_dev || n_tokens != 257) return fail(MC_EINVAL, "clip_fea must be [257, %d]", c.clip_dim);
@@ -653,7 +710,7 @@
 mc_status mc_set_vace_context(mc_engine* e, const float* vace_dev, float context_scale, mc_stream stream_) {
   hipStream_t s = (hipStream_t)stream_;
   MC_TRY(check_ready(e));
-  e->pair_drop();
+  MC_TRY(e->pair_drop());
   if (e->NV <= 0) return fail(MC_EINVAL, "engine was created without VACE blocks");
   const mc_config& c = e->cfg;
   const int d = e->d;
@@ -764,17 +821,18 @@
 
 mc_status mc_embed(mc_engine* e, const float* latent_dev, const float* t_dev, double t_host,
                    const void* context_dev, mc_dtype ctx_dtype, int ctx_len, mc_stream stream_) {
-  if (e) e->pair_drop();
+  if (e) MC_TRY(e->pair_drop());
   const mc_status st = embed(e, latent_dev, t_dev, t_host, context_dev, ctx_dtype, ctx_len, e ? e->buf<float>("x") : nullptr,
                              (hipStream_t)stream_);
   if (e && st == MC_OK) e->phase_open = true;
   return st;
 }
 
-static mc_status ln_for_gemm(mc_engine* e, const Linear& l, const float* x, const float* sc, const float* sh, int mode,
+static mc_status ln_for_gemm(mc_engine* e, const Linear& l, const Pass& ps, const float* sc, const float* sh, int mode,
                              const float* sc2, const float* sh2, const uint8_t* sel, hipStream_t s, ActSrc* a) {
-  const int d = e->d, Lp = e->Lp;
-  bf16_t* xn = e->buf<bf16_t>("xn");
+  const int d = e->d, Lp = ps.M;
+  const float* x = ps.x;
+  bf16_t* xn = ps.xn;
   *a = ActSrc{xn, d, l.q && mc::g_fp8_fused_quant};
   if (a->quantised) {
     HIP_TRY(mc::launch_ln_modulate_fp8(x, d, sc, sh, mode, e->cfg.eps, e->buf<uint8_t>("aq"), d,
@@ -791,17 +849,17 @@
 }
 static const uint8_t* tok_sel(const mc_engine* e) { return e->tok_t ? e->buf<uint8_t>("tok_sel") : nullptr; }
 
-static mc_status block_pre_kv(mc_engine* e, const Layer& l, const float* em, float* x, hipStream_t s) {
-  const int d = e->d, Lp = e->Lp;
+static mc_status block_pre_kv(mc_engine* e, const Layer& l, const float* em, const Pass& ps, hipStream_t s) {
+  const int d = e->d, Lp = ps.M;
   const float* em2 = second_set(e, em);
   ActSrc a;
   {
     Prof pr(e, MC_PROF_LN_MODULATE, s);
-    MC_TRY(ln_for_gemm(e, l.qkv, x, em + d, em, 0, em2 ? em2 + d : nullptr, em2, tok_sel(e), s, &a));
+    MC_TRY(ln_for_gemm(e, l.qkv, ps, em + d, em, 0, em2 ? em2 + d : nullptr, em2, tok_sel(e), s, &a));
   }
   mc::GemmParams p = {};
   if (!e->sp) {
-    bf16_t* qkv = e->buf<bf16_t>("qkv");
+    bf16_t* qkv = ps.qkv;
     p.Cb = qkv; p.ldc = 3 * d;
     {
       Prof pr(e, MC_PROF_GEMM_QKV, s);
@@ -839,8 +897,8 @@
   return MC_OK;
 }
 
-static mc_status block_pre(mc_engine* e, const Layer& l, const float* em, float* x, hipStream_t s) {
-  MC_TRY(block_pre_kv(e, l, em, x, s));
+static mc_status block_pre(mc_engine* e, const Layer& l, const float* em, const Pass& ps, hipStream_t s) {
+  MC_TRY(block_pre_kv(e, l, em, ps, s));
   return block_pre_q(e, l, s);
 }
 
@@ -852,21 +910,21 @@
 
 mc_status mc_block_pre_attn(mc_engine* e, int layer, mc_stream stream_) {
   MC_TRY(check_layer_call(e, layer));
-  e->pair_drop();
-  return block_pre(e, e->layers[layer], e->emod(e->layers[layer]), e->buf<float>("x"), (hipStream_t)stream_);
+  MC_TRY(e->pair_drop());
+  return block_pre(e, e->layers[layer], e->emod(e->layers[layer]), pass_one(e, e->buf<float>("x")), (hipStream_t)stream_);
 }
 
 mc_status mc_block_pre_kv(mc_engine* e, int layer, mc_stream stream_) {
   MC_TRY(check_layer_call(e, layer));
   if (!e->sp) return fail(MC_ESTATE, "mc_block_pre_kv needs a sequence-parallel engine (sp_size > 1 or sp_phases) (one GPU: mc_block_pre_attn / mc_forward)");
-  e->pair_drop();
-  return block_pre_kv(e, e->layers[layer], e->emod(e->layers[layer]), e->buf<float>("x"), (hipStream_t)stream_);
+  MC_TRY(e->pair_drop());
+  return block_pre_kv(e, e->layers[layer], e->emod(e->layers[layer]), pass_one(e, e->buf<float>("x")), (hipStream_t)stream_);
 }
 
 mc_status mc_block_pre_q(mc_engine* e, int layer, mc_stream stream_) {
   MC_TRY(check_layer_call(e, layer));
   if (!e->sp) return fail(MC_ESTATE, "mc_block_pre_q needs a sequence-parallel engine (sp_size > 1 or sp_phases)");
-  e->pair_drop();
+  MC_TRY(e->pair_drop());
   return block_pre_q(e, e->layers[layer], (hipStream_t)stream_);
 }
 
@@ -931,8 +989,7 @@
     return fail(MC_EINVAL, "sp chunks %d: rows per shard %d / chunks must be a multiple of 64", chunks, e->Lp);
   e->sp_chunks = chunks;
   e->attn_layer = -2;
-  e->pair_drop();
-  return MC_OK;
+  return e->pair_drop();
 }
 
 mc_status mc_sp_geometry(const mc_engine* e, int* num_layers, int* seq_len, int* rows_per_rank, int* head_stride, int* dim,
@@ -958,15 +1015,20 @@
   return MC_OK;
 }
 
-static mc_status block_post_self(mc_engine* e, const Layer& l, const float* em, float* x, int layer, bf16_t* cq, hipStream_t s) {
-  const int d = e->d, Lp = e->Lp;
-  bf16_t* ao = e->buf<bf16_t>("ao");
+static mc_status block_post_self(mc_engine* e, const Layer& l, const float* em, const Pass& ps, int layer, bf16_t* cq,
+                                   hipStream_t s) {
+  const int d = e->d, Lp = ps.M;
+  float* x = ps.x;
+  bf16_t* ao = ps.ao;
   const float* em2 = second_set(e, em);
   const uint8_t* sel = tok_sel(e);
 
   if (!e->sp) {
-    Prof pr(e, MC_PROF_ATTN_SELF, s);
-    MC_TRY(attend(e, e->buf<bf16_t>("qkv"), 3 * d, ao, qkv_keys(e), nullptr, nullptr, s));
+    for (int hf = 0; hf < ps.halves; ++hf) {
+      Prof pr(e, MC_PROF_ATTN_SELF, s);
+      const bf16_t* qkv = ps.qkv + (size_t)hf * e->Lp * 3 * d;
+      MC_TRY(attend(e, qkv, 3 * d, ao + (size_t)hf * e->Lp * d, qkv_keys(e, qkv), nullptr, nullptr, s));
+    }
   } else {
     attn_chain_open(e, layer);
     while (e->attn_rounds_done < sp_rounds(e)) MC_TRY(sp_attn_launch(e, layer, e->attn_rounds_done, s));
@@ -982,7 +1044,7 @@
   ActSrc xn;
   {
     Prof pr(e, MC_PROF_LN_MODULATE, s);
-    MC_TRY(ln_for_gemm(e, l.cq, x, l.n3w, l.n3b, 1, nullptr, nullptr, nullptr, s, &xn));
+    MC_TRY(ln_for_gemm(e, l.cq, ps, l.n3w, l.n3b, 1, nullptr, nullptr, nullptr, s, &xn));
   }
   {
     Prof pr(e, MC_PROF_GEMM_CROSS_Q, s);
@@ -1013,23 +1075,25 @@
   return MC_OK;
 }
 
-static mc_status block_post_ctx(mc_engine* e, const Layer& l, const float* em, float* x, const bf16_t* cq, bool capture,
-                                int branch, mc_mode mode, hipStream_t s) {
-  const int d = e->d, Lp = e->Lp, ffn = e->ffn;
-  bf16_t* ao = e->buf<bf16_t>("ao");
+static mc_status block_post_ctx(mc_engine* e, const Layer& l, const float* em, const Pass& ps, const bf16_t* cq, size_t cq_half,
+                                bool capture, hipStream_t s) {
+  const int d = e->d, Lp = ps.M, ffn = e->ffn;
+  float* x = ps.x;
+  bf16_t* ao = ps.ao;
   const float* em2 = second_set(e, em);
   const uint8_t* sel = tok_sel(e);
-  bf16_t* ckv = e->buf<bf16_t>("ckv");
   {
-    if (e->ctx_active >= 0) {
-      ckv = e->buf<bf16_t>("ckv_cache") + ((size_t)e->ctx_active * (e->NL + e->NV) + l.index) * e->ctx_rows * 2 * d;
-    } else {
-      Prof pr(e, MC_PROF_OTHER, s);
-      MC_TRY(context_kv(e, l, e->buf<bf16_t>("ctx"), ckv, s));
-    }
-    {
+    for (int hf = 0; hf < ps.halves; ++hf) {
+      bf16_t* ckv = e->buf<bf16_t>("ckv");
+      if (ps.ctx[hf] >= 0) {
+        ckv = e->buf<bf16_t>("ckv_cache") + ((size_t)ps.ctx[hf] * (e->NL + e->NV) + l.index) * e->ctx_rows * 2 * d;
+      } else {
+        Prof pr(e, MC_PROF_OTHER, s);
+        MC_TRY(context_kv(e, l, e->buf<bf16_t>("ctx"), ckv, s));
+      }
       Prof pr(e, MC_PROF_ATTN_CROSS, s);
-      MC_TRY(attend(e, cq, d, ao, kv_pairs(ckv, d, e->ctx_rows, e->cfg.text_len), nullptr, nullptr, s));
+      MC_TRY(attend(e, cq + hf * cq_half, d, ao + (size_t)hf * e->Lp * d, kv_pairs(ckv, d, e->ctx_rows, e->cfg.text_len), nullptr,
+                    nullptr, s));
     }
     if (e->cfg.clip_dim > 0) {
       Prof pr(e, MC_PROF_OTHER, s);
@@ -1048,10 +1112,10 @@
   ActSrc xn;
   {
     Prof pr(e, MC_PROF_LN_MODULATE, s);
-    MC_TRY(ln_for_gemm(e, l.ffn1, x, em + 4 * d, em + 3 * d, 0, em2 ? em2 + 4 * d : nullptr, em2 ? em2 + 3 * d : nullptr, sel,
+    MC_TRY(ln_for_gemm(e, l.ffn1, ps, em + 4 * d, em + 3 * d, 0, em2 ? em2 + 4 * d : nullptr, em2 ? em2 + 3 * d : nullptr, sel,
                        s, &xn));
   }
-  bf16_t* h = e->buf<bf16_t>("h");
+  bf16_t* h = ps.h;
   mc::GemmParams p = {};
   p.Cb = h; p.ldc = ffn;
   const bool h_fp8 = l.ffn1.mx && l.ffn2.mx && mc::g_fp8_fused_quant;
@@ -1068,21 +1132,29 @@
   q.X = x; q.ldx = d; q.gate = em + 5 * d;
   if (e->splitk_bytes) { q.splitk_ws = e->buf<float>("splitk"); q.splitk_ws_bytes = e->splitk_bytes; }
   if (em2) { q.gate2 = em2 + 5 * d; q.gate_sel = sel; }
-  if (capture) {
+  if (!capture) {
+    Prof pr(e, MC_PROF_GEMM_FFN2, s);
+    return linear(e, l.ffn2, whole(l.ffn2), Lp, hidden, q, mc::EPI_RESID_GATE, s);
+  }
+  for (int hf = 0; hf < ps.halves; ++hf) {
+    q.X = x + (size_t)hf * e->Lp * d;
     q.X0 = e->buf<bf16_t>("x0"); q.ldx0 = d;
-    q.R = capture_dst(e, branch, mode); q.ldr = d;
-  }
-  {
-    Prof pr(e, MC_PROF_GEMM_FFN2, s);
-    MC_TRY(linear(e, l.ffn2, whole(l.ffn2), Lp, hidden, q, capture ? mc::EPI_RESID_CAPTURE : mc::EPI_RESID_GATE, s));
-  }
-  return capture ? capture_written(e, branch, mode, true, s) : MC_OK;
-}
-
-static mc_status block_post(mc_engine* e, const Layer& l, const float* em, float* x, int layer, bf16_t* cq, bool capture,
-                            int branch, mc_mode mode, hipStream_t s) {
-  MC_TRY(block_post_self(e, l, em, x, layer, cq, s));
-  return block_post_ctx(e, l, em, x, cq, capture, branch, mode, s);
+    q.R = capture_dst(e, ps.branch[hf], ps.mode); q.ldr = d;
+    ActSrc rows = hidden;
+    rows.rows = h + (size_t)hf * e->Lp * ffn;
+    {
+      Prof pr(e, MC_PROF_GEMM_FFN2, s);
+      MC_TRY(linear(e, l.ffn2, whole(l.ffn2), e->Lp, rows, q, mc::EPI_RESID_CAPTURE, s));
+    }
+    MC_TRY(capture_written(e, ps.branch[hf], ps.mode, true, s));
+  }
+  return MC_OK;
+}
+
+static mc_status block_post(mc_engine* e, const Layer& l, const float* em, const Pass& ps, int layer, bf16_t* cq, bool capture,
+                            hipStream_t s) {
+  MC_TRY(block_post_self(e, l, em, ps, layer, cq, s));
+  return block_post_ctx(e, l, em, ps, cq, 0, capture, s);
 }
 
 static bool hint_on_last_layer(const mc_engine* e) {
@@ -1093,9 +1165,9 @@
   if (!e || !e->embedded) return fail(MC_ESTATE, "mc_embed must run first");
   if (layer < 0 || layer >= e->NL) return fail(MC_EINVAL, "layer %d out of range", layer);
   if (branch < 0 || branch >= e->cfg.n_branches) return fail(MC_EINVAL, "branch %d out of range", branch);
-  e->pair_drop();
-  return block_post(e, e->layers[layer], e->emod(e->layers[layer]), e->buf<float>("x"), layer, e->buf<bf16_t>("qkv"),
-                    layer == e->NL - 1 && !hint_on_last_layer(e), branch, mode, (hipStream_t)stream_);
+  MC_TRY(e->pair_drop());
+  return block_post(e, e->layers[layer], e->emod(e->layers[layer]), pass_one(e, e->buf<float>("x"), branch, mode), layer,
+                    e->buf<bf16_t>("qkv"), layer == e->NL - 1 && !hint_on_last_layer(e), (hipStream_t)stream_);
 }
 
 static mc_status vace_pre_kv(mc_engine* e, int i, hipStream_t s) {
@@ -1108,7 +1180,7 @@
     p.X = xc; p.ldx = d; p.gate = nullptr;
     MC_TRY(linear(e, e->before, whole(e->before), Lp, ActSrc{e->buf<bf16_t>("c0"), d}, p, mc::EPI_RESID_GATE, s));
   }
-  return block_pre_kv(e, e->vlayers[i], e->emod(e->vlayers[i]), xc, s);
+  return block_pre_kv(e, e->vlayers[i], e->emod(e->vlayers[i]), pass_one(e, xc), s);
 }
 
 static mc_status vace_pre(mc_engine* e, int i, hipStream_t s) {
@@ -1119,7 +1191,7 @@
 static mc_status vace_post(mc_engine* e, int i, int branch, mc_mode mode, hipStream_t s) {
   const int d = e->d, Lp = e->Lp;
   float* xc = e->buf<float>("xc");
-  MC_TRY(block_post(e, e->vlayers[i], e->emod(e->vlayers[i]), xc, -1, e->buf<bf16_t>("qkv"), false, branch, mode, s));
+  MC_TRY(block_post(e, e->vlayers[i], e->emod(e->vlayers[i]), pass_one(e, xc, branch, mode), -1, e->buf<bf16_t>("qkv"), false, s));
   bf16_t* xn = e->buf<bf16_t>("xn");
   HIP_TRY(mc::launch_cast_bf16(xc, xn, (size_t)Lp * d, s));
   mc::GemmParams h = {};
@@ -1211,7 +1283,7 @@
     return MC_OK;
   };
   for (int l = layer_begin; l < layer_end; ++l) {
-    MC_TRY(block_pre_kv(e, e->layers[l], e->emod(e->layers[l]), e->buf<float>("x"), s));
+    MC_TRY(block_pre_kv(e, e->layers[l], e->emod(e->layers[l]), pass_one(e, e->buf<float>("x")), s));
     MC_TRY(chain(l, e->layers[l], l));
     MC_TRY(mc_block_post_attn(e, l, branch, mode, stream));
     if (e->NV > 0 && l % e->cfg.vace_stride == 0 && l / e->cfg.vace_stride < e->NV) {
@@ -1255,7 +1327,7 @@
 
 mc_status mc_head(mc_engine* e, int branch, mc_mode mode, mc_stream stream) {
   if (!e) return fail(MC_ESTATE, "mc_embed must run first");
-  e->pair_drop();
+  MC_TRY(e->pair_drop());
   e->phase_open = false;
   return head(e, e->buf<float>("x"), branch, mode, (hipStream_t)stream);
 }
@@ -1271,29 +1343,96 @@
   return MC_OK;
 }
 
-mc_status mc_pair_begin(mc_engine* e) {
+static mc_status pair_begin(mc_engine* e, bool may_defer) {
   if (!e) return fail(MC_EINVAL, "null engine");
+  MC_TRY(pair_flush(e, mc_engine::PAIR_NONE));
   e->pair = e->pair_capable() ? mc_engine::PAIR_ARMED : mc_engine::PAIR_NONE;
-  return MC_OK;
-}
+  e->pair_may_defer = may_defer;
+  return MC_OK;
+}
+
+mc_status mc_pair_begin(mc_engine* e) { return pair_begin(e, false); }
+
+mc_status mc_pair_begin_batched(mc_engine* e) { return pair_begin(e, true); }
 
 mc_status mc_pair_end(mc_engine* e) {
   if (!e) return fail(MC_EINVAL, "null engine");
-  e->pair = mc_engine::PAIR_NONE;
-  return MC_OK;
+  const PairStep step = pair_step(e->pair, MC_PAIR_EV_END, 0);
+  const mc_status st = step.flush ? pair_flush(e, step.next) : MC_OK;
+  e->pair = step.next;
+  return st;
+}
+
+static mc_status run_layers(mc_engine* e, const Pass& ps, int first, const bf16_t* cq0, float* const out[2], hipStream_t s) {
+  const int d = e->d;
+  for (int l = first; l < e->NL; ++l) {
+    const Layer& ly = e->layers[l];
+    const float* em = e->emod(ly);
+    const bool capture = l == e->NL - 1 && !hint_on_last_layer(e);
+    if (l == first && cq0) {
+      MC_TRY(block_post_ctx(e, ly, em, ps, cq0, 0, capture, s));
+    } else {
+      MC_TRY(block_pre(e, ly, em, ps, s));
+      MC_TRY(block_post_self(e, ly, em, ps, l, ps.qkv, s));
+      MC_TRY(block_post_ctx(e, ly, em, ps, ps.qkv, (size_t)e->Lp * d, capture, s));
+    }
+    if (e->NV > 0 && l % e->cfg.vace_stride == 0 && l / e->cfg.vace_stride < e->NV)
+      MC_TRY(vace_block(e, l / e->cfg.vace_stride, ps.branch[0], ps.mode, s));
+  }
+  if (hint_on_last_layer(e)) MC_TRY(capture_unfused(e, ps.branch[0], ps.mode, s));
+  for (int hf = 0; hf < ps.halves; ++hf) {
+    MC_TRY(head(e, ps.x + (size_t)hf * e->Lp * d, ps.branch[hf], ps.mode, s));
+    MC_TRY(mc_unpatchify(e, e->buf<float>("head_tokens"), 0, e->L, out[hf], (mc_stream)s));
+  }
+  return MC_OK;
+}
+
+static mc_status pair_flush(mc_engine* e, int then) {
+  if (e->pair != mc_engine::PAIR_DEFERRED) return MC_OK;
+  e->pair = mc_engine::PAIR_DEAD;
+  Pass ps = pass_one(e, e->buf<float>("pair2_x"), e->pair_def.branch, MC_MODE_FULL);
+  ps.ctx[0] = e->pair_def.ctx;
+  float* const out[2] = {e->pair_def.out, nullptr};
+  MC_TRY(run_layers(e, ps, 0, e->buf<bf16_t>("pair_cq"), out, e->pair_def.s));
+  e->pair = then;
+  return MC_OK;
+}
+
+static mc_status pair_run_both(mc_engine* e, int branch, float* out_dev, hipStream_t s) {
+  e->pair = mc_engine::PAIR_DEAD;
+  const Pass ps = {e->buf<float>("pair2_x"), e->buf<bf16_t>("pair2_xn"), e->buf<bf16_t>("pair2_qkv"), e->buf<bf16_t>("pair2_ao"),
+                   e->buf<bf16_t>("pair2_h"), 2 * e->Lp, 2, {e->pair_def.ctx, e->ctx_active}, {e->pair_def.branch, branch},
+                   MC_MODE_FULL};
+  float* const out[2] = {e->pair_def.out, out_dev};
+  return run_layers(e, ps, 0, e->buf<bf16_t>("pair_cq"), out, s);
+}
+
+static bool pair_batch_fits(const mc_engine* e) {
+  return (size_t)2 * e->Lp * std::max(3 * e->d, e->ffn) < (1ull << 31);
 }
 
 static mc_status forward(mc_engine* e, const float* latent_dev, const float* t_dev, double t_host, const void* context_dev,
                          mc_dtype ctx_dtype, int ctx_len, int branch, mc_mode mode, float* out_dev, hipStream_t s) {
   const int d = e->d;
   const bool runs = mode != MC_MODE_SKIP;
-  const bool reuse = e->pair == mc_engine::PAIR_KEPT && runs && latent_dev == e->pair_latent && t_dev == e->pair_t_dev &&
-                     t_host == e->pair_t_host;
-  const bool keep = e->pair == mc_engine::PAIR_ARMED && runs;
-  e->pair = keep ? mc_engine::PAIR_KEPT : e->pair == mc_engine::PAIR_NONE ? mc_engine::PAIR_NONE : mc_engine::PAIR_DEAD;
+  const bool slot_ready = !context_dev && e->ctx_active >= 0 && e->ctx_valid[e->ctx_active];
+  const bool can_defer = e->pair_may_defer && e->pair_batch() && !e->tok_t && pair_batch_fits(e);
+  const unsigned facts = (runs ? MC_PAIR_F_RUNS : 0) | (mode == MC_MODE_FULL ? MC_PAIR_F_FULL : 0) |
+                         (latent_dev == e->pair_latent && t_dev == e->pair_t_dev && t_host == e->pair_t_host ? MC_PAIR_F_SAME_INPUT : 0) |
+                         (slot_ready ? MC_PAIR_F_CTX_SLOT : 0) | (s == e->pair_def.s ? MC_PAIR_F_SAME_STREAM : 0) |
+                         (can_defer ? MC_PAIR_F_CAN_DEFER : 0);
+  const PairStep step = pair_step(e->pair, MC_PAIR_EV_FORWARD, facts);
+  if (step.flush) MC_TRY(pair_flush(e, mc_engine::PAIR_KEPT));
+  if (step.action == MC_PAIR_ACT_BATCH) {
+    MC_TRY(check_ready(e));
+    return pair_run_both(e, branch, out_dev, s);
+  }
+  const bool reuse = step.action == MC_PAIR_ACT_REUSE, defer = step.action == MC_PAIR_ACT_DEFER;
+  const bool keep = defer || step.action == MC_PAIR_ACT_KEEP;
+  e->pair = defer ? mc_engine::PAIR_KEPT : step.next;
   if (keep) { e->pair_latent = latent_dev; e->pair_t_dev = t_dev; e->pair_t_host = t_host; }
-  float* x = e->buf<float>(keep ? "pair_x" : "x");
-  bf16_t* cq = e->buf<bf16_t>(keep || reuse ? "pair_cq" : "qkv");
+  float* x = defer ? e->buf<float>("pair2_x") : keep ? e->buf<float>("pair_x") : reuse ? e->pair_kept_x : e->buf<float>("x");
+  const bf16_t* cq0 = keep || reuse ? e->buf<bf16_t>("pair_cq") : nullptr;
   if (reuse) {
     MC_TRY(check_ready(e));
     Prof pr(e, context_dev ? MC_PROF_EMBED : -1, s);
@@ -1301,26 +1440,27 @@
   } else {
     MC_TRY(embed(e, latent_dev, t_dev, t_host, context_dev, ctx_dtype, ctx_len, x, s));
   }
-  for (int l = 0; runs && l < e->NL; ++l) {
-    const Layer& ly = e->layers[l];
-    const float* em = e->emod(ly);
-    bf16_t* lcq = l == 0 ? cq : e->buf<bf16_t>("qkv");
-    if (!(reuse && l == 0)) {
-      MC_TRY(block_pre(e, ly, em, x, s));
-      MC_TRY(block_post_self(e, ly, em, x, l, lcq, s));
-    }
-    if (keep && l == 0) {
-      Prof pr(e, MC_PROF_OTHER, s);
-      if (hipMemcpyAsync(e->buf<float>("x"), x, (size_t)e->Lp * d * 4, hipMemcpyDeviceToDevice, s) != hipSuccess)
-        return fail(MC_EHIP, "hipMemcpyAsync of the kept stream failed");
-    }
-    MC_TRY(block_post_ctx(e, ly, em, x, lcq, l == e->NL - 1 && !hint_on_last_layer(e), branch, mode, s));
-    if (e->NV > 0 && l % e->cfg.vace_stride == 0 && l / e->cfg.vace_stride < e->NV)
-      MC_TRY(vace_block(e, l / e->cfg.vace_stride, branch, mode, s));
-  }
-  if (runs && hint_on_last_layer(e)) MC_TRY(capture_unfused(e, branch, mode, s));
-  MC_TRY(head(e, x, branch, mode, s));
-  return mc_unpatchify(e, e->buf<float>("head_tokens"), 0, e->L, out_dev, (mc_stream)s);
+  const Pass ps = pass_one(e, x, branch, mode);
+  float* const out[2] = {out_dev, nullptr};
+  if (keep) {
+    const Layer& ly = e->layers[0];
+    MC_TRY(block_pre(e, ly, e->emod(ly), ps, s));
+    MC_TRY(block_post_self(e, ly, e->emod(ly), ps, 0, e->buf<bf16_t>("pair_cq"), s));
+    e->pair_kept_x = defer ? x + (size_t)e->Lp * d : e->buf<float>("x");
+    Prof pr(e, MC_PROF_OTHER, s);
+    if (hipMemcpyAsync(e->pair_kept_x, x, (size_t)e->Lp * d * 4, hipMemcpyDeviceToDevice, s) != hipSuccess)
+      return fail(MC_EHIP, "hipMemcpyAsync of the kept stream failed");
+  }
+  if (defer) {
+    e->pair_def.ctx = e->ctx_active; e->pair_def.branch = branch; e->pair_def.out = out_dev; e->pair_def.s = s;
+    e->pair = mc_engine::PAIR_DEFERRED;
+    return MC_OK;
+  }
+  if (!runs) {
+    MC_TRY(head(e, x, branch, mode, s));
+    return mc_unpatchify(e, e->buf<float>("head_tokens"), 0, e->L, out_dev, (mc_stream)s);
+  }
+  return run_layers(e, ps, 0, cq0, out, s);
 }
 
 mc_status mc_forward(mc_engine* e, const float* latent_dev, const float* t_dev, double t_host,
@@ -1334,7 +1474,7 @@
   if (branch < 0 || branch >= e->cfg.n_branches) return fail(MC_EINVAL, "branch %d out of range", branch);
   const mc_status st = forward(e, latent_dev, t_dev, t_host, context_dev, ctx_dtype, ctx_len, branch, mode, out_dev,
                                (hipStream_t)stream);
-  if (st != MC_OK) e->pair_drop();
+  if (st != MC_OK && e->pair != mc_engine::PAIR_NONE) e->pair = mc_engine::PAIR_DEAD;
   return st;
 }
 
@@ -1355,6 +1495,7 @@
 mc_status mc_import_residual(mc_engine* e, int branch, const float* src_dev, mc_stream stream) {
   if (!e || !e->work.ws || !src_dev) return fail(MC_EINVAL, "null argument / no workspace");
   if (branch < 0 || branch >= e->cfg.n_branches) return fail(MC_EINVAL, "branch %d out of range", branch);
+  MC_TRY(e->pair_drop());
   float* dst = e->residual(e->res_slot[branch]);
   if (dst != src_dev)
     HIP_TRY(hipMemcpyAsync(dst, src_dev, (size_t)e->Lr * e->d * sizeof(float), hipMemcpyDeviceToDevice,
@@ -1370,6 +1511,7 @@
   if (slot < 0 || slot > 1) return fail(MC_EINVAL, "context slot %d out of range (0, 1)", slot);
   if (e->cfg.no_context_cache) return fail(MC_ESTATE, "the engine was created with no_context_cache: pass the context to every forward");
   if (!context_dev) return fail(MC_EINVAL, "null context");
+  if (e->pair == mc_engine::PAIR_DEFERRED && slot == e->pair_def.ctx) MC_TRY(e->pair_drop());
   const int d = e->d;
   bf16_t* ctx = e->buf<bf16_t>("ctx_cache") + (size_t)slot * e->ctx_rows * d;
   e->ctx_valid[slot] = false;
@@ -1394,8 +1536,8 @@
   if (!e) return fail(MC_EINVAL, "null engine");
   if (t_tokens_dev && e->NV > 0) return fail(MC_EINVAL, "per-token timesteps are not defined for the VACE model");
   if (t_tokens_dev && e->cfg.no_token_timesteps) return fail(MC_ESTATE, "the engine was created with no_token_timesteps");
+  MC_TRY(e->pair_drop());
   e->tok_t = t_tokens_dev;
-  e->pair_drop();
   return MC_OK;
 }
 
@@ -1441,9 +1583,16 @@
 
 mc_status mc_state_reset(mc_engine* e) {
   if (!e) return fail(MC_EINVAL, "null engine");
+  MC_TRY(e->pair_drop());
   e->have_res[0] = e->have_res[1] = false;
   e->have_stats[0] = e->have_stats[1] = false;
   return MC_OK;
+}
+
+int mc_op_pair_step(int state, int event, unsigned facts, int* next_state) {
+  const PairStep st = pair_step(state, event, facts);
+  if (next_state) *next_state = st.next;
+  return st.action | (st.flush ? MC_PAIR_ACT_FLUSH_FIRST : 0);
 }
 
 mc_status mc_op_rope_table(int F, int Hp, int Wp, int tok0, int n_tok, float* cs_host) {
diff --git a/magcache_amd/engine.py b/magcache_amd/engine.py
--- a/magcache_amd/engine.py
+++ b/magcache_amd/engine.py
@@ -113,7 +113,8 @@
                      vace_in_dim=cfg.get("vace_in_dim", 0) if vace_geometry(cfg)[0] else 0,
                      fp8_linear=int(cfg.get("fp8_linear", 0) or 0),
                      no_context_cache=int(bool(cfg.get("no_context_cache", 0))),
-                     no_token_timesteps=int(bool(cfg.get("no_token_timesteps", 0))), sp_phases=int(bool(sp_phases)))
+                     no_token_timesteps=int(bool(cfg.get("no_token_timesteps", 0))), sp_phases=int(bool(sp_phases)),
+                     no_pair_batch=int(bool(cfg.get("no_pair_batch", 0))))
         self.context_cache = not cfg.get("no_context_cache", 0)
         self.sp_rank, self.sp_size, self.n_branches = sp_rank, sp_size, n_branches
         self.sharded = sp_size > 1 or bool(sp_phases)
@@ -286,6 +287,9 @@
 
     def pair_begin(self):
         check(self.lib.mc_pair_begin(self.h))
+
+    def pair_begin_batched(self):
+        check(self.lib.mc_pair_begin_batched(self.h))
 
     def pair_end(self):
         check(self.lib.mc_pair_end(self.h))
diff --git a/magcache_amd/model.py b/magcache_amd/model.py
--- a/magcache_amd/model.py
+++ b/magcache_amd/model.py
@@ -247,7 +247,7 @@
         return self.engine.lora_info()
 
     def pair_begin(self):
-        begin = getattr(self.engine, "pair_begin", None)
+        begin = getattr(self.engine, "pair_begin_batched", None) or getattr(self.engine, "pair_begin", None)
         if begin is not None:
             begin()
 
```

Result: no change. 5.443 (-0.4%).
